# EasyVision-Ton/VMG

Measured on AMD Instinct MI355X. Metric: LR-frames/s (train: forward+loss+backward+AdamW), VMG-REDS-few_levels 4x SR, higher is better.
Workload: dtype bf16; 1 GPU; VMG-REDS-few_levels train step, per-GPU batch 4x7x3x64x64 -> 4x SR (BASELINE configs[1]); global_batch=4, frames_per_clip=7, parallelism=dp1, launch=eager, recompute_chains=False, fp8_chains=False

## Files before the change

include/vmg_hip.h:

```cpp
#ifndef VMG_HIP_H
#define VMG_HIP_H

#include <stdint.h>

#ifdef __cplusplus
extern "C" {
#endif

#define VMG_F32 0
#define VMG_BF16 1

#define VMG_ACT_NONE 0
#define VMG_ACT_RELU 1
#define VMG_ACT_LRELU 2
#define VMG_ACT_GELU 3

#define VMG_CONV_GENERAL 0
#define VMG_CONV_KSPLIT 2
#define VMG_CONV_WS 3
#define VMG_CONV_LINEAR_WRES 4
#define VMG_CONV_WSTAT 6

const char* vmg_last_error(void);
int vmg_version(void);

typedef struct vmg_ctx vmg_ctx;
vmg_ctx* vmg_create(int device);
int vmg_destroy(vmg_ctx* ctx);
int vmg_ctx_device(const vmg_ctx* ctx);
int vmg_max_lds_bytes(void);

int64_t vmg_conv_pack_bytes(int dtype, int ks, int on, int nsrc, const int* src_ch, int cout_tiles);
int vmg_conv_pack(int dtype, const float* w, int O, int I, int ks, int o0, int on, int nsrc, const int* src_off,
                  const int* src_ch, int transpose_flip, int cout_tiles, void* packed, void* stream);

int64_t vmg_convws_pack_bytes(int on, int nsrc, const int* src_ch, int cout_tiles);
int vmg_convws_pack(const float* w, int O, int I, int o0, int on, int nsrc, const int* src_off, const int* src_ch, int transpose_flip,
                    int cout_tiles, void* packed, void* stream);

typedef struct vmg_conv_desc {
  int dtype, ks, cout_tiles;
  int N, H, W, Cout;
  int nsrc;
  const void* src[4];
  int64_t src_ps[4];
  int src_ch[4];
  const void* packed;
  const float* bias;
  void* out;
  int64_t out_ps;
  void* out_pre;
  const void* res;
  int64_t res_ps;
  const void* aux;
  int64_t aux_ps;
  int act;
  float slope, alpha;
  int actgrad;
  int pixel_shuffle;
  int mt;
  int deep;
} vmg_conv_desc;

int vmg_conv_fwd(const vmg_conv_desc* d, void* stream);
enum {
  VMG_CONV_FAM_IGEMM = 1,
  VMG_CONV_FAM_KSPLIT = 2,
  VMG_CONV_FAM_WS = 3,
  VMG_CONV_FAM_LINEAR_WRES = 4,
  VMG_CONV_FAM_WSTAT = 5,
  VMG_CONV_PLAN_INTS = 11
};
int vmg_conv_fwd_plan(const vmg_conv_desc* d, int ncu, int* plan);
typedef struct vmg_chain_desc {
  int dtype, N, H, W, C, nblk, nsrc;
  const void* src[4];
  int64_t src_ps[4];
  int src_ch[4];
  const void* packed0;
  const float* bias0;
  float slope0;
  int cout_tiles0, deep0;
  const void* const* packed1;
  const float* const* bias1;
  const void* const* packed2;
  const float* const* bias2;
  float r_scaling;
  int cout_tiles, deep;
  void* const* y;
  void* const* t;
  void* const* g_y;
  void* const* g_t;
} vmg_chain_desc;
int vmg_resblock_chain_fwd(const vmg_chain_desc* d, void* stream);
int vmg_resblock_chain_bwd(const vmg_chain_desc* d, void* stream);

void* vmg_replay_build(void* hip_graph, int* n_ops, int* n_kernels);
int vmg_replay_kernel_info(void* replay, int idx, void** func, unsigned* grid_x, unsigned* block_x, void** first_arg);
int vmg_replay_run(void* replay, int first, int last, void* stream);
void vmg_replay_destroy(void* replay);

int vmg_pack_entry_bytes(void);
int vmg_pack_entry(void* entry, int kind, int dtype, const float* w, int O, int I, int ks, int o0, int on, int nsrc, const int* src_off,
                   const int* src_ch, int transpose_flip, int cout_tiles, void* packed, int blk0);
int vmg_pack_run(const void* plan_dev, int n, int total_blocks, void* stream);

int vmg_conv_debug_stamps(void* buf);

int vmg_conv_wgrad(int dtype, int ks, int N, int H, int W, const void* x, int64_t x_ps, int Cin, const void* dy,
                   int64_t dy_ps, int Cout, float* dW, int I_total, int o0, int i0, float* db, float scale,
                   void* stream);
int vmg_conv_wgrad_batched(int dtype, int ks, int npairs, const void* const* x, const void* const* dy, int N, int H, int W,
                           int64_t x_ps, int Cin, int64_t dy_ps, int Cout, float* dW, int I_total, int o0, int i0, float* db,
                           float scale, void* stream);

int64_t vmg_conv_wgrad_ws_bytes(void);
int vmg_conv_wgrad_batched_ws(int dtype, int ks, int npairs, const void* const* x, const void* const* dy, int N, int H, int W,
                              int64_t x_ps, int Cin, int64_t dy_ps, int Cout, float* dW, int I_total, int o0, int i0, float* db,
                              float scale, void* ws, int64_t ws_bytes, void* stream);
int vmg_conv_wgrad3_multi(int nprob, int npairs, const void* const* x, const void* const* dy, int N, int H, int W, int64_t x_ps, int Cin,
                          int64_t dy_ps, int Cout, float* const* dW, int I_total, int o0, int i0, float* const* db, const float* scales, void* ws,
                          int64_t ws_bytes, void* stream);
int vmg_conv_wgrad3_variant(int variant);
int vmg_linear_wgrad2_multi(int nprob, int npairs, const void* const* x, const void* const* dy, int64_t M, int64_t x_ps, int Cin, int64_t dy_ps,
                            int Cout, float* const* dW, int I_total, int o0, int i0, float* const* db, const float* scales, void* ws,
                            int64_t ws_bytes, void* stream);
#define VMG_WGRAD_V1 1
#define VMG_WGRAD_3 2
#define VMG_WGRAD_3B 3
#define VMG_WGRAD_L2 4
#define VMG_WGRAD_7 5
int vmg_conv_wgrad_last_kernel(void);
#define VMG_WGRAD_ENTRY_PLAIN 0
#define VMG_WGRAD_ENTRY_WS 1
#define VMG_WGRAD_ENTRY_MULTI 2
#define VMG_WGRAD_ALIGN_X16 1
#define VMG_WGRAD_ALIGN_DY16 2
#define VMG_WGRAD_ALIGN_DY2 4
#define VMG_WGRAD_PLAN_INTS 7
int vmg_conv_wgrad_plan(int entry, int dtype, int ks, int nprob, int npairs, int N, int H, int W, int64_t x_ps, int Cin, int64_t dy_ps, int Cout,
                        int I_total, int o0, int i0, int align, int64_t ws_bytes, int* plan);

int vmg_act_bwd(int dtype, const void* dy, const void* ref, void* out, int64_t n, int act, float slope, float alpha,
                void* stream);
int vmg_pixel_shuffle(int dtype, const void* in, void* out, int N, int H, int W, int c, int to_depth, void* stream);
int vmg_sum_n(int dtype, const void* const* srcs, int nsrc, void* out, int64_t n, void* stream);
int vmg_cast_clear(int dtype, float* acc, const void* add, void* out, int64_t n, void* stream);
int vmg_pair_steps(int dtype, int mode, void* const* steps, void* a, void* b, int n, int t, int64_t frame_elems, void* stream);
int vmg_frame_gather(int dtype, const void* src, void* dst, const int* idx, int64_t frame_elems, int n_src_frames, int n_dst_frames, int nsrc,
                     void* stream);
int vmg_pixel_unshuffle_actgrad(int dtype, const void* dy, const void* ref, void* out, int N, int H, int W, int c, int act, float slope,
                                float alpha, void* stream);
int vmg_layernorm_fwd(int dtype, const void* x, const float* w, const float* b, void* y, float* mean, float* rstd, int64_t M,
                      int C, float eps, void* stream);
int64_t vmg_layernorm_bwd_ws_bytes(void);
int vmg_layernorm_bwd(int dtype, int ndy, const void* const* dy, const void* x, const float* mean, const float* rstd, const float* w,
                      const void* add, void* dx, float* dw, float* db, int64_t M, int C, void* ws, void* stream);

int vmg_space_depth_ln_fwd(int dtype, int mode, const void* x, const float* w, const float* b, void* y, float* mean, float* rstd, int N, int H,
                           int W, int cseg, float eps, void* stream);
int vmg_space_depth_ln_bwd(int dtype, int mode, const void* dy, const void* x, const float* mean, const float* rstd, const float* w, void* dx,
                           float* dw, float* db, int N, int H, int W, int cseg, void* ws, void* stream);

int64_t vmg_group_reduce_ws_bytes(void);
int vmg_group_reduce(int dtype, const void* a, const void* b, const void* c3, float* out, int G, int64_t R, int C, int mode, float scale,
                     float* ws, int64_t ws_bytes, void* stream);
int vmg_group_reduce3(int dtype, const void* a, const void* b0, const void* b1, const void* b2, float* out, int G, int64_t R, int C, float scale,
                      float* ws, int64_t ws_bytes, void* stream);
int vmg_tab_elementwise(int dtype, int op, const void* p0, const void* p1, const void* p2, const float* coef, const float* add, float s,
                        void* o0, void* o1, void* o2, int64_t rows, int64_t R, int C, void* stream);

int vmg_warp_bilinear_fwd(int dtype, const void* x, const float* flow, void* out, int N, int H, int W, int C, void* stream);
int vmg_warp_bilinear_bwd(int dtype, const void* x, const float* flow, const void* dy, void* dx_acc, float* dflow, int N, int H,
                          int W, int C, void* stream);
int vmg_warp_nearest_planes(const float* loc, const float* flow, float* out, int N, int K2, int H, int W, void* stream);
int vmg_flow_smooth(const float* in, float* out, int64_t planes, int H, int W, int r, int backward, void* stream);

int vmg_ltam_fwd(int dtype, const void* q, const void* const* keys, const void* const* vals, const float* loc, const float* rpe,
                 const float* decay, void* out, float* lse, int n, int h, int w, int c, int heads, int wh, int ww, int t, float scale,
                 void* stream);
int vmg_ltam_bwd(int dtype, const void* q, const void* const* keys, const void* const* vals, const float* loc, const float* rpe,
                 const float* decay, const void* out, const float* lse, const void* dout, void* dq, void* const* dk_acc,
                 void* const* dv_acc, float* drpe, int n, int h, int w, int c, int heads, int wh, int ww, int t, float scale,
                 void* stream);
int64_t vmg_ltam_tab_bytes(int t);
int vmg_ltam_fwd_tab(int dtype, const void* q, const void* const* keys, const void* const* vals, const float* loc, const float* rpe,
                     const float* decay, void* out, float* lse, int n, int h, int w, int c, int heads, int wh, int ww, int t, float scale,
                     void* ws, int64_t ws_bytes, void* stream);
int vmg_ltam_bwd_tab(int dtype, const void* q, const void* const* keys, const void* const* vals, const float* loc, const float* rpe,
                     const float* decay, const void* out, const float* lse, const void* dout, void* dq, void* const* dk_acc,
                     void* const* dv_acc, float* drpe, int n, int h, int w, int c, int heads, int wh, int ww, int t, float scale,
                     void* ws, int64_t ws_bytes, void* stream);

int vmg_ltam_max_fwd(int dtype, const void* q, const void* const* keys, const void* const* vals, const float* loc, void* out, int* idx,
                     float* score, int n, int h, int w, int c, int heads, int t, void* stream);
int vmg_ltam_max_bwd(int dtype, const void* q, const void* const* keys, const void* const* vals, const float* loc, const int* idx,
                     const void* dout, void* dq, void* const* dk_acc, void* const* dv_acc, int n, int h, int w, int c, int heads, int t,
                     void* stream);
int vmg_ltam_max_fwd_tab(int dtype, const void* q, const void* const* keys, const void* const* vals, const float* loc, void* out, int* idx,
                         float* score, int n, int h, int w, int c, int heads, int t, void* ws, int64_t ws_bytes, void* stream);
int vmg_ltam_max_bwd_tab(int dtype, const void* q, const void* const* keys, const void* const* vals, const float* loc, const int* idx,
                         const void* dout, void* dq, void* const* dk_acc, void* const* dv_acc, int n, int h, int w, int c, int heads, int t,
                         void* ws, int64_t ws_bytes, void* stream);

int vmg_prof_begin(vmg_ctx* ctx, int klass, int stride, int max_samples);
int vmg_prof_end(vmg_ctx* ctx, int64_t* launches_seen, int* samples, double* total_ms);
int vmg_prof_select_pixels(vmg_ctx* ctx, int64_t pixels);
double vmg_prof_null_interval_us(int reps, void* stream);

int vmg_morphfc_fwd(int axis, int chunk, const void* x, const void* relu_mask, const void* packed, const float* bias, void* out, void* tok_out,
                    int BT, int H, int W, int C, int Cp, int cout_tiles, int relu, float in_scale, float out_scale, void* stream);
int64_t vmg_morphfc_token_rows(int axis, int chunk, int BT, int H, int W);
int64_t vmg_morph_token_rows(int axis, int chunk, int BT, int H, int W);
int vmg_morph_tokens_gather(int dtype, int axis, int chunk, const void* x, void* tok, int BT, int H, int W, int C, int Cp, int ld, void* stream);
int vmg_morph_tokens_scatter(int dtype, int axis, int chunk, const void* tok, void* out, int BT, int H, int W, int C, int Cp, int ld, void* stream);

int vmg_win3d_attn_fwd(int dtype, const void* q, const void* kv, const float* bq, const float* bkv, const float* table, void* out, float* lse,
                       int B, int D, int H, int W, int C, int heads, int wt, int sd, int sh, int sw, void* stream);
int64_t vmg_win3d_attn_bwd_ws_bytes(int B, int D, int H, int W, int heads, int wt);
int vmg_win3d_attn_bwd(int dtype, const void* q, const void* kv, const float* bq, const float* bkv, const float* table, const void* out,
                       const float* lse, const void* d_out, void* dq, void* dkv, float* dtable, float* dbq, float* dbkv, void* ws, int B, int D, int H, int W,
                       int C, int heads, int wt, int sd, int sh, int sw, void* stream);
int vmg_win3d_variant(int variant);

int vmg_maxpool_fwd(int dtype, const void* x, void* y, unsigned char* idx, int N, int H, int W, int C, int f, void* stream);
int vmg_maxpool_bwd(int dtype, const void* dy, const unsigned char* idx, void* dx, int N, int H, int W, int C, int f, void* stream);

int vmg_se_mlp_fwd(const float* m, const float* w1, const float* b1, const float* w2, const float* b2, float* pre, float* out, int G, int C,
                   int Hd, int Co, int act1, int mode, void* stream);
int vmg_se_mlp_bwd(const float* dout, const float* out, const float* m, const float* pre, const float* w1, const float* w2, float* dm,
                   float* dw1, float* db1, float* dw2, float* db2, float* ws, int G, int C, int Hd, int Co, int act1, int mode, float dm_scale,
                   int accumulate, void* stream);

int vmg_avgpool2_nhwc(int dtype, const void* x, void* y, int n, int h, int w, int c, void* stream);
int vmg_upsample2x_ac_fwd(const float* x, float* y, int n, int h, int w, int c, float scale, void* stream);
int vmg_upsample2x_ac_bwd(const float* dy, float* dx, int n, int h, int w, int c, float scale, void* stream);
int vmg_spy_operand_fwd(int dtype, const void* ref, const void* warped, const float* up, void* out, int64_t npix, void* stream);
int vmg_spy_operand_bwd(int dtype, const void* dx8, void* dwarped, float* dup, int64_t npix, void* stream);
int vmg_spy_flow_add(int dtype, const float* up, const void* res, float* out, int64_t n, void* stream);
int vmg_spy_prep(int dtype, const float* img, const float* mean, const float* stdv, void* out, int64_t n, int h, int w, void* stream);
typedef struct vmg_spy_module_desc {
  int N, H, W;
  const void* x;
  const void* packed[5];
  const float* bias[5];
  void* y[4];
  void* out;
  void* dpre[4];
} vmg_spy_module_desc;
int vmg_spy_module_fwd(const vmg_spy_module_desc* d, void* stream);
int vmg_spy_module_bwd(const vmg_spy_module_desc* d, void* stream);

int vmg_tile_accumulate(int dtype, const void* patch, float* E, float* Wt, int64_t planes, int ph, int pw, int EH, int EW, int oh, int ow,
                        int top, int bottom, int left, int right, void* stream);
int vmg_tile_finalize(const float* E, const float* Wt, float* out_f32, unsigned char* out_u8, int64_t n, void* stream);

int64_t vmg_frame_metrics_ws_bytes(int T, int H, int W);
// ... 86 lines not shown
```

vmg_amd/csrc/conv_igemm.hip:

```cpp
#include <stdlib.h>

#include <type_traits>

#include "common.h"

namespace {

constexpr int MAX_ISRC = 32;
constexpr int CBMAX = 160;

__host__ __device__ constexpr int kstg(int ks) { return ks > 1 ? ks : 2; }
__host__ __device__ constexpr int stage_bytes(int ks, int ntb, int cb) { return kstg(ks) * 4 * ntb * 16 * cb; }
__host__ __device__ constexpr int stage_stride(int ks, int ntb, int cb) { return (stage_bytes(ks, ntb, cb) + 4095) / 4096 * 4096; }
__host__ __device__ inline int stages_of(int ks, int ch) {
  const int nb = (ch / 8 + 3) / 4;
  return ks > 1 ? ks * nb : (nb + 1) / 2;
}

struct ConvK {
  const char* src[MAX_ISRC];
  long long src_ps[MAX_ISRC];
  short src_ch[MAX_ISRC];
  short src_nst[MAX_ISRC];
  int src_pixb[MAX_ISRC];
  int nsrc;
  const char* wpack;
  const float* bias;
  char* out;
  long long out_ps;
  char* out_pre;
  const char* res;
  long long res_ps;
  const char* aux;
  long long aux_ps;
  int N, H, W, Cout, tiles_x, tiles_y;
  long long M;
  int act;
  float slope, alpha;
  int actgrad, ps;
  int nstages;
  int halo_bytes;
  int ring;
  int vec8;
  unsigned long long* stamps;
  int dbg;
};

template <typename T>
struct Frag;
template <>
struct Frag<bf16> {
  bf16x8 v;
  __device__ __forceinline__ void load(const char* p) { v = *reinterpret_cast<const bf16x8*>(p); }
};
template <>
struct Frag<float> {
  float4 lo, hi;
  __device__ __forceinline__ void load(const char* p) {
    lo = *reinterpret_cast<const float4*>(p);
    hi = *reinterpret_cast<const float4*>(p + 16);
  }
};
__device__ __forceinline__ f32x4 mma(const Frag<bf16>& w, const Frag<bf16>& x, f32x4 c) {
  return __builtin_amdgcn_mfma_f32_16x16x32_bf16(w.v, x.v, c, 0, 0, 0);
}
__device__ __forceinline__ f32x4 mma(const Frag<float>& w, const Frag<float>& x, f32x4 c) {
  c = __builtin_amdgcn_mfma_f32_16x16x4f32(w.lo.x, x.lo.x, c, 0, 0, 0);
  c = __builtin_amdgcn_mfma_f32_16x16x4f32(w.lo.y, x.lo.y, c, 0, 0, 0);
  c = __builtin_amdgcn_mfma_f32_16x16x4f32(w.lo.z, x.lo.z, c, 0, 0, 0);
  c = __builtin_amdgcn_mfma_f32_16x16x4f32(w.lo.w, x.lo.w, c, 0, 0, 0);
  c = __builtin_amdgcn_mfma_f32_16x16x4f32(w.hi.x, x.hi.x, c, 0, 0, 0);
  c = __builtin_amdgcn_mfma_f32_16x16x4f32(w.hi.y, x.hi.y, c, 0, 0, 0);
  c = __builtin_amdgcn_mfma_f32_16x16x4f32(w.hi.z, x.hi.z, c, 0, 0, 0);
  c = __builtin_amdgcn_mfma_f32_16x16x4f32(w.hi.w, x.hi.w, c, 0, 0, 0);
  return c;
}

__device__ uint4 g_conv_zero16;
__device__ uint4 g_wstat_trash;

#ifdef VMG_DIAG
#define VMG_DBG(a, bit) ((a).dbg & (bit))
__device__ __forceinline__ void conv_stamp(const ConvK& a, int wave, int slot) {
  if (a.stamps) {
    const unsigned long long t = __builtin_amdgcn_s_memrealtime();
    if ((threadIdx.x & 63) == 0) a.stamps[((size_t)(blockIdx.y * gridDim.x + blockIdx.x) * 4 + wave) * 8 + slot] = t;
  }
}
#else
#define VMG_DBG(a, bit) 0
__device__ __forceinline__ void conv_stamp(const ConvK&, int, int) {}
#endif

__device__ __forceinline__ int xcd_remap(int bid, int nblk, int dbg) {
#ifndef VMG_DIAG
  dbg = 0;
#endif
  if ((nblk & 7) != 0 || (dbg & 128)) return bid;
  return (bid & 7) * (nblk >> 3) + (bid >> 3);
}

__device__ __forceinline__ void glds16_asm(const char* gsrc, char* lds_dst) {
  unsigned keep;
  const unsigned ldst = __builtin_amdgcn_readfirstlane((unsigned)(uintptr_t)LDS_PTR(lds_dst));
  asm volatile("s_mov_b32 %0, m0\n\ts_mov_b32 m0, %2\n\ts_nop 0\n\tglobal_load_lds_dwordx4 %1, off\n\ts_mov_b32 m0, %0"
               : "=&s"(keep) : "v"(gsrc), "s"(ldst) : "memory");
}

__device__ __forceinline__ void glds16_asm_s(const char* sbase, int voff, char* lds_dst) {
  unsigned keep;
  const unsigned ldst = __builtin_amdgcn_readfirstlane((unsigned)(uintptr_t)LDS_PTR(lds_dst));
  asm volatile("s_mov_b32 %0, m0\n\ts_mov_b32 m0, %3\n\ts_nop 0\n\tglobal_load_lds_dwordx4 %1, %2\n\ts_mov_b32 m0, %0"
               : "=&s"(keep) : "v"(voff), "s"(sbase), "s"(ldst) : "memory");
}

template <typename T, int KS, int MT>
__device__ __forceinline__ void stage_halo(const ConvK& a, int s, char* halo, int n, int ty, int tx, long long m0, int tid) {
  constexpr int ES = ElemTraits<T>::ES;
  constexpr int TH = 4 * MT;
  constexpr int TWH = 16 + KS - 1;
  constexpr int THH = TH + KS - 1;
  const int lane = tid & 63, wave = tid >> 6;
// ... 301 lines not shown
        if (j + 1 < KSTG) load_frags(j + 1, (j + 1) & 1);
#pragma unroll
        for (int ct = 0; ct < NTB; ++ct)
#pragma unroll
          for (int mt = 0; mt < MT; ++mt) acc[ct][mt] = mma(wf[j & 1][ct], xf[j & 1][mt], acc[ct][mt]);
      }
    }
  }
  asm volatile("s_waitcnt vmcnt(0)" ::: "memory");

#pragma unroll
  for (int mt = 0; mt < MT; ++mt) {
    f32x4 r[NTB];
#pragma unroll
    for (int ct = 0; ct < NTB; ++ct) r[ct] = acc[ct][mt];
    conv_epilogue_row<T, KS, NTB>(a, r, wave * MT + mt, TH, cb, nt_real, n, ty, tx, m0, px, g);
  }
}

template <int NTB>
struct EpiLds {
  static constexpr int COB = NTB * 16, C8 = 2 * NTB, PSTR = COB * 4 + 16, NIT = (16 * C8 + 63) / 64;
  static constexpr int BYTES = 16 * PSTR;
};

template <int KS, int NTB>
__device__ __forceinline__ void conv_epilogue_prefetch8(const ConvK& a, int row, int TH, int cb, int n, int ty, int tx, long long m0, int lane,
                                                        bf16x8 (&pre_res)[EpiLds<NTB>::NIT], bf16x8 (&pre_aux)[EpiLds<NTB>::NIT]) {
  using E = EpiLds<NTB>;
  const bf16* res = reinterpret_cast<const bf16*>(a.res);
  const bf16* aux = reinterpret_cast<const bf16*>(a.aux);
#pragma unroll
  for (int it = 0; it < E::NIT; ++it) {
    const int j = it * 64 + lane, pxi = j / E::C8, c8 = j - pxi * E::C8;
    long long pix;
    const bool valid = conv_row_pixel<KS>(a, row, TH, n, ty, tx, m0, pxi & 15, pix);
    const int co = cb * E::COB + c8 * 8;
    if (j < 16 * E::C8 && valid && co < a.Cout) {
      if (res) pre_res[it] = *reinterpret_cast<const bf16x8*>(res + pix * a.res_ps + co);
      if (aux) pre_aux[it] = *reinterpret_cast<const bf16x8*>(aux + pix * a.aux_ps + co);
    }
  }
}

template <int KS, int NTB>
__device__ __forceinline__ void conv_epilogue_lds8(const ConvK& a, const f32x4 (&acc)[NTB], char* stg, int row, int TH, int cb, int n, int ty, int tx,
                                                   long long m0, int lane, const bf16x8 (&pre_res)[EpiLds<NTB>::NIT],
                                                   const bf16x8 (&pre_aux)[EpiLds<NTB>::NIT], const float* lbias) {
  using E = EpiLds<NTB>;
  const int px = lane & 15, g = lane >> 4;
#pragma unroll
  for (int ct = 0; ct < NTB; ++ct) *reinterpret_cast<f32x4*>(stg + px * E::PSTR + (ct * 16 + g * 4) * 4) = acc[ct];
  bf16* out = reinterpret_cast<bf16*>(a.out);
  bf16* out_pre = reinterpret_cast<bf16*>(a.out_pre);
  const float neg = a.act == VMG_ACT_RELU ? 0.f : (a.act == VMG_ACT_LRELU ? a.slope : 1.f);
#pragma unroll
  for (int it = 0; it < E::NIT; ++it) {
    const int j = it * 64 + lane, pxi = j / E::C8, c8 = j - pxi * E::C8;
    long long pix;
    const bool valid = conv_row_pixel<KS>(a, row, TH, n, ty, tx, m0, pxi & 15, pix);
    const int co = cb * E::COB + c8 * 8;
    if (!(j < 16 * E::C8 && valid && co < a.Cout) || VMG_DBG(a, 8)) continue;
    const f32x4 lo = *reinterpret_cast<const f32x4*>(stg + pxi * E::PSTR + c8 * 32);
    const f32x4 hi = *reinterpret_cast<const f32x4*>(stg + pxi * E::PSTR + c8 * 32 + 16);
    float v[8] = {lo[0], lo[1], lo[2], lo[3], hi[0], hi[1], hi[2], hi[3]};
    if (a.bias) {
      const f32x4 b0 = *reinterpret_cast<const f32x4*>(lbias + c8 * 8), b1 = *reinterpret_cast<const f32x4*>(lbias + c8 * 8 + 4);
#pragma unroll
      for (int r = 0; r < 4; ++r) { v[r] += b0[r]; v[4 + r] += b1[r]; }
    }
    if (out_pre) {
      bf16x8 t;
#pragma unroll
      for (int r = 0; r < 8; ++r) t[r] = (bf16)v[r];
      *reinterpret_cast<bf16x8*>(out_pre + pix * a.out_ps + co) = t;
    }
    if (a.act == VMG_ACT_GELU) {
#pragma unroll
      for (int r = 0; r < 8; ++r) v[r] = gelu_erf(v[r]) * a.alpha;
    } else {
#pragma unroll
      for (int r = 0; r < 8; ++r) v[r] = (v[r] > 0.f ? v[r] : v[r] * neg) * a.alpha;
    }
    if (a.aux) {
#pragma unroll
      for (int r = 0; r < 8; ++r) {
        const float u = (float)pre_aux[it][r];
        v[r] *= a.actgrad == 3 ? gelu_erf_grad(u) : (u > 0.f ? 1.f : (a.actgrad == 2 ? a.slope : 0.f));
      }
    }
    if (a.res) {
#pragma unroll
      for (int r = 0; r < 8; ++r) v[r] += (float)pre_res[it][r];
    }
    bf16x8 t;
#pragma unroll
    for (int r = 0; r < 8; ++r) t[r] = (bf16)v[r];
    *reinterpret_cast<bf16x8*>(out + pix * a.out_ps + co) = t;
  }
}

template <typename T, int KS, int NTB>
__global__ __launch_bounds__(256, (NTB <= 3 ? 3 : 2)) void conv_ksplit_kernel(const ConvK a) {
  constexpr int ES = ElemTraits<T>::ES, CB = ElemTraits<T>::CHUNKB;
  constexpr int TH = 4;
  constexpr int TWH = 16 + KS - 1;
  constexpr int COB = NTB * 16;
  constexpr int SS = stage_stride(KS, NTB, CB);
  constexpr int KSB = 4 * COB * CB;
  extern __shared__ __attribute__((aligned(16))) char smem[];
  char* halo = smem;
  char* zslot = smem + a.halo_bytes;
  float* lbias = reinterpret_cast<float*>(zslot + 16);
  if (VMG_DBG(a, 16)) return;

  const int tid = threadIdx.x, lane = tid & 63;
  const int wave = __builtin_amdgcn_readfirstlane(tid >> 6);
  const int px = lane & 15, g = lane >> 4;
  const int cb = blockIdx.y;
  const int nt_real = min(NTB, (a.Cout - cb * COB + 15) >> 4);
  int n = 0, ty = 0, tx = 0;
  long long m0 = 0;
  if (KS > 1) {
    int bid = xcd_remap(blockIdx.x, gridDim.x, a.dbg);
    tx = bid % a.tiles_x;
    int r = bid / a.tiles_x;
    ty = r % a.tiles_y;
    n = r / a.tiles_y;
  } else {
    m0 = (long long)blockIdx.x * 64;
  }
  conv_stamp(a, wave, 0);
  if (tid < 4) reinterpret_cast<int*>(zslot)[tid] = 0;
  const float bias_r = (tid < COB && a.bias && cb * COB + tid < a.Cout) ? a.bias[cb * COB + tid] : 0.f;

  constexpr bool BF = std::is_same<T, bf16>::value;
  const bool vec8 = BF && a.vec8 != 0;
  bf16x8 pre_res[EpiLds<NTB>::NIT], pre_aux[EpiLds<NTB>::NIT];
  if (vec8) conv_epilogue_prefetch8<KS, NTB>(a, wave, TH, cb, n, ty, tx, m0, lane, pre_res, pre_aux);

  f32x4 acc[NTB][4];
#pragma unroll
  for (int ct = 0; ct < NTB; ++ct)
#pragma unroll
    for (int i = 0; i < 4; ++i) acc[ct][i] = f32x4{0.f, 0.f, 0.f, 0.f};

  const char* wlane = a.wpack + (long long)cb * a.nstages * SS + g * (COB * CB) + px * CB;
  int st0 = 0;
  for (int s = 0; s < a.nsrc; ++s) {
    const int ch = a.src_ch[s], pixb = a.src_pixb[s];
    const int CH = ch >> 3, nb = (CH + 3) >> 2;
    if (s > 0) __syncthreads();
    conv_stamp(a, wave, 1);
    stage_halo<T, KS, 1>(a, s, halo, n, ty, tx, m0, tid);
    if (s == 0 && tid < COB) lbias[tid] = bias_r;
    conv_stamp(a, wave, 3);
    __syncthreads();
    conv_stamp(a, wave, 4);

    const int nks = VMG_DBG(a, 32) ? 0 : (KS > 1 ? 9 * nb : nb);
    const int per = ((nks + 3) / 4 + 2) / 3 * 3;
    const int k0 = wave * per;
    const int rowb = TWH * pixb;
    const char* pixp = halo + px * pixb;
    int rowoff[4];
#pragma unroll
    for (int i = 0; i < 4; ++i) rowoff[i] = ((wave + i) & 3) * rowb;

    Frag<T> wf[3][NTB], xf[3][4];
    struct Cur { int k, cbk, ky, kx; long long woff; };
    auto cur_at = [&](int k) {
      Cur c;
      c.k = k;
      const int kc = min(k, nks - 1);
      if (KS > 1) {
        c.cbk = kc / 9;
        const int tap = kc - 9 * c.cbk;
// ... 266 lines not shown
      }
    };
    bf16* out = reinterpret_cast<bf16*>(a.out);
    bf16* out_pre = FULL ? reinterpret_cast<bf16*>(a.out_pre) : nullptr;
    const bf16* res = FULL ? reinterpret_cast<const bf16*>(a.res) : nullptr;
    const bf16* aux = FULL ? reinterpret_cast<const bf16*>(a.aux) : nullptr;
    const float neg = a.act == VMG_ACT_RELU ? 0.f : (a.act == VMG_ACT_LRELU ? a.slope : 1.f);
    int ipos[NCT], ipatch[NCT], ico[NCT];
#pragma unroll
    for (int i = 0; i < NCT; ++i) {
      const int j = 64 * h + lane + 256 * i;
      const int p = j / C8, c8 = j - p * C8;
      ipos[i] = ((p >> 4) << 8) | (p & 15);
      ipatch[i] = p * PSTR + c8 * 32;
      ico[i] = c8 * 8;
    }
    const int nstore = NCT * (out_pre ? 2 : 1);
    int ioff[NCT];
    float ibias[NCT][8];
#pragma unroll
    for (int i = 0; i < NCT; ++i) {
      ioff[i] = (((ipos[i] >> 8) * a.W + (ipos[i] & 255)) * (int)a.out_ps + ico[i]) * 2;
#pragma unroll
      for (int q = 0; q < 8; ++q) ibias[i][q] = (a.bias && cb * COB + ico[i] + q < a.Cout) ? a.bias[cb * COB + ico[i] + q] : 0.f;
    }

    if (tile_of(0) < band1) issue_halo(tile_of(0), 0);
    asm volatile("s_waitcnt vmcnt(0)" ::: "memory");
    for (int it = 0;; ++it) {
      barrier();
      const bool more = tile_of(it) < band1;
      if (more && tile_of(it + 1) < band1) issue_halo(tile_of(it + 1), (it + 1) & 1);
      if (it > 0 && !VMG_DBG(a, 64)) {
        const int t = tile_of(it - 1);
        const int tx = t % a.tiles_x, r = t / a.tiles_x;
        const int ty = r % a.tiles_y, n = r / a.tiles_y;
        const long long pix0 = ((long long)n * a.H + ty * TH) * a.W + tx * 16;
        if (!FULL && ty * TH + TH <= a.H && tx * 16 + 16 <= a.W && cb * COB + COB <= a.Cout && !VMG_DBG(a, 8)) {
          char* obase = reinterpret_cast<char*>(out + pix0 * a.out_ps + cb * COB);
#pragma unroll
          for (int i = 0; i < NCT; ++i) {
            const f32x4 lo = *reinterpret_cast<const f32x4*>(patch + ipatch[i]);
            const f32x4 hi = *reinterpret_cast<const f32x4*>(patch + ipatch[i] + 16);
            float v[8] = {lo[0], lo[1], lo[2], lo[3], hi[0], hi[1], hi[2], hi[3]};
            bf16x8 tq;
#pragma unroll
            for (int q = 0; q < 8; ++q) {
              if (a.bias) v[q] += ibias[i][q];
              v[q] = (v[q] > 0.f ? v[q] : v[q] * neg) * a.alpha;
              tq[q] = (bf16)v[q];
            }
            *reinterpret_cast<bf16x8*>(obase + ioff[i]) = tq;
          }
        } else
#pragma unroll
        for (int i = 0; i < NCT; ++i) {
          const int y = ty * TH + (ipos[i] >> 8), x = tx * 16 + (ipos[i] & 255);
          const int co = cb * COB + ico[i];
          const bool valid = y < a.H && x < a.W && co < a.Cout && !VMG_DBG(a, 8);
          const long long pix = valid ? pix0 + (long long)(ipos[i] >> 8) * a.W + (ipos[i] & 255) : 0;
          const f32x4 lo = *reinterpret_cast<const f32x4*>(patch + ipatch[i]);
          const f32x4 hi = *reinterpret_cast<const f32x4*>(patch + ipatch[i] + 16);
          float v[8] = {lo[0], lo[1], lo[2], lo[3], hi[0], hi[1], hi[2], hi[3]};
          if (a.bias) {
            const f32x4 b0 = *reinterpret_cast<const f32x4*>(lbias + ico[i]), b1 = *reinterpret_cast<const f32x4*>(lbias + ico[i] + 4);
#pragma unroll
            for (int q = 0; q < 4; ++q) { v[q] += b0[q]; v[4 + q] += b1[q]; }
          }
          const int cov = valid ? co : 0;
          if (out_pre) {
            bf16x8 tq;
#pragma unroll
            for (int q = 0; q < 8; ++q) tq[q] = (bf16)v[q];
            bf16* dstp = valid ? out_pre + pix * a.out_ps + co : reinterpret_cast<bf16*>(&g_wstat_trash);
            *reinterpret_cast<bf16x8*>(dstp) = tq;
          }
          if (FULL && a.act == VMG_ACT_GELU) {
#pragma unroll
            for (int q = 0; q < 8; ++q) v[q] = gelu_erf(v[q]) * a.alpha;
          } else {
#pragma unroll
            for (int q = 0; q < 8; ++q) v[q] = (v[q] > 0.f ? v[q] : v[q] * neg) * a.alpha;
          }
          if (aux) {
            const bf16x8 au = *reinterpret_cast<const bf16x8*>(aux + pix * a.aux_ps + cov);
#pragma unroll
            for (int q = 0; q < 8; ++q) {
              const float u = (float)au[q];
              v[q] *= a.actgrad == 3 ? gelu_erf_grad(u) : (u > 0.f ? 1.f : (a.actgrad == 2 ? a.slope : 0.f));
            }
          }
          if (res) {
            const bf16x8 rv = *reinterpret_cast<const bf16x8*>(res + pix * a.res_ps + cov);
#pragma unroll
            for (int q = 0; q < 8; ++q) v[q] += (float)rv[q];
          }
          bf16x8 tq;
#pragma unroll
          for (int q = 0; q < 8; ++q) tq[q] = (bf16)v[q];
          bf16* dst = valid ? out + pix * a.out_ps + co : reinterpret_cast<bf16*>(&g_wstat_trash);
          *reinterpret_cast<bf16x8*>(dst) = tq;
        }
      }
      if (!more) break;
      barrier();
      if (it > 0 && !VMG_DBG(a, 64)) {
        if (nstore == NCT) asm volatile("s_waitcnt vmcnt(%0)" ::"n"(NCT) : "memory");
        else asm volatile("s_waitcnt vmcnt(%0)" ::"n"(2 * NCT) : "memory");
      } else {
        asm volatile("s_waitcnt vmcnt(0)" ::: "memory");
      }
    }
    return;
  }

  barrier();
  Frag<T> wreg[NK][RW];
  const char* wlane = wl + g * (COB * CB) + px * CB;
#pragma unroll
  for (int j = 0; j < NK; ++j)
#pragma unroll
    for (int ct = 0; ct < RW; ++ct) wreg[j][ct].load(wlane + (j / 3) * SS + (j % 3) * KSB + ct * 16 * CB);
  for (int it = 0;; ++it) {
    const int t = tile_of(it);
    if (t >= band1) break;
    const int buf = it & 1;
    f32x4 acc[2][NCT];
#pragma unroll
    for (int mt = 0; mt < 2; ++mt)
#pragma unroll
      for (int ct = 0; ct < NCT; ++ct) acc[mt][ct] = f32x4{0.f, 0.f, 0.f, 0.f};
    const char* hb = halo + buf * HB + ((2 * wave) * TWH + px) * PIXB;
    if (!VMG_DBG(a, 32)) {
      Frag<T> xf[2][2], wf[2][NCT > RW ? NCT - RW : 1];
      auto load_frags = [&](int j, int set) {
        const int cbk = j / 9, tap = j - cbk * 9, ky = tap / 3, kx = tap - ky * 3;
        const char* xc = hb + min(4 * cbk + g, CH - 1) * CB;
#pragma unroll
        for (int mt = 0; mt < 2; ++mt) xf[set][mt].load(xc + ((mt + ky) * TWH + kx) * PIXB);
#pragma unroll
        for (int ct = RW; ct < NCT; ++ct) wf[set][ct - RW].load(wlane + (j / 3) * SS + (j % 3) * KSB + ct * 16 * CB);
      };
      load_frags(0, 0);
#pragma unroll
      for (int j = 0; j < NK; ++j) {
        if (j + 1 < NK) load_frags(j + 1, (j + 1) & 1);
#pragma unroll
        for (int ct = 0; ct < NCT; ++ct)
#pragma unroll
          for (int mt = 0; mt < 2; ++mt) acc[mt][ct] = mma(ct < RW ? wreg[j][ct < RW ? ct : 0] : wf[j & 1][ct >= RW ? ct - RW : 0], xf[j & 1][mt], acc[mt][ct]);
      }
    }
    barrier();
#pragma unroll
    for (int mt = 0; mt < 2; ++mt)
#pragma unroll
      for (int ct = 0; ct < NCT; ++ct) *reinterpret_cast<f32x4*>(patch + ((2 * wave + mt) * 16 + px) * PSTR + (ct * 16 + g * 4) * 4) = acc[mt][ct];
    barrier();
  }
}

template <int NCT>
struct WsGeo {
  static constexpr int COB = NCT * 16;
  static constexpr int KSB = COB * 64;
  static constexpr int STG = 3 * KSB;
  static constexpr int TH = 8, TWH = 18, THH = 10;
  static constexpr int NLW = 3;
  static constexpr int THREADS = (4 + NLW) * 64;
  static constexpr int NIT = EpiLds<NCT>::NIT;
};
__host__ __device__ inline int ws_rem_ksteps(int R) { return R == 0 ? 0 : (R == 1 ? 3 : (R == 2 ? 6 : 9)); }
__host__ __device__ inline int ws_ksteps(int CH) { return 9 * (CH / 4) + ws_rem_ksteps(CH % 4); }
__host__ __device__ inline void ws_slot(int CH, int j, int g, int& tap, int& chunk) {
  const int nfull = CH / 4, R = CH % 4;
  if (j < 9 * nfull) { tap = j % 9; chunk = 4 * (j / 9) + g; return; }
  const int jr = j - 9 * nfull;
  if (R == 1) { tap = 4 * jr + g; chunk = 4 * nfull; }
  else if (R == 2) { tap = 2 * jr + (g >> 1); chunk = 4 * nfull + (g & 1); }
// ... 248 lines not shown
        rd(2, 2);
        mm(1);
        phase_fence();
        if (R == 3) __builtin_amdgcn_s_waitcnt(0xC07F);
        ws_stamp(a, wave, 3 + t);
        __builtin_amdgcn_s_barrier();
        asm volatile("" ::: "memory");
        advance();
        stage_offsets();
        rd(0, 0);
        mm(2);
        phase_fence();
      }
      rd(1, 1);
      mm(0);
      phase_fence();
      rd(2, 2);
      mm(1);
      phase_fence();
      __builtin_amdgcn_s_waitcnt(0xC07F);
      ws_stamp(a, wave, 3 + t);
      __builtin_amdgcn_s_barrier();
      asm volatile("" ::: "memory");
      mm(2);
      __builtin_amdgcn_sched_barrier(0);
      ++t;
      if (s + 1 < a.nsrc) {
        __builtin_amdgcn_s_barrier();
        asm volatile("" ::: "memory");
        next_source();
        stage_offsets();
        rd(0, 0);
        __builtin_amdgcn_sched_barrier(0);
      }
    }
    ws_stamp(a, wave, 28);
    char* prow = ring + ((2 * wave) * 16 + px) * I::PSTR + g * 16;
#pragma unroll
    for (int ct = 0; ct < NCT; ++ct) {
      *reinterpret_cast<f32x4*>(prow + ct * 64) = acc[ct][0];
      *reinterpret_cast<f32x4*>(prow + 16 * I::PSTR + ct * 64) = acc[ct][1];
    }
    __builtin_amdgcn_s_waitcnt(0xC07F);
  }
  ws_stamp(a, wave, 29);
  __builtin_amdgcn_s_barrier();
  asm volatile("" ::: "memory");

  {
    bf16* out = reinterpret_cast<bf16*>(a.out) + tile_pix * a.out_ps + cb * COB;
    bf16* out_pre = a.out_pre ? reinterpret_cast<bf16*>(a.out_pre) + tile_pix * a.out_ps + cb * COB : nullptr;
    const bf16* auxb = a.aux ? reinterpret_cast<const bf16*>(a.aux) + tile_pix * a.aux_ps + cb * COB : nullptr;
#pragma unroll
    for (int it = 0; it < I::NIT; ++it) {
      int pxl, c8;
      I::decode(it * I::THREADS + tid, pxl, c8);
      const int row = pxl >> 4, col = pxl & 15;
      const bool valid = (pxl < 128) & (ty * G::TH + row < a.H) & (tx * 16 + col < a.W) & (cb * COB + c8 * 8 < a.Cout);
      if (!valid) continue;
      const char* pp = ring + pxl * I::PSTR + c8 * 32;
      const f32x4 lo = *reinterpret_cast<const f32x4*>(pp), hi = *reinterpret_cast<const f32x4*>(pp + 16);
      float v[8] = {lo[0], lo[1], lo[2], lo[3], hi[0], hi[1], hi[2], hi[3]};
      const int opix = row * a.W + col;
      if (out_pre) {
        bf16x8 tq;
#pragma unroll
        for (int r = 0; r < 8; ++r) tq[r] = (bf16)v[r];
        *reinterpret_cast<bf16x8*>(out_pre + opix * (int)a.out_ps + c8 * 8) = tq;
      }
      if (a.act == VMG_ACT_GELU) {
#pragma unroll
        for (int r = 0; r < 8; ++r) v[r] = gelu_erf(v[r]);
      } else if (a.act == VMG_ACT_RELU) {
#pragma unroll
        for (int r = 0; r < 8; ++r) v[r] = fmaxf(v[r], 0.f);
      } else if (a.act == VMG_ACT_LRELU) {
#pragma unroll
        for (int r = 0; r < 8; ++r) v[r] = v[r] > 0.f ? v[r] : v[r] * a.slope;
      }
      if (a.alpha != 1.0f) {
#pragma unroll
        for (int r = 0; r < 8; ++r) v[r] *= a.alpha;
      }
      if (auxb) {
        bf16x8 u = pre[it];
        if (a.res) u = *reinterpret_cast<const bf16x8*>(auxb + opix * (int)a.aux_ps + c8 * 8);
#pragma unroll
        for (int r = 0; r < 8; ++r) {
          const float uf = (float)u[r];
          v[r] *= a.actgrad == 3 ? gelu_erf_grad(uf) : (uf > 0.f ? 1.f : (a.actgrad == 2 ? a.slope : 0.f));
        }
      }
      if (a.res) {
#pragma unroll
        for (int r = 0; r < 8; ++r) v[r] += (float)pre[it][r];
      }
      bf16x8 tq;
#pragma unroll
      for (int r = 0; r < 8; ++r) tq[r] = (bf16)v[r];
      __builtin_nontemporal_store(tq, reinterpret_cast<bf16x8*>(out + opix * (int)a.out_ps + c8 * 8));
    }
  }
  ws_stamp(a, wave, 31);
}

struct PackK {
  const float* w;
  char* out;
  int O, I, ks, o0, on, nsrc, transpose_flip, cob, ncb, nstages, ss_elems;
  int groups;
  int fast3;
  long long units;
  short src_off[MAX_ISRC], src_ch[MAX_ISRC], src_st0[MAX_ISRC], src_nst[MAX_ISRC];
};

__device__ __forceinline__ float pack_weight_value(const PackK& p, int oc, int kc, int tap, int KK) {
  if (p.groups <= 1) {
    if (!p.transpose_flip) return p.w[((long long)oc * p.I + kc) * KK + tap];
    return p.w[((long long)kc * p.I + oc) * KK + (KK - 1 - tap)];
  }
  const int og = p.O / p.groups;
  if (!p.transpose_flip) {
    const int kl = kc - (oc / og) * p.I;
    return (kl >= 0 && kl < p.I) ? p.w[((long long)oc * p.I + kl) * KK + tap] : 0.f;
  }
  const int g = oc / p.I;
  return (kc / og == g) ? p.w[((long long)kc * p.I + (oc - g * p.I)) * KK + (KK - 1 - tap)] : 0.f;
}

template <typename T>
__device__ __forceinline__ void pack_std_vec8(const PackK& p, long long i8) {
  const unsigned i = (unsigned)i8 * 8u;
  const int KK = p.ks * p.ks, KSTG = kstg(p.ks);
  const int body = KSTG * 4 * p.cob * 8;
  const unsigned r = i / (unsigned)p.ss_elems;
  const int within = (int)(i - r * (unsigned)p.ss_elems);
  const int cb = (int)(r / (unsigned)p.nstages);
  const int stage = (int)(r - (unsigned)cb * (unsigned)p.nstages);
  float v[8];
#pragma unroll
  for (int e = 0; e < 8; ++e) v[e] = 0.f;
  if (within < body) {
    int t = within >> 3;
    const int co = t % p.cob;
    t /= p.cob;
    const int g = t & 3, j = t >> 2;
    int s = 0;
    while (s + 1 < p.nsrc && stage >= p.src_st0[s + 1]) ++s;
    const int sl = stage - p.src_st0[s];
    const int CH = p.src_ch[s] >> 3;
    int tap, q;
    if (p.ks > 1) { const int cbk = sl / p.ks, ky = sl - p.ks * cbk; tap = ky * p.ks + j; q = 4 * cbk + g; }
    else { tap = 0; q = 4 * (2 * sl + j) + g; }
    const int col = cb * p.cob + co;
    if (q < CH && col < p.on) {
      const int kc = p.src_off[s] + q * 8;
      const int oc = p.o0 + col;
#pragma unroll
      for (int e = 0; e < 8; ++e) v[e] = pack_weight_value(p, oc, kc + e, tap, KK);
    }
  }
  if constexpr (std::is_same<T, bf16>::value) {
    bf16x8 o;
#pragma unroll
    for (int e = 0; e < 8; ++e) o[e] = (bf16)v[e];
    *reinterpret_cast<bf16x8*>(reinterpret_cast<bf16*>(p.out) + i) = o;
  } else {
    f32x4* o = reinterpret_cast<f32x4*>(reinterpret_cast<float*>(p.out) + i);
    o[0] = f32x4{v[0], v[1], v[2], v[3]};
    o[1] = f32x4{v[4], v[5], v[6], v[7]};
  }
}

template <typename T>
__global__ void conv_pack_kernel(const PackK p) {
  const long long total8 = (long long)p.ncb * p.nstages * p.ss_elems / 8;
  for (long long i = blockIdx.x * (long long)blockDim.x + threadIdx.x; i < total8; i += (long long)gridDim.x * blockDim.x) pack_std_vec8<T>(p, i);
}

// ... 499 lines not shown
  VMG_LAUNCH_CHECK();
  return 0;
}

extern "C" int vmg_pack_entry_bytes(void) { return (int)sizeof(PackEntry); }

extern "C" int vmg_pack_entry(void* entry, int kind, int dtype, const float* w, int O, int I, int ks, int o0, int on, int nsrc, const int* src_off,
                              const int* src_ch, int transpose_flip, int cout_tiles, void* packed, int blk0) {
  VMG_CHECK(entry && (kind == 0 || kind == 1) && blk0 >= 0, "pack_entry: bad arguments");
  PackEntry e;
  memset(&e, 0, sizeof(e));
  int rc;
  if (kind == 1) {
    VMG_CHECK(ks == 3 && dtype == VMG_BF16, "pack_entry: the weight-streaming layout is bf16 3x3");
    rc = fill_pack_ws(e.p, e.total, w, O, I, o0, on, nsrc, src_off, src_ch, transpose_flip, cout_tiles, packed);
  } else {
    rc = fill_pack_std(e.p, e.total, dtype, w, O, I, ks, o0, on, nsrc, src_off, src_ch, transpose_flip, cout_tiles, packed);
  }
  if (rc) return rc;
  e.kind = kind; e.dtype = dtype; e.blk0 = blk0;
  long long nb = e.p.fast3 ? (e.p.units + 255) / 256 : (e.total + 256LL * 16 - 1) / (256LL * 16);
  e.nblk = (int)(nb < 1 ? 1 : (nb > 64 ? 64 : nb));
  memcpy(entry, &e, sizeof(e));
  return e.nblk;
}

extern "C" int vmg_pack_run(const void* plan_dev, int n, int total_blocks, void* stream) {
  VMG_CHECK(plan_dev && n > 0 && total_blocks > 0, "pack_run: bad arguments");
  static_assert(sizeof(PackEntry) % 4 == 0, "the block-owner table sits behind the entries");
  hipLaunchKernelGGL(pack_batch_kernel, dim3(total_blocks), dim3(256), 0, (hipStream_t)stream, (const PackEntry*)plan_dev, n);
  VMG_LAUNCH_CHECK();
  return 0;
}

static int conv_plan(const vmg_conv_desc* d, int ncu, ConvK& k, ConvPlan& p) {
  VMG_CHECK(d != nullptr, "conv_fwd: null descriptor");
  VMG_CHECK(d->ks == 1 || d->ks == 3 || d->ks == 7, "conv_fwd: ks must be 1, 3 or 7");
  VMG_CHECK(d->dtype == VMG_F32 || d->dtype == VMG_BF16, "conv_fwd: bad dtype");
  VMG_CHECK(d->nsrc >= 1 && d->nsrc <= 4, "conv_fwd: nsrc must be 1..4");
  VMG_CHECK(d->N > 0 && d->H > 0 && d->W > 0 && d->Cout > 0, "conv_fwd: bad shape");
  VMG_CHECK(d->packed && d->out, "conv_fwd: null packed weights / output");
  VMG_CHECK(!d->pixel_shuffle || (d->Cout % 4 == 0), "conv_fwd: pixel_shuffle needs Cout %% 4 == 0");
  VMG_CHECK(!(d->actgrad != 0 && d->aux == nullptr), "conv_fwd: actgrad without aux");
  VMG_CHECK(d->deep == VMG_CONV_GENERAL || d->deep == VMG_CONV_KSPLIT || d->deep == VMG_CONV_WS || d->deep == VMG_CONV_LINEAR_WRES ||
                d->deep == VMG_CONV_WSTAT,
            "conv_fwd: unknown kernel route deep = %d", d->deep);
  const int es = d->dtype == VMG_BF16 ? 2 : 4, cbytes = es * 8;
  memset(&k, 0, sizeof(k));
  memset(&p, 0, sizeof(p));
  short xoff[MAX_ISRC];
  int parent[MAX_ISRC];
  const int n = expand_sources(d->nsrc, nullptr, d->src_ch, xoff, k.src_ch, parent);
  VMG_CHECK(n > 0, "conv_fwd: source channel counts must be multiples of 8");
  int mt = d->mt;
  if (d->dtype == VMG_F32) mt = 1;
  const long long M = (long long)d->N * d->H * d->W;
  const int ntb = d->cout_tiles;
  VMG_CHECK(ntb > 0, "conv_fwd: cout_tiles must be positive");
  const int ncb = cdiv(d->Cout, ntb * 16);
  if (d->ks == 7) mt = 1;
  if (mt == 0) mt = 1;
  VMG_CHECK(mt == 1 || mt == 2, "conv_fwd: mt must be 1 or 2");
  const int TH = 4 * mt, TWH = 16 + d->ks - 1, THH = TH + d->ks - 1;
  int kt = 0, halo = 0;
  for (int s = 0; s < n; ++s) {
    const int par = parent[s];
    VMG_CHECK(d->src[par] != nullptr, "conv_fwd: null source %d", par);
    VMG_CHECK(d->src_ps[par] >= d->src_ch[par] && (d->src_ps[par] * es) % 16 == 0, "conv_fwd: source pixel stride must be >= channels and 16-byte aligned");
    VMG_CHECK(((uintptr_t)d->src[par]) % 16 == 0, "conv_fwd: source pointer must be 16-byte aligned");
    k.src[s] = (const char*)d->src[par] + (long long)xoff[s] * es;
    k.src_ps[s] = d->src_ps[par];
    k.src_nst[s] = (short)stages_of(d->ks, k.src_ch[s]);
    k.src_pixb[s] = choose_pixb(k.src_ch[s], es, cbytes);
    kt += k.src_nst[s];
    const int hb = THH * TWH * k.src_pixb[s];
    if (hb > halo) halo = hb;
  }
  k.nsrc = n;
  k.wpack = (const char*)d->packed; k.bias = d->bias;
  k.out = (char*)d->out; k.out_ps = d->out_ps; k.out_pre = (char*)d->out_pre;
  k.res = (const char*)d->res; k.res_ps = d->res_ps; k.aux = (const char*)d->aux; k.aux_ps = d->aux_ps;
  k.N = d->N; k.H = d->H; k.W = d->W; k.Cout = d->Cout; k.M = M;
  k.tiles_x = cdiv(d->W, 16); k.tiles_y = cdiv(d->H, TH);
  k.act = d->act; k.slope = d->slope; k.alpha = d->alpha; k.actgrad = d->aux ? d->actgrad : 0; k.ps = d->pixel_shuffle;
#ifdef VMG_DIAG
  {
    const char* e = getenv("VMG_CONV_DBG");
    k.dbg = e ? atoi(e) : 0;
    k.stamps = g_conv_stamps;
  }
#endif
  {
    auto al = [](const void* ptr) { return ((uintptr_t)ptr & 15) == 0; };
    k.vec8 = d->dtype == VMG_BF16 && !d->pixel_shuffle && (d->Cout % 16) == 0 && (d->out_ps % 8) == 0 && al(d->out) &&
             (!d->out_pre || al(d->out_pre)) && (!d->res || ((d->res_ps % 8) == 0 && al(d->res))) &&
             (!d->aux || ((d->aux_ps % 8) == 0 && al(d->aux)));
  }
  k.nstages = kt; k.halo_bytes = (halo + 1023) & ~1023;
  VMG_CHECK(d->out_ps >= (d->pixel_shuffle ? d->Cout / 4 : d->Cout), "conv_fwd: out pixel stride too small");
  p.dtype = d->dtype; p.ks = d->ks; p.mt = mt; p.ntb = ntb; p.vec8 = k.vec8; p.gy = ncb;
  auto cus = [&]() { return ncu > 0 ? ncu : vmg_cu_count(vmg_current_device()); };
  if (d->deep == VMG_CONV_WS) {
    VMG_CHECK(d->dtype == VMG_BF16 && d->ks == 3 && k.vec8 && (ntb == 3 || ntb == 7 || ntb == 8 || ntb == 9), "conv_fwd: the weight-streaming kernel is bf16 3x3 with 16-byte aligned rows, cout_tiles 3, 7, 8 or 9");
    for (int s = 0; s < n; ++s) VMG_CHECK(k.src_ch[s] % 16 == 0, "conv_fwd: the weight-streaming kernel takes channel blocks that are multiples of 16 (got %d)", k.src_ch[s]);
    int kt3 = 0, halo3 = 0;
    for (int s = 0; s < n; ++s) {
      k.src_pixb[s] = k.src_ch[s] * 2;
      k.src_nst[s] = (short)(ws_ksteps(k.src_ch[s] >> 3) / 3);
      kt3 += k.src_nst[s];
      const int hb = 10 * 18 * k.src_pixb[s];
      if (hb > halo3) halo3 = hb;
    }
    k.nstages = kt3;
    k.halo_bytes = (halo3 + 1023) & ~1023;
    k.tiles_y = cdiv(d->H, 8);
    k.ring = ntb <= 3 ? 3 : ((k.halo_bytes + 4 * ws_stage_bytes(ntb) + ntb * 16 * 4 <= 160 * 1024) ? 4 : 3);
    p.lds = k.halo_bytes + k.ring * ws_stage_bytes(ntb) + ntb * 16 * 4;
    VMG_CHECK(p.lds <= 160 * 1024, "conv (weight-streaming): LDS request %d B exceeds 160 KiB", p.lds);
    const long long nblk = (long long)k.N * k.tiles_y * k.tiles_x;
    VMG_CHECK(nblk > 0 && nblk < (1ll << 31), "conv: bad grid %lld", nblk);
    p.family = VMG_CONV_FAM_WS; p.gx = (int)nblk;
    return 0;
  }
  if (d->deep == VMG_CONV_WSTAT && d->dtype == VMG_BF16 && d->ks == 3 && mt == 1 && k.vec8 && n == 1 && (ntb == 1 || ntb == 3 || ntb == 4) && k.src_ch[0] <= 64 && k.src_ch[0] % 8 == 0 &&
      k.src_ps[0] % 8 == 0 && d->W <= 255 * 16 && (long long)d->W * k.src_ps[0] * 2 * 10 < (1ll << 31)) {
    const int nb = (k.src_ch[0] / 8 + 3) / 4;
    VMG_CHECK(k.nstages == 3 * nb, "conv (weights-stationary): %d stages in the pack, %d expected", k.nstages, 3 * nb);
    k.tiles_y = cdiv(d->H, 8);
    const long long ntiles = (long long)k.N * k.tiles_y * k.tiles_x;
    VMG_CHECK(ntiles > 0 && ntiles < (1ll << 30), "conv: bad tile count %lld", ntiles);
    int nwg = cus() & ~7;
    if (nwg < 8) nwg = 8;
    while (nwg > 8 && (long long)(nwg >> 3) > cdiv64(ntiles, 8)) nwg -= 8;
    const bool full = k.res || k.aux || k.out_pre || k.act == VMG_ACT_GELU;
    p.family = VMG_CONV_FAM_WSTAT; p.variant = nb | (full ? 16 : 0); p.gx = nwg; p.lds = wstat_lds_bytes(ntb, nb);
    return 0;
  }
  if (d->deep == VMG_CONV_LINEAR_WRES && d->dtype == VMG_BF16 && d->ks == 1 && k.vec8 && (ntb == 3 || ntb == 5)) {
    int ns = 0;
    if (n == 1 && k.src_ch[0] <= 160 && k.src_pixb[0] == k.src_ch[0] * 2) ns = 1;
    else if (n == 2 && ntb == 3 && d->nsrc == 1 && k.src_ch[0] == k.src_ch[1] && k.src_ch[0] <= 160 && k.src[1] == k.src[0] + k.src_ch[0] * 2 &&
             k.src_nst[0] == k.src_nst[1])
      ns = 2;
    if (ns) {
      const long long ntiles = cdiv64(k.M, 16);
      VMG_CHECK(ntiles > 0 && ntiles < (1ll << 31), "conv: bad tile count %lld", ntiles);
      const int wg_per_cu = ns == 1 ? 2 : 1, c = cus();
      long long waves = (long long)(wg_per_cu * c / ncb > 0 ? wg_per_cu * c / ncb : 1) * 4;
      long long tpw = cdiv64(ntiles, waves);
      if (tpw < 4) tpw = 4;
      p.family = VMG_CONV_FAM_LINEAR_WRES; p.variant = ns; p.gx = (int)cdiv64(cdiv64(ntiles, tpw), 4); p.tpw = (int)tpw; p.lds = wres_lds_bytes(ntb, ns);
      return 0;
    }
  }
  const bool ksplit = d->ks != 7 && d->deep == VMG_CONV_KSPLIT;
  if (ksplit) {
    VMG_CHECK(d->dtype == VMG_BF16 && mt == 1, "conv_fwd: the k-split variant is bf16, mt = 1");
    if (!(ntb == 1 || ntb == 3 || ntb == 4 || ntb == 5)) {
      vmg_set_error("conv (k-split): cout_tiles must be 1, 3, 4 or 5 (got %d)", ntb);
      return -1;
    }
    const int scratch = 12 * ntb * 1024;
    p.lds = (k.halo_bytes > scratch ? k.halo_bytes : scratch) + 16 + ntb * 16 * 4;
    VMG_CHECK(p.lds <= 160 * 1024, "conv (k-split): LDS request %d B exceeds 160 KiB", p.lds);
    k.halo_bytes = p.lds - 16 - ntb * 16 * 4;
    p.family = VMG_CONV_FAM_KSPLIT;
  } else {
    if (d->ks == 7) {
      if (!(ntb == 1 || ntb == 2 || ntb == 4)) {
        vmg_set_error("conv (7x7): cout_tiles must be 1, 2 or 4 (got %d)", ntb);
        return -1;
      }
    } else if (!(ntb == 1 || ntb == 3 || ntb == 4 || ntb == 5 || ntb == 7 || ntb == 8 || ntb == 9)) {
      vmg_set_error("conv: cout_tiles must be 1, 3, 4, 5, 7, 8 or 9 (got %d)", ntb);
      return -1;
    }
    p.lds = k.halo_bytes + 2 * stage_stride(d->ks, ntb, cbytes);
    VMG_CHECK(p.lds <= 160 * 1024, "conv: LDS request %d B exceeds 160 KiB", p.lds);
    p.family = VMG_CONV_FAM_IGEMM;
  }
  const long long nblk = (d->ks > 1) ? (long long)k.N * k.tiles_y * k.tiles_x : cdiv64(k.M, 64 * mt);
  VMG_CHECK(nblk > 0 && nblk < (1ll << 31), "conv: bad grid %lld", nblk);
  p.gx = (int)nblk;
  return 0;
}

static int conv_launch(const ConvK& k, const ConvPlan& p, hipStream_t st) {
  switch (p.family) {
    case VMG_CONV_FAM_WS:
      return p.ntb == 9 ? launch_ws<9>(k, p, st) : (p.ntb == 7 ? launch_ws<7>(k, p, st) : (p.ntb == 8 ? launch_ws<8>(k, p, st) : launch_ws<3>(k, p, st)));
    case VMG_CONV_FAM_WSTAT:
      switch (p.ntb * 2 + ((p.variant & 15) - 1)) {
        case 2: return launch_wstat<1, 1>(k, p, st);
        case 3: return launch_wstat<1, 2>(k, p, st);
        case 6: return launch_wstat<3, 1>(k, p, st);
        case 7: return launch_wstat<3, 2>(k, p, st);
        case 8: return launch_wstat<4, 1>(k, p, st);
        case 9: return launch_wstat<4, 2>(k, p, st);
      }
      break;
    case VMG_CONV_FAM_LINEAR_WRES:
      if (p.variant == 2) return launch_linear_wres<3, 2>(k, p, st);
      return p.ntb == 3 ? launch_linear_wres<3>(k, p, st) : launch_linear_wres<5>(k, p, st);
    case VMG_CONV_FAM_KSPLIT:
      return p.ks == 3 ? dispatch_ksplit<bf16, 3>(k, p, st) : dispatch_ksplit<bf16, 1>(k, p, st);
    case VMG_CONV_FAM_IGEMM:
      if (p.ks == 7) return p.dtype == VMG_BF16 ? dispatch_ks7<bf16>(k, p, st) : dispatch_ks7<float>(k, p, st);
      if (p.dtype == VMG_BF16) {
        if (p.ks == 3) return p.mt == 2 ? dispatch_ntb<bf16, 3, 2>(k, p, st) : dispatch_ntb<bf16, 3, 1>(k, p, st);
        return p.mt == 2 ? dispatch_ntb<bf16, 1, 2>(k, p, st) : dispatch_ntb<bf16, 1, 1>(k, p, st);
      }
      if (p.ks == 3) return dispatch_ntb<float, 3, 1>(k, p, st);
      return dispatch_ntb<float, 1, 1>(k, p, st);
  }
  vmg_set_error("conv_fwd: no kernel for plan family %d", p.family);
  return -1;
}

extern "C" int vmg_conv_fwd(const vmg_conv_desc* d, void* stream) {
  ConvK k;
  ConvPlan p;
  if (conv_plan(d, 0, k, p)) return -1;
  return conv_launch(k, p, (hipStream_t)stream);
}

extern "C" int vmg_conv_fwd_plan(const vmg_conv_desc* d, int ncu, int* plan) {
  VMG_CHECK(plan != nullptr && ncu >= 0, "conv_fwd_plan: null plan / negative ncu");
  ConvK k;
  ConvPlan p;
  if (conv_plan(d, ncu, k, p)) return -1;
  const int v[VMG_CONV_PLAN_INTS] = {p.family, p.dtype, p.ks, p.mt, p.ntb, p.variant, p.vec8, p.gx, p.gy, p.tpw, p.lds};
  for (int i = 0; i < VMG_CONV_PLAN_INTS; ++i) plan[i] = v[i];
  return 0;
}

static void chain_base(const vmg_chain_desc* c, vmg_conv_desc& d) {
  memset(&d, 0, sizeof(d));
  d.dtype = c->dtype; d.ks = 3; d.N = c->N; d.H = c->H; d.W = c->W; d.Cout = c->C; d.alpha = 1.f;
  d.nsrc = 1; d.src_ps[0] = c->C; d.src_ch[0] = c->C; d.out_ps = c->C; d.cout_tiles = c->cout_tiles; d.deep = c->deep; d.mt = 1;
}

extern "C" int vmg_resblock_chain_fwd(const vmg_chain_desc* c, void* stream) {
  VMG_CHECK(c && c->nblk >= 0 && c->nsrc >= 1 && c->nsrc <= 4 && c->y && c->packed0, "resblock_chain_fwd: bad descriptor");
  VMG_CHECK(c->nblk == 0 || (c->t && c->packed1 && c->packed2 && c->bias1 && c->bias2), "resblock_chain_fwd: null block arrays");
  vmg_conv_desc d;
  chain_base(c, d);
  d.nsrc = c->nsrc;
  for (int s = 0; s < c->nsrc; ++s) { d.src[s] = c->src[s]; d.src_ps[s] = c->src_ps[s]; d.src_ch[s] = c->src_ch[s]; }
  d.packed = c->packed0; d.bias = c->bias0; d.out = c->y[0]; d.act = VMG_ACT_LRELU; d.slope = c->slope0;
  d.cout_tiles = c->cout_tiles0; d.deep = c->deep0;
  int rc = vmg_conv_fwd(&d, stream);
  if (rc) return rc;
  for (int k = 0; k < c->nblk; ++k) {
    chain_base(c, d);
    d.src[0] = c->y[k]; d.packed = c->packed1[k]; d.bias = c->bias1[k]; d.out = c->t[k]; d.act = VMG_ACT_RELU;
    if ((rc = vmg_conv_fwd(&d, stream))) return rc;
    chain_base(c, d);
    d.src[0] = c->t[k]; d.packed = c->packed2[k]; d.bias = c->bias2[k]; d.out = c->y[k + 1]; d.alpha = c->r_scaling;
    d.res = c->y[k]; d.res_ps = c->C;
    if ((rc = vmg_conv_fwd(&d, stream))) return rc;
  }
  return 0;
}

extern "C" int vmg_resblock_chain_bwd(const vmg_chain_desc* c, void* stream) {
  VMG_CHECK(c && c->nblk >= 0 && c->g_y, "resblock_chain_bwd: bad descriptor");
  VMG_CHECK(c->nblk == 0 || (c->t && c->g_t && c->packed1 && c->packed2), "resblock_chain_bwd: null block arrays");
  vmg_conv_desc d;
  for (int k = c->nblk - 1; k >= 0; --k) {
    chain_base(c, d);
    d.src[0] = c->g_y[k + 1]; d.packed = c->packed2[k]; d.out = c->g_t[k]; d.alpha = c->r_scaling; d.aux = c->t[k]; d.aux_ps = c->C; d.actgrad = 1;
    int rc = vmg_conv_fwd(&d, stream);
    if (rc) return rc;
    chain_base(c, d);
    d.src[0] = c->g_t[k]; d.packed = c->packed1[k]; d.out = c->g_y[k]; d.res = c->g_y[k + 1]; d.res_ps = c->C;
    if ((rc = vmg_conv_fwd(&d, stream))) return rc;
  }
  return 0;
}
```

vmg_amd/csrc/warp.hip:

```cpp
#include "common.h"

namespace {

__device__ __forceinline__ float unnorm_coord(float pix, float flow, int size) {
  const float g = __fadd_rn(pix, flow);
  const float denom = (float)(size - 1 > 1 ? size - 1 : 1);
  const float gn = __fsub_rn(__fdiv_rn(__fmul_rn(2.0f, g), denom), 1.0f);
  return __fmul_rn(__fdiv_rn(__fadd_rn(gn, 1.0f), 2.0f), (float)(size - 1));
}

__device__ __forceinline__ float clip_border(float v, int size, float* grad_mult) {
  const float hi = (float)(size - 1);
  if (v <= 0.f) { if (grad_mult) *grad_mult = 0.f; return 0.f; }
  if (v >= hi) { if (grad_mult) *grad_mult = 0.f; return hi; }
  if (grad_mult) *grad_mult = 1.f;
  return v;
}

template <typename T>
struct V16 {
  static constexpr int N = 16 / sizeof(T);
  T v[N];
};

template <typename T>
__global__ __launch_bounds__(256) void warp_bilinear_fwd_kernel(const T* __restrict__ x, const float* __restrict__ flow,
                                                                T* __restrict__ out, int N, int H, int W, int C) {
  constexpr int VN = V16<T>::N;
  const int nvec = C / VN;
  const long long total = (long long)N * H * W * nvec;
  for (long long i = blockIdx.x * 256LL + threadIdx.x; i < total; i += (long long)gridDim.x * 256) {
    const int v = (int)(i % nvec);
    const long long pix = i / nvec;
    const int px = (int)(pix % W);
    const int py = (int)((pix / W) % H);
    const long long n = pix / ((long long)W * H);
    const float fx = flow[pix * 2], fy = flow[pix * 2 + 1];
    const float ix = clip_border(unnorm_coord((float)px, fx, W), W, nullptr);
    const float iy = clip_border(unnorm_coord((float)py, fy, H), H, nullptr);
    const float x0f = floorf(ix), y0f = floorf(iy);
    const int x0 = (int)x0f, y0 = (int)y0f, x1 = x0 + 1, y1 = y0 + 1;
    const float x1f = x0f + 1.f, y1f = y0f + 1.f;
    const float wnw = (x1f - ix) * (y1f - iy), wne = (ix - x0f) * (y1f - iy), wsw = (x1f - ix) * (iy - y0f), wse = (ix - x0f) * (iy - y0f);
    const T* base = x + n * H * W * C + v * VN;
    float acc[VN];
#pragma unroll
    for (int e = 0; e < VN; ++e) acc[e] = 0.f;
    auto corner = [&](int yy, int xx, float wgt) {
      if (yy >= 0 && yy < H && xx >= 0 && xx < W) {
        const V16<T> t = *reinterpret_cast<const V16<T>*>(base + ((long long)yy * W + xx) * C);
#pragma unroll
        for (int e = 0; e < VN; ++e) acc[e] += to_f32(t.v[e]) * wgt;
      }
    };
    corner(y0, x0, wnw);
    corner(y0, x1, wne);
    corner(y1, x0, wsw);
    corner(y1, x1, wse);
    V16<T> o;
#pragma unroll
    for (int e = 0; e < VN; ++e) o.v[e] = from_f32<T>(acc[e]);
    *reinterpret_cast<V16<T>*>(out + pix * C + v * VN) = o;
  }
}

typedef __attribute__((ext_vector_type(2))) __bf16 wp_bf16x2;
template <typename T>
__global__ __launch_bounds__(256) void warp_bilinear_bwd_kernel(const T* __restrict__ x, const float* __restrict__ flow,
                                                                const T* __restrict__ dy, float* __restrict__ dx_acc,
                                                                float* __restrict__ dflow, int N, int H, int W, int C) {
  const int lane = threadIdx.x & 63;
  const long long npix = (long long)N * H * W;
  for (long long pix = blockIdx.x * 4LL + (threadIdx.x >> 6); pix < npix; pix += (long long)gridDim.x * 4) {
    const int px = (int)(pix % W);
    const int py = (int)((pix / W) % H);
    const long long n = pix / ((long long)W * H);
    const float fx = flow[pix * 2], fy = flow[pix * 2 + 1];
    float gmx, gmy;
    const float ix = clip_border(unnorm_coord((float)px, fx, W), W, &gmx);
    const float iy = clip_border(unnorm_coord((float)py, fy, H), H, &gmy);
    const float x0f = floorf(ix), y0f = floorf(iy);
    const int x0 = (int)x0f, y0 = (int)y0f, x1 = x0 + 1, y1 = y0 + 1;
    const float x1f = x0f + 1.f, y1f = y0f + 1.f;
    const float tx = ix - x0f, ty = iy - y0f;
    const float wnw = (x1f - ix) * (y1f - iy), wne = (ix - x0f) * (y1f - iy), wsw = (x1f - ix) * (iy - y0f), wse = (ix - x0f) * (iy - y0f);
    const bool vnw = y0 >= 0 && y0 < H && x0 >= 0 && x0 < W, vne = y0 >= 0 && y0 < H && x1 >= 0 && x1 < W;
    const bool vsw = y1 >= 0 && y1 < H && x0 >= 0 && x0 < W, vse = y1 >= 0 && y1 < H && x1 >= 0 && x1 < W;
    const long long ib = n * H * W * C;
    const long long onw = ib + ((long long)y0 * W + x0) * C, one = ib + ((long long)y0 * W + x1) * C;
    const long long osw = ib + ((long long)y1 * W + x0) * C, ose = ib + ((long long)y1 * W + x1) * C;
    float gix = 0.f, giy = 0.f;
    if constexpr (sizeof(T) == 2) {
      for (int cb = 0; cb < C; cb += 128) {
        const int cp = cb + 2 * lane;
        const bool in = cp < C;
        const long long own = pix * C;
        const int cl = in ? cp : 0;
        const wp_bf16x2 gp = *reinterpret_cast<const wp_bf16x2*>(dy + own + cl);
        const wp_bf16x2 xnw = *reinterpret_cast<const wp_bf16x2*>(x + (vnw ? onw : own) + cl), xne = *reinterpret_cast<const wp_bf16x2*>(x + (vne ? one : own) + cl);
        const wp_bf16x2 xsw = *reinterpret_cast<const wp_bf16x2*>(x + (vsw ? osw : own) + cl), xse = *reinterpret_cast<const wp_bf16x2*>(x + (vse ? ose : own) + cl);
        const float g0 = in ? (float)gp[0] : 0.f, g1 = in ? (float)gp[1] : 0.f;
        const int sl = lane >> 1;
        const float a0 = __shfl(g0, sl, 64), a1 = __shfl(g1, sl, 64), b0 = __shfl(g0, 32 + sl, 64), b1 = __shfl(g1, 32 + sl, 64);
        const float glo = (lane & 1) ? a1 : a0, ghi = (lane & 1) ? b1 : b0;
        const int clo = cb + lane, chi = cb + 64 + lane;
        auto corner = [&](long long o, float wgt, float sx, float sy, wp_bf16x2 xp) __attribute__((always_inline)) {
          if (clo < C) atomicAdd(dx_acc + o + clo, glo * wgt);
          if (chi < C) atomicAdd(dx_acc + o + chi, ghi * wgt);
          const float xv = (float)xp[0] * g0 + (float)xp[1] * g1;
          gix += xv * sx;
          giy += xv * sy;
        };
        if (vnw) corner(onw, wnw, -(1.f - ty), -(1.f - tx), xnw);
        if (vne) corner(one, wne, (1.f - ty), -tx, xne);
        if (vsw) corner(osw, wsw, -ty, (1.f - tx), xsw);
        if (vse) corner(ose, wse, ty, tx, xse);
      }
    } else {
      for (int c = lane; c < C; c += 64) {
        const float g = to_f32(dy[pix * C + c]);
        if (vnw) { atomicAdd(dx_acc + onw + c, g * wnw); const float xv = to_f32(x[onw + c]) * g; gix -= xv * (1.f - ty); giy -= xv * (1.f - tx); }
        if (vne) { atomicAdd(dx_acc + one + c, g * wne); const float xv = to_f32(x[one + c]) * g; gix += xv * (1.f - ty); giy -= xv * tx; }
        if (vsw) { atomicAdd(dx_acc + osw + c, g * wsw); const float xv = to_f32(x[osw + c]) * g; gix -= xv * ty; giy += xv * (1.f - tx); }
        if (vse) { atomicAdd(dx_acc + ose + c, g * wse); const float xv = to_f32(x[ose + c]) * g; gix += xv * ty; giy += xv * tx; }
      }
    }
    gix = wave_sum(gix);
    giy = wave_sum(giy);
    if (lane == 0) {
      dflow[pix * 2] = gix * gmx;
      dflow[pix * 2 + 1] = giy * gmy;
    }
  }
}

__global__ __launch_bounds__(256) void warp_nearest_planes_kernel(const float* __restrict__ loc, const float* __restrict__ flow,
                                                                  float* __restrict__ out, int N, int K2, int H, int W) {
  const long long total = (long long)N * H * W;
  for (long long pix = blockIdx.x * 256LL + threadIdx.x; pix < total; pix += (long long)gridDim.x * 256) {
    const int px = (int)(pix % W);
    const int py = (int)((pix / W) % H);
    const long long n = pix / ((long long)W * H);
    const float ix = clip_border(unnorm_coord((float)px, flow[pix * 2], W), W, nullptr);
    const float iy = clip_border(unnorm_coord((float)py, flow[pix * 2 + 1], H), H, nullptr);
    const int xn = (int)nearbyintf(ix), yn = (int)nearbyintf(iy);
    const bool ok = xn >= 0 && xn < W && yn >= 0 && yn < H;
    for (int k = 0; k < K2; ++k) {
      const long long plane = (n * K2 + k) * H * W;
      out[plane + (long long)py * W + px] = ok ? loc[plane + (long long)yn * W + xn] : 0.f;
    }
  }
}

int grid_for(long long total) {
  long long b = (total + 255) / 256;
  return (int)(b > 8192 ? 8192 : (b < 1 ? 1 : b));
}

__device__ __forceinline__ int fs_reflect(int p, int n) { return p < n ? p : 2 * (n - 1) - p; }

__global__ void flow_smooth_fwd_kernel(const float* __restrict__ in, float* __restrict__ out, long long planes, int H, int W, int r) {
  const long long total = planes * H * W;
  const float inv = 1.0f / (float)(r * r);
  for (long long i = blockIdx.x * (long long)blockDim.x + threadIdx.x; i < total; i += (long long)gridDim.x * blockDim.x) {
    const int x = (int)(i % W), y = (int)((i / W) % H);
    const float* pl = in + (i / ((long long)W * H)) * H * W;
    const int y0 = (y / r) * r, x0 = (x / r) * r;
    float s = 0.f;
    for (int dy = 0; dy < r; ++dy) {
      const float* row = pl + (long long)fs_reflect(y0 + dy, H) * W;
      for (int dx = 0; dx < r; ++dx) s += row[fs_reflect(x0 + dx, W)];
    }
    out[i] = s * inv;
  }
}

__global__ void flow_smooth_bwd_kernel(const float* __restrict__ dout, float* __restrict__ din, long long planes, int H, int W, int r) {
  const long long total = planes * H * W;
  const int hf = (H + r - 1) / r * r, wf = (W + r - 1) / r * r;
  const float inv = 1.0f / (float)(r * r);
  for (long long i = blockIdx.x * (long long)blockDim.x + threadIdx.x; i < total; i += (long long)gridDim.x * blockDim.x) {
    const int x = (int)(i % W), y = (int)((i / W) % H);
    const float* pl = dout + (i / ((long long)W * H)) * H * W;
    int py[2] = {y, 2 * (H - 1) - y}, px[2] = {x, 2 * (W - 1) - x};
    const int ny = (py[1] >= H && py[1] < hf) ? 2 : 1, nx = (px[1] >= W && px[1] < wf) ? 2 : 1;
    float acc = 0.f;
    for (int a = 0; a < ny; ++a) {
      const int y0 = (py[a] / r) * r;
      for (int b = 0; b < nx; ++b) {
        const int x0 = (px[b] / r) * r;
        float g = 0.f;
        for (int dy = 0; dy < r && y0 + dy < H; ++dy)
          for (int dx = 0; dx < r && x0 + dx < W; ++dx) g += pl[(long long)(y0 + dy) * W + x0 + dx];
        acc += g;
      }
    }
    din[i] = acc * inv;
  }
}

}

extern "C" int vmg_warp_bilinear_fwd(int dtype, const void* x, const float* flow, void* out, int N, int H, int W, int C, void* stream) {
  VMG_CHECK(dtype == VMG_F32 || dtype == VMG_BF16, "warp_fwd: bad dtype");
  VMG_CHECK(x && flow && out && N > 0 && H > 0 && W > 0 && C > 0, "warp_fwd: bad arguments");
  const int vn = dtype == VMG_BF16 ? 8 : 4;
  VMG_CHECK(C % vn == 0, "warp_fwd: C must be a multiple of %d", vn);
  VMG_CHECK(((uintptr_t)x | (uintptr_t)out) % 16 == 0, "warp_fwd: pointers must be 16-byte aligned");
  const long long total = (long long)N * H * W * (C / vn);
  hipStream_t st = (hipStream_t)stream;
  if (dtype == VMG_BF16) hipLaunchKernelGGL(warp_bilinear_fwd_kernel<bf16>, dim3(grid_for(total)), dim3(256), 0, st, (const bf16*)x, flow, (bf16*)out, N, H, W, C);
  else hipLaunchKernelGGL(warp_bilinear_fwd_kernel<float>, dim3(grid_for(total)), dim3(256), 0, st, (const float*)x, flow, (float*)out, N, H, W, C);
  VMG_LAUNCH_CHECK();
  return 0;
}

extern "C" int vmg_warp_bilinear_bwd(int dtype, const void* x, const float* flow, const void* dy, void* dx_acc, float* dflow, int N,
                                     int H, int W, int C, void* stream) {
  VMG_CHECK(dtype == VMG_F32 || dtype == VMG_BF16, "warp_bwd: bad dtype");
  VMG_CHECK(x && flow && dy && dx_acc && dflow && N > 0 && H > 0 && W > 0 && C > 0, "warp_bwd: bad arguments");
  const int vn = dtype == VMG_BF16 ? 8 : 4;
  VMG_CHECK(C % vn == 0, "warp_bwd: C must be a multiple of %d", vn);
  VMG_CHECK(((uintptr_t)x | (uintptr_t)dy | (uintptr_t)dx_acc) % 16 == 0, "warp_bwd: pointers must be 16-byte aligned");
  const long long total = (long long)N * H * W * 64;
  hipStream_t st = (hipStream_t)stream;
  if (dtype == VMG_BF16) {
    hipLaunchKernelGGL(warp_bilinear_bwd_kernel<bf16>, dim3(grid_for(total)), dim3(256), 0, st, (const bf16*)x, flow, (const bf16*)dy, (float*)dx_acc, dflow, N, H, W, C);
  } else {
    hipLaunchKernelGGL(warp_bilinear_bwd_kernel<float>, dim3(grid_for(total)), dim3(256), 0, st, (const float*)x, flow, (const float*)dy, (float*)dx_acc, dflow, N, H, W, C);
  }
  VMG_LAUNCH_CHECK();
  return 0;
}

extern "C" int vmg_warp_nearest_planes(const float* loc, const float* flow, float* out, int N, int K2, int H, int W, void* stream) {
  VMG_CHECK(loc && flow && out && N > 0 && K2 > 0 && H > 0 && W > 0, "warp_nearest: bad arguments");
  hipLaunchKernelGGL(warp_nearest_planes_kernel, dim3(grid_for((long long)N * H * W)), dim3(256), 0, (hipStream_t)stream, loc, flow, out, N, K2, H, W);
  VMG_LAUNCH_CHECK();
  return 0;
}

extern "C" int vmg_flow_smooth(const float* in, float* out, int64_t planes, int H, int W, int r, int backward, void* stream) {
  VMG_CHECK(in && out && planes > 0 && H > 0 && W > 0 && r >= 1, "flow_smooth: bad arguments");
  const int hf = (H + r - 1) / r * r, wf = (W + r - 1) / r * r;
  VMG_CHECK(hf - H < H && wf - W < W, "flow_smooth: the reflected padding must be smaller than the plane (as F.pad(mode='reflect') demands)");
  const long long total = planes * H * W;
  if (backward) hipLaunchKernelGGL(flow_smooth_bwd_kernel, dim3(grid_for(total)), dim3(256), 0, (hipStream_t)stream, in, out, (long long)planes, H, W, r);
  else hipLaunchKernelGGL(flow_smooth_fwd_kernel, dim3(grid_for(total)), dim3(256), 0, (hipStream_t)stream, in, out, (long long)planes, H, W, r);
  VMG_LAUNCH_CHECK();
  return 0;
}
```

vmg_amd/functional.py:

```python
from __future__ import annotations

import contextlib
from typing import List, Optional, Sequence

import torch

from . import hip
from . import kernels as K
from .hip import HipError
from .wgrad import DEFERRED, _wgrad_entries, _wgrad_now, flush_deferred_wgrads, recorded, set_wgrad_mode

class _Fn(torch.autograd.Function):

    @classmethod
    def apply(cls, *args):
        return super(torch.autograd.Function, cls).apply(*args)


def _pad_to(n: int, m: int = 8) -> int:
    return (n + m - 1) // m * m


def choose_tiling(M: int, cout: int, ks: int, dtype: torch.dtype, src_ch: Optional[Sequence[int]] = None, pixel_shuffle: bool = False):
    if USE_WS and src_ch is not None and not pixel_shuffle:
        t = K.ws_eligible(cout, ks, dtype, src_ch)
        if t and M <= 16384 and cout in (112, 144):
            return (4 if cout == 112 else 3), 1, hip.CONV_KSPLIT
        if t:
            return t, 1, hip.CONV_WS
    if dtype == torch.bfloat16 and ks == 3 and cout in (144, 288):
        return 3, 1, hip.CONV_KSPLIT
    if dtype == torch.bfloat16 and ks == 1 and src_ch is not None and len(src_ch) == 1 and M >= 65536 and not pixel_shuffle:
        if cout == 144 and src_ch[0] == 144:
            return 5, 1, hip.CONV_LINEAR_WRES
        if cout == 288 and src_ch[0] == 144:
            return 5, 1, hip.CONV_LINEAR_WRES
        if cout == 144 and src_ch[0] == 288:
            return 3, 1, hip.CONV_LINEAR_WRES
    if dtype == torch.bfloat16 and ks == 3 and not pixel_shuffle and M >= (1 << 18) and src_ch is not None and len(src_ch) == 1 and \
            src_ch[0] <= 64 and src_ch[0] % 8 == 0 and cout in (16, 48, 64):
        return cout // 16, 1, hip.CONV_WSTAT
    if dtype == torch.bfloat16 and ks == 3 and not pixel_shuffle and M >= (1 << 20) and src_ch is not None and len(src_ch) == 1 and \
            (cout <= 16 or src_ch[0] <= 16):
        return None, 2, hip.CONV_GENERAL
    return None, 1, hip.CONV_GENERAL


USE_WS = True
GROUPED_DENSE = True

class _PlanState:

    def __init__(self):
        self.plan, self.stamp, self.wkey, self.ents, self.packs = K.PackPlan(), -1, None, [], []


def _from_param(ent) -> bool:
    pw, weight = ent[1], ent[2]
    return pw.call is not None and pw.call[0] == weight.data_ptr()


class _PackCache:

    def __init__(self):
        self.ents = {}
        self.q8 = {}
        self.volatile = set()
        self.epoch = 0
        self.stamp = 0
        self.stable = _PlanState()
        self.vol = _PlanState()
        self.decay = None

    def get(self, key, weight: torch.Tensor, build, planned: bool = True):
        ents = self.ents if planned else self.q8
        ver = (weight._version, self.epoch)
        hit = ents.get(key)
        buf = None
        if hit is not None:
            if hit[2] is weight:
                if hit[0] == ver:
                    return hit[1]
                buf = hit[1].buf
            if planned and hit[0][1] == ver[1] and key not in self.volatile:
                self.volatile.add(key)
                self.stamp += 1
        ent = [ver, build(key, weight, buf), weight]
        if planned and key not in self.volatile and _from_param(ent):
            self.stamp += 1
        ents[key] = ent
        return ent[1]

    def clear(self):
        self.ents.clear()
        self.q8.clear()
        self.volatile.clear()
        self.decay = None
        self.stamp += 1

    def bump_epoch(self):
        self.epoch += 1

    def settled(self, since: int, with_repack: bool) -> bool:
        return self.stamp == since and self.vol.stamp == since and (not with_repack or self.stable.stamp == since)

    def _run_plan(self, st: _PlanState, wkey, member, reset_sig: bool = False):
        fresh = st.stamp != self.stamp or st.wkey != wkey
        if fresh:
            st.ents = [ent for key, ent in self.ents.items() if member(key, ent)]
            st.packs, st.stamp, st.wkey = [ent[1] for ent in st.ents], self.stamp, wkey
            if reset_sig:
                st.plan.sig = None
        if not st.packs:
            return
        st.plan.run(st.packs, reuse=not fresh)
        ep = self.epoch
        for ent in st.ents:
            ent[0] = (ent[2]._version, ep)

    def repack_all(self):
        self._run_plan(self.stable, None, lambda key, ent: key not in self.volatile and _from_param(ent))

    def decay_weights_and_repack(self, weights: Sequence[torch.Tensor], gammas: Sequence[torch.Tensor], n: int = 1):
        wkey = tuple(map(id, weights))
        if weights[0].is_cuda:
            dkey = (wkey, tuple(map(id, gammas)))
            if self.decay is None or self.decay[0] != dkey:
                self.decay = (dkey, K.DecayList(weights, gammas))
            self.decay[1].run(n)
        else:
            with torch.no_grad():
                for _ in range(int(n)):
# ... 331 lines not shown
    y0, _ = K.conv_forward(srcs, packed(w0, dt, "fwd", src_ch, tiles=t0_, deep=d0_), b0, N, H, W, act=hip.ACT_LRELU, slope=0.1, mt=m0_, deep=d0_)
    ys, ts = K.resblock_chain_forward_q8(y0, [packed_q8(params[2 + 4 * k]) for k in range(nblk)], [params[3 + 4 * k] for k in range(nblk)],
                                         [packed_q8(params[4 + 4 * k]) for k in range(nblk)], [params[5 + 4 * k] for k in range(nblk)], r_scaling, keep_t)
    FP8_STATS["chains"] += 1
    return ys, ts


class _ResidualChain(_Fn):

    @staticmethod
    def _run(srcs, params, r_scaling, own_output):
        nblk = (len(params) - 2) // 4
        N, H, W = srcs[0].shape[0], srcs[0].shape[1], srcs[0].shape[2]
        dt = srcs[0].dtype
        M = N * H * W
        src_ch = [t.shape[-1] for t in srcs]
        w0, b0 = params[0], params[1]
        C = w0.shape[0]
        t0_, _, d0_ = choose_tiling(M, C, 3, dt, src_ch)
        tiles, _, deep = choose_tiling(M, C, 3, dt, [C])
        pw1 = [packed(params[2 + 4 * k], dt, "fwd", [C], tiles=tiles, deep=deep) for k in range(nblk)]
        pw2 = [packed(params[4 + 4 * k], dt, "fwd", [C], tiles=tiles, deep=deep) for k in range(nblk)]
        return K.resblock_chain_forward(srcs, packed(w0, dt, "fwd", src_ch, tiles=t0_, deep=d0_), b0, 0.1, d0_, pw1,
                                        [params[3 + 4 * k] for k in range(nblk)], pw2, [params[5 + 4 * k] for k in range(nblk)], r_scaling, deep,
                                        own_output=own_output)

    @staticmethod
    def forward(ctx, r_scaling, nsrc, fp8, *args):
        recompute = nsrc < 0
        nsrc = abs(nsrc)
        srcs = list(args[:nsrc])
        params = args[nsrc:]
        nblk = (len(params) - 2) // 4
        N, H, W = srcs[0].shape[0], srcs[0].shape[1], srcs[0].shape[2]
        dt = srcs[0].dtype
        M = N * H * W
        src_ch = [t.shape[-1] for t in srcs]
        w0, b0 = params[0], params[1]
        C = w0.shape[0]
        fp8 = bool(fp8) and dt == torch.bfloat16 and nblk > 0 and K.q8_eligible(C, C)
        ctx.fp8 = fp8
        if fp8:
            ys, ts = _chain_forward_fp8(srcs, params, r_scaling, keep_t=any(ctx.needs_input_grad) and not recompute)
        else:
            t0_, _, d0_ = choose_tiling(M, C, 3, dt, src_ch)
            tiles, _, deep = choose_tiling(M, C, 3, dt, [C])
            pw1 = [packed(params[2 + 4 * k], dt, "fwd", [C], tiles=tiles, deep=deep) for k in range(nblk)]
            pw2 = [packed(params[4 + 4 * k], dt, "fwd", [C], tiles=tiles, deep=deep) for k in range(nblk)]
            ys, ts = K.resblock_chain_forward(srcs, packed(w0, dt, "fwd", src_ch, tiles=t0_, deep=d0_), b0, 0.1, d0_, pw1,
                                              [params[3 + 4 * k] for k in range(nblk)], pw2, [params[5 + 4 * k] for k in range(nblk)], r_scaling, deep,
                                              own_output=recompute)
        ctx.recompute = recompute
        ctx.meta = (r_scaling, nsrc, nblk, N, H, W, src_ch, C)
        ctx.wgrad = any(ctx.needs_input_grad[3 + nsrc:])
        ctx.defer = ctx.wgrad and DEFERRED.mode == "deferred"
        if ctx.defer:
            for p, pb in zip(params[0::2], params[1::2]):
                ctx.gen = DEFERRED.note_use(p, pb)
        ctx.params = params
        if recompute:
            ctx.save_for_backward(*srcs)
        else:
            ctx.save_for_backward(*srcs, *ys[:max(nblk, 1)], *ts)
        return ys[-1]

    @staticmethod
    def backward(ctx, g):
        r, nsrc, nblk, N, H, W, src_ch, C = ctx.meta
        params = ctx.params
        srcs = list(ctx.saved_tensors[:nsrc])
        if ctx.recompute:
            ys, ts = _chain_forward_fp8(srcs, params, r, True) if ctx.fp8 else _ResidualChain._run(srcs, params, r, False)
            ys = ys[:max(nblk, 1)]
        else:
            ys = list(ctx.saved_tensors[nsrc:nsrc + max(nblk, 1)])
            ts = list(ctx.saved_tensors[nsrc + max(nblk, 1):])
        y0 = ys[0]
        dt = g.dtype
        M = N * H * W
        tiles, mt, deep = choose_tiling(M, C, 3, dt, [C])
        pg = [None] * len(params)
        pd1 = [packed(params[2 + 4 * k], dt, "dgrad", None, 0, C, tiles=tiles, deep=deep) for k in range(nblk)]
        pd2 = [packed(params[4 + 4 * k], dt, "dgrad", None, 0, C, tiles=tiles, deep=deep) for k in range(nblk)]
        gys, gts = K.resblock_chain_backward(g, ts, pd1, pd2, r, deep)
        with DEFERRED.collecting() if ctx.defer else contextlib.nullcontext():
            for k in range(nblk - 1, -1, -1):
                w1, b1, w2, b2 = params[2 + 4 * k: 6 + 4 * k]
                if ctx.defer:
                    DEFERRED.add(w2, b2, [ts[k]], [C], gys[k + 1], 3, N, H, W, scale=r, gen=ctx.gen)
                    DEFERRED.add(w1, b1, [ys[k]], [C], gts[k], 3, N, H, W, gen=ctx.gen)
                elif ctx.wgrad:
                    pg[4 + 4 * k], pg[5 + 4 * k] = _wgrad_now(w2, True, [ts[k]], [C], gys[k + 1], 3, N, H, W, scale=r)
                    pg[2 + 4 * k], pg[3 + 4 * k] = _wgrad_now(w1, True, [ys[k]], [C], gts[k], 3, N, H, W)
            g = gys[0]
            w0, b0 = params[0], params[1]
            dpre0 = K.act_backward(g, y0, hip.ACT_LRELU, 0.1, 1.0)
            d_srcs = []
            off = 0
            for i, c in enumerate(src_ch):
                if ctx.needs_input_grad[3 + i]:
                    t_, m_, d_ = choose_tiling(M, c, 3, dt, [C])
                    dx, _ = K.conv_forward([dpre0], packed(w0, dt, "dgrad", None, off, c, tiles=t_, deep=d_), None, N, H, W, mt=m_, deep=d_)
                    d_srcs.append(dx)
                else:
                    d_srcs.append(None)
                off += c
            if ctx.defer:
                DEFERRED.add(w0, b0, srcs, src_ch, dpre0, 3, N, H, W, gen=ctx.gen)
            elif ctx.wgrad:
                pg[0], pg[1] = _wgrad_now(w0, True, srcs, src_ch, dpre0, 3, N, H, W)
        return (None, None, None, *d_srcs, *pg)


def residual_chain(srcs: Sequence[torch.Tensor], conv0, blocks, r_scaling: float, recompute: bool = False, fp8: bool = False) -> torch.Tensor:
    params = [conv0.weight, conv0.bias]
    for b in blocks:
        params += [b.conv1.weight, b.conv1.bias, b.conv2.weight, b.conv2.bias]
    ok = all(isinstance(p, torch.nn.Parameter) for p in params) and all(t.is_contiguous() and t.shape[-1] % 8 == 0 for t in srcs)
    if not ok:
        raise HipError("residual_chain needs contiguous sources with multiples of 8 channels and nn.Parameter weights")
    return _ResidualChain.apply(float(r_scaling), -len(srcs) if recompute else len(srcs), bool(fp8 or FP8_CHAINS), *srcs, *params)


def linear(x: torch.Tensor, weight: torch.Tensor, bias: Optional[torch.Tensor], act: int = hip.ACT_NONE, alpha: float = 1.0,
           res: Optional[torch.Tensor] = None, slope: float = 0.0, fuse_src_act: bool = False) -> torch.Tensor:
    M = x.numel() // x.shape[-1]
    out = conv2d([x], weight, bias, 1, 1, M, ks=1, act=act, slope=slope, alpha=alpha,
                 res=None if res is None else res, fuse_src_act=fuse_src_act)
    y = out.reshape(*x.shape[:-1], weight.shape[0])
    tok = getattr(out, "_vmg_act_tok", None)
    if tok is not None and y is not out:
        y._vmg_act_tok = tok
    return y


def _ln_forward(ctx, x, w, b, eps, mode=None):
    x = x.contiguous()
    y, mean, rstd = K.layernorm_forward(x, w, b, eps) if mode is None else K.space_depth_ln_forward(x, mode, w, b, eps)
    ctx.mode = mode
    ctx.save_for_backward(x, mean, rstd, w)
    DEFERRED.claim(ctx, w, b)
    return y, x


def _ln_backward(ctx, dys, dskip=None):
    if not dys:
        DEFERRED.done(ctx)
        return dskip, None, None
    x, mean, rstd, w = ctx.saved_tensors
    if ctx.mode is None:
        dx, dw, db = K.layernorm_backward(dys, x, mean, rstd, w, into=DEFERRED.into(ctx), add=dskip)
    else:
        dx, dw, db = K.space_depth_ln_backward(dys[0], x, ctx.mode, mean, rstd, w, into=DEFERRED.into(ctx))
    DEFERRED.done(ctx)
    return (dx, None, None) if ctx.direct else (dx, dw, db)


class _LayerNorm(_Fn):

    @staticmethod
    def forward(ctx, x, w, b, eps):
        return _ln_forward(ctx, x, w, b, eps)[0]

    @staticmethod
    def backward(ctx, dy):
        return (*_ln_backward(ctx, [dy]), None)


class _SpaceDepthLayerNorm(_Fn):

    @staticmethod
    def forward(ctx, x, w, b, eps, mode):
        return _ln_forward(ctx, x, w, b, eps, mode)[0]

    @staticmethod
    def backward(ctx, dy):
        return (*_ln_backward(ctx, [dy]), None, None)


# ... 531 lines not shown


def spy_operand(ref: torch.Tensor, warped: torch.Tensor, up: torch.Tensor) -> torch.Tensor:
    return _SpyOperand.apply(ref, warped, up)


class _SpyFlowAdd(_Fn):
    @staticmethod
    def forward(ctx, up, res):
        ctx.dt = res.dtype
        return K.spy_flow_add(up.contiguous(), res.contiguous())

    @staticmethod
    def backward(ctx, g):
        return g, g.to(ctx.dt)


def spy_flow_add(up: torch.Tensor, res: torch.Tensor) -> torch.Tensor:
    return _SpyFlowAdd.apply(up, res)


class _SpyModule(_Fn):

    @staticmethod
    def forward(ctx, x8, *wb):
        ws, bs = wb[0::2], wb[1::2]
        dt = x8.dtype
        n, h, w, _ = x8.shape
        ctx.want_dx = ctx.needs_input_grad[0]
        ctx.want_w = [ctx.needs_input_grad[1 + 2 * i] for i in range(5)]
        ctx.want_b = [ctx.needs_input_grad[2 + 2 * i] for i in range(5)]
        keep = any(ctx.needs_input_grad)
        packs = [packed(wt, dt, "fwd", [wt.shape[1]]) for wt in ws]
        out, ys = K.spy_module_forward(x8.contiguous(), packs, bs, keep)
        ctx.geo = (n, h, w)
        if keep:
            ctx.defer = [DEFERRED.defers(ws[i], bs[i], ctx.want_w[i]) for i in range(5)]
            ctx.gen = [DEFERRED.note_use(ws[i], bs[i]) if ctx.defer[i] else 0 for i in range(5)]
            ctx.bias_ref = bs
            ctx.save_for_backward(x8, *ys, *ws)
        return out

    @staticmethod
    def backward(ctx, dy):
        n, h, w = ctx.geo
        saved = ctx.saved_tensors
        x8, ys, ws = saved[0], saved[1:5], saved[5:10]
        dpre4 = _pad_channels(dy.contiguous())
        pds = [packed(wt, dy.dtype, "dgrad", None, 0, wt.shape[1]) for wt in ws]
        dpre, dx = K.spy_module_backward(dpre4, pds, ys, ctx.want_dx)
        dpre_w = list(dpre) + [dpre4[..., :2]]
        grads = [None] * 10
        for i in range(4, -1, -1):
            srcs, src_ch = [x8 if i == 0 else ys[i - 1]], [ws[i].shape[1]]
            if ctx.defer[i]:
                DEFERRED.add(ws[i], ctx.bias_ref[i], srcs, src_ch, dpre_w[i], 7, n, h, w, gen=ctx.gen[i])
            elif ctx.want_w[i]:
                grads[2 * i], grads[2 * i + 1] = _wgrad_now(ws[i], ctx.want_b[i], srcs, src_ch, dpre_w[i], 7, n, h, w)
            elif ctx.want_b[i]:
                grads[2 * i + 1] = dpre_w[i].float().reshape(-1, ws[i].shape[0]).sum(0)
        return (dx, *grads)


def spy_module(x8: torch.Tensor, convs) -> torch.Tensor:
    wb = []
    for c in convs:
        wb += [c.weight, c.bias]
    return _SpyModule.apply(x8, *wb)


def identity_grid(n: int, h: int, w: int, device) -> torch.Tensor:
    ys, xs = torch.meshgrid(torch.arange(h, device=device), torch.arange(w, device=device), indexing="ij")
    return torch.stack([xs, ys], 0).float()[None].expand(n, -1, -1, -1).contiguous()


def _norm_grid(g, h, w):
    gx = 2.0 * g[..., 0] / max(w - 1, 1) - 1.0
    gy = 2.0 * g[..., 1] / max(h - 1, 1) - 1.0
    return torch.stack((gx, gy), -1)


class _WarpBilinear(_Fn):
    @staticmethod
    def forward(ctx, x, flow):
        x = x.contiguous()
        flow = flow.contiguous()
        ctx.save_for_backward(x, flow)
        return K.warp_bilinear_forward(x, flow)

    @staticmethod
    def backward(ctx, dy):
        x, flow = ctx.saved_tensors
        return K.warp_bilinear_backward(x, flow, dy)


def grid_sample_flow(x: torch.Tensor, flow: torch.Tensor, mode: str, padding: str) -> torch.Tensor:
    if mode != "bilinear" or padding != "border":
        raise HipError("the HIP flow warp implements bilinear / border (the only combination on the path)")
    return _WarpBilinear.apply(x, flow.float())


class _FlowSmooth(_Fn):
    @staticmethod
    def forward(ctx, flow, r):
        ctx.r = r
        return K.flow_smooth(flow.contiguous(), r)

    @staticmethod
    def backward(ctx, g):
        return K.flow_smooth(g.contiguous(), ctx.r, backward=True), None


def flow_smooth(flow: torch.Tensor, r: int) -> torch.Tensor:
    return _FlowSmooth.apply(flow.float(), int(r))


def warp_locations(loc: torch.Tensor, flow: torch.Tensor) -> torch.Tensor:
    return K.warp_nearest_planes(loc.detach(), flow.detach().contiguous())


class _FanOut(_Fn):
    @staticmethod
    def forward(ctx, x, k):
        ctx.set_materialize_grads(False)
        return tuple(x.view_as(x) for _ in range(k))

    @staticmethod
    def backward(ctx, *gs):
        gs = [g for g in gs if g is not None]
        if not gs:
            return None, None
        if len(gs) == 1:
            return gs[0], None
        g0 = gs[0]
        vn = 8 if g0.dtype == torch.bfloat16 else 4
        if len(gs) <= 4 and g0.dtype in (torch.bfloat16, torch.float32) and g0.numel() % vn == 0 and all(g.dtype == g0.dtype and g.shape == g0.shape for g in gs):
            return K.sum_n([g.contiguous() for g in gs]), None
        tot = gs[0]
        for g in gs[1:]:
            tot = tot + g
        return tot, None


def fan_out(x: torch.Tensor, k: int):
    if k == 1 or not (torch.is_grad_enabled() and x.requires_grad):
        return (x,) * k
    return _FanOut.apply(x, k)


class _GradBank:
    __slots__ = ("buf", "dtype")

    def __init__(self, dtype):
        self.buf = None
        self.dtype = dtype


class _Banked(_Fn):

    @staticmethod
    def forward(ctx, x, bank):
        ctx.bank = bank
        ctx.set_materialize_grads(False)
        return x.view_as(x)

    @staticmethod
    def backward(ctx, g):
        buf, ctx.bank.buf = ctx.bank.buf, None
        if buf is None:
            return g, None
        dt = ctx.bank.dtype
        if dt != torch.float32 and buf.numel() % 4 == 0 and (g is None or g.dtype == dt):
            out = K.cast_clear(buf, dt, add=g.contiguous() if g is not None else None)
            K.ACC_POOL.give(buf)
            return out, None
        if g is not None:
            buf.add_(g)
        return buf.to(dt), None


def grad_bank(x: torch.Tensor) -> torch.Tensor:
    if not (torch.is_grad_enabled() and x.requires_grad):
        return x
    bank = _GradBank(x.dtype)
    y = _Banked.apply(x, bank)
    y._vmg_bank = bank
    return y


LTAM_ARG_KEYFRAMES = 32


def ltam_route(t: int) -> str:
    return "args" if t <= LTAM_ARG_KEYFRAMES else "table"


class _LTAM(_Fn):
    @staticmethod
    def forward(ctx, q, loc, rpe, decay_v, cfg, *kv):
        heads, wh, ww, scale, banks = cfg
        t = len(kv) // 2
        keys = [x.contiguous() for x in kv[:t]]
        vals = [x.contiguous() for x in kv[t:]]
        q = q.contiguous()
        loc = loc.contiguous()
        rpe_c = rpe.detach().contiguous()
        fwd = K.ltam_forward if ltam_route(t) == "args" else K.ltam_forward_tab
        out, lse = fwd(q, keys, vals, loc, rpe_c, decay_v, heads, wh, ww, scale)
        ctx.cfg = cfg
        ctx.t = t
        ctx.direct = DEFERRED.direct(rpe) and rpe.dtype == torch.float32 and rpe.is_contiguous()
        if ctx.direct:
            ctx.rpe_param, ctx.gen = rpe, DEFERRED.note_params(rpe)
        ctx.save_for_backward(q, loc, rpe_c, decay_v, out, lse, *keys, *vals)
        return out

    @staticmethod
    def backward(ctx, dout):
        heads, wh, ww, scale, banks = ctx.cfg
        t = ctx.t
        q, loc, rpe, decay_v, out, lse = ctx.saved_tensors[:6]
        keys = list(ctx.saved_tensors[6:6 + t])
        vals = list(ctx.saved_tensors[6 + t:])
        into = []
        for i, b in enumerate(banks):
            if b is None or not ctx.needs_input_grad[5 + i]:
                into.append(None)
                continue
            if b.buf is None:
                b.buf = K.ACC_POOL.take(q.shape, q.device) if q.dtype != torch.float32 else torch.zeros_like(q, dtype=torch.float32)
            into.append(b.buf)
        bwd = K.ltam_backward if ltam_route(t) == "args" else K.ltam_backward_tab
        dq, dk, dv, drpe = bwd(q, keys, vals, loc, rpe, decay_v, out, lse, dout, heads, wh, ww, scale, dk_into=into[:t], dv_into=into[t:],
                               drpe_into=DEFERRED.grad_of(ctx.rpe_param) if ctx.direct else None)
        if ctx.direct:
            DEFERRED.written(ctx.gen, ctx.rpe_param)
            drpe = None
        gkv = [None if into[i] is not None else (g if g.dtype == q.dtype else g.to(q.dtype)) for i, g in enumerate(dk + dv)]
        return (dq, None, drpe, None, None, *gkv)


def ltam_attention(q, keys, vals, loc, rpe, decay_v, heads: int, wh: int, ww: int, scale: float):
    banks = tuple(getattr(x, "_vmg_bank", None) for x in list(keys) + list(vals))
    return _LTAM.apply(q, loc, rpe, decay_v, (heads, wh, ww, float(scale), banks), *keys, *vals)


class _LTAMMax(_Fn):
    @staticmethod
    def forward(ctx, q, loc, cfg, *kv):
        heads, banks = cfg
        t = len(kv) // 2
        keys = [x.contiguous() for x in kv[:t]]
        vals = [x.contiguous() for x in kv[t:]]
        q = q.contiguous()
        loc = loc.contiguous()
        fwd = K.ltam_max_forward if ltam_route(t) == "args" else K.ltam_max_forward_tab
        out, idx, _ = fwd(q, keys, vals, loc, heads)
        ctx.cfg = cfg
        ctx.t = t
        ctx.save_for_backward(q, loc, idx, *keys, *vals)
        return out

    @staticmethod
    def backward(ctx, dout):
        heads, banks = ctx.cfg
        t = ctx.t
        q, loc, idx = ctx.saved_tensors[:3]
        keys = list(ctx.saved_tensors[3:3 + t])
        vals = list(ctx.saved_tensors[3 + t:])
        into = []
        for i, b in enumerate(banks):
            if b is None or not ctx.needs_input_grad[3 + i]:
                into.append(None)
                continue
            if b.buf is None:
                b.buf = K.ACC_POOL.take(q.shape, q.device) if q.dtype != torch.float32 else torch.zeros_like(q, dtype=torch.float32)
            into.append(b.buf)
        bwd = K.ltam_max_backward if ltam_route(t) == "args" else K.ltam_max_backward_tab
        dq, dk, dv = bwd(q, keys, vals, loc, idx, dout, heads, dk_into=into[:t], dv_into=into[t:])
        gkv = [None if into[i] is not None else (g if g.dtype == q.dtype else g.to(q.dtype)) for i, g in enumerate(dk + dv)]
        return (dq, None, None, *gkv)


def ltam_max_attention(q, keys, vals, loc, heads: int):
    banks = tuple(getattr(x, "_vmg_bank", None) for x in list(keys) + list(vals))
    return _LTAMMax.apply(q, loc, (heads, banks), *keys, *vals)


class _Win3dAttention(_Fn):

    @staticmethod
    def forward(ctx, q, kv, bq, bkv, table, heads, wt, shift):
        q, kv = q.contiguous(), kv.contiguous()
        tab = table.detach().contiguous()
        out, lse = K.win3d_attn_forward(q, kv, bq, bkv, tab, heads, wt, shift)
        ctx.cfg = (heads, wt, shift)
        ctx.save_for_backward(q, kv, bq, bkv, tab, out, lse)
        ctx.direct = bq is not None and bkv is not None and DEFERRED.direct(bq, bkv)
        if ctx.direct:
            ctx.params, ctx.gen = (bq, bkv), DEFERRED.note_extra(bq, bkv)
        return out

    @staticmethod
    def backward(ctx, dout):
        q, kv, bq, bkv, tab, out, lse = ctx.saved_tensors
        heads, wt, shift = ctx.cfg
        if ctx.direct:
            into = tuple(DEFERRED.grad_of(p) for p in ctx.params)
            dq, dkv, dtable, _, _ = K.win3d_attn_backward(q, kv, bq, bkv, tab, out, lse, dout, heads, wt, shift, into=into)
            DEFERRED.extra_written(ctx.gen, *ctx.params)
            return dq, dkv, None, None, dtable, None, None, None
        dq, dkv, dtable, dbq, dbkv = K.win3d_attn_backward(q, kv, bq, bkv, tab, out, lse, dout, heads, wt, shift)
        return dq, dkv, dbq, dbkv, dtable, None, None, None


def win3d_attention(q: torch.Tensor, kv: torch.Tensor, bq, bkv, table: torch.Tensor, heads: int, wt: int, shift) -> torch.Tensor:
    return _Win3dAttention.apply(q, kv, bq, bkv, table, int(heads), int(wt), tuple(int(v) for v in shift))
```

vmg_amd/hip.py:

```python
from __future__ import annotations

import ctypes
import os
from ctypes import POINTER, c_char_p, c_float, c_int, c_int64, c_void_p

import torch

HERE = os.path.dirname(os.path.abspath(__file__))
LIB_PATH = os.environ.get("VMG_HIP_LIB") or os.path.join(HERE, "libvmg_hip.so")

F32, BF16 = 0, 1
ACT_NONE, ACT_RELU, ACT_LRELU, ACT_GELU = 0, 1, 2, 3
CONV_GENERAL, CONV_KSPLIT, CONV_WS, CONV_LINEAR_WRES, CONV_WSTAT = 0, 2, 3, 4, 6
CONV_FAM_IGEMM, CONV_FAM_KSPLIT, CONV_FAM_WS, CONV_FAM_LINEAR_WRES, CONV_FAM_WSTAT = 1, 2, 3, 4, 5
CONV_PLAN_INTS = 11
WGRAD_V1, WGRAD_3, WGRAD_3B, WGRAD_L2, WGRAD_7 = 1, 2, 3, 4, 5


def wgrad_kernel_id(kind: int, a: int = 0, b: int = 0, c: int = 0) -> int:
    return kind << 24 | a << 16 | b << 8 | c


class HipError(RuntimeError):
    pass


class ConvDesc(ctypes.Structure):
    _fields_ = [
        ("dtype", c_int), ("ks", c_int), ("cout_tiles", c_int),
        ("N", c_int), ("H", c_int), ("W", c_int), ("Cout", c_int),
        ("nsrc", c_int),
        ("src", c_void_p * 4), ("src_ps", c_int64 * 4), ("src_ch", c_int * 4),
        ("packed", c_void_p), ("bias", c_void_p),
        ("out", c_void_p), ("out_ps", c_int64), ("out_pre", c_void_p),
        ("res", c_void_p), ("res_ps", c_int64),
        ("aux", c_void_p), ("aux_ps", c_int64),
        ("act", c_int), ("slope", c_float), ("alpha", c_float),
        ("actgrad", c_int), ("pixel_shuffle", c_int), ("mt", c_int), ("deep", c_int),
    ]


class ChainDesc(ctypes.Structure):
    _fields_ = [
        ("dtype", c_int), ("N", c_int), ("H", c_int), ("W", c_int), ("C", c_int), ("nblk", c_int), ("nsrc", c_int),
        ("src", c_void_p * 4), ("src_ps", c_int64 * 4), ("src_ch", c_int * 4),
        ("packed0", c_void_p), ("bias0", c_void_p), ("slope0", c_float), ("cout_tiles0", c_int), ("deep0", c_int),
        ("packed1", POINTER(c_void_p)), ("bias1", POINTER(c_void_p)), ("packed2", POINTER(c_void_p)), ("bias2", POINTER(c_void_p)),
        ("r_scaling", c_float), ("cout_tiles", c_int), ("deep", c_int),
        ("y", POINTER(c_void_p)), ("t", POINTER(c_void_p)), ("g_y", POINTER(c_void_p)), ("g_t", POINTER(c_void_p)),
    ]


class SpyModuleDesc(ctypes.Structure):
    _fields_ = [
        ("N", c_int), ("H", c_int), ("W", c_int),
        ("x", c_void_p), ("packed", c_void_p * 5), ("bias", c_void_p * 5), ("y", c_void_p * 4), ("out", c_void_p), ("dpre", c_void_p * 4),
    ]


class ConvQ8Desc(ctypes.Structure):
    _fields_ = [
        ("N", c_int), ("H", c_int), ("W", c_int), ("Cin", c_int), ("Cout", c_int),
        ("src", c_void_p), ("packed", c_void_p), ("bias", c_void_p),
        ("out", c_void_p), ("out_ps", c_int64), ("outq", c_void_p),
        ("res", c_void_p), ("res_ps", c_int64),
        ("act", c_int), ("slope", c_float), ("alpha", c_float),
    ]


class ChainQ8Desc(ctypes.Structure):
    _fields_ = [
        ("N", c_int), ("H", c_int), ("W", c_int), ("C", c_int), ("nblk", c_int),
        ("q0", c_void_p), ("qa", c_void_p), ("qb", c_void_p),
        ("packed1", POINTER(c_void_p)), ("bias1", POINTER(c_void_p)), ("packed2", POINTER(c_void_p)), ("bias2", POINTER(c_void_p)),
        ("y", POINTER(c_void_p)), ("t", POINTER(c_void_p)), ("r_scaling", c_float),
    ]


_lib = None

SIGNATURES = {
    "vmg_last_error": (c_char_p, []),
    "vmg_version": (c_int, []),
    "vmg_max_lds_bytes": (c_int, []),
    "vmg_conv_pack_bytes": (c_int64, [c_int, c_int, c_int, c_int, POINTER(c_int), c_int]),
    "vmg_conv_pack": (c_int, [c_int, c_void_p, c_int, c_int, c_int, c_int, c_int, c_int, POINTER(c_int), POINTER(c_int),
                              c_int, c_int, c_void_p, c_void_p]),
    "vmg_convws_pack_bytes": (c_int64, [c_int, c_int, POINTER(c_int), c_int]),
    "vmg_convws_pack": (c_int, [c_void_p, c_int, c_int, c_int, c_int, c_int, POINTER(c_int), POINTER(c_int), c_int, c_int, c_void_p, c_void_p]),
    "vmg_conv_fwd": (c_int, [POINTER(ConvDesc), c_void_p]),
    "vmg_conv_fwd_plan": (c_int, [POINTER(ConvDesc), c_int, POINTER(c_int)]),
    "vmg_resblock_chain_fwd": (c_int, [POINTER(ChainDesc), c_void_p]),
    "vmg_resblock_chain_bwd": (c_int, [POINTER(ChainDesc), c_void_p]),
    "vmg_act_bwd": (c_int, [c_int, c_void_p, c_void_p, c_void_p, c_int64, c_int, c_float, c_float, c_void_p]),
    "vmg_pixel_shuffle": (c_int, [c_int, c_void_p, c_void_p, c_int, c_int, c_int, c_int, c_int, c_void_p]),
    "vmg_sum_n": (c_int, [c_int, c_void_p, c_int, c_void_p, c_int64, c_void_p]),
    "vmg_cast_clear": (c_int, [c_int, c_void_p, c_void_p, c_void_p, c_int64, c_void_p]),
    "vmg_pair_steps": (c_int, [c_int, c_int, c_void_p, c_void_p, c_void_p, c_int, c_int, c_int64, c_void_p]),
    "vmg_frame_gather": (c_int, [c_int, c_void_p, c_void_p, c_void_p, c_int64, c_int, c_int, c_int, c_void_p]),
    "vmg_pixel_unshuffle_actgrad": (c_int, [c_int, c_void_p, c_void_p, c_void_p, c_int, c_int, c_int, c_int, c_int, c_float, c_float, c_void_p]),
    "vmg_layernorm_fwd": (c_int, [c_int, c_void_p, c_void_p, c_void_p, c_void_p, c_void_p, c_void_p, c_int64, c_int, c_float, c_void_p]),
    "vmg_layernorm_bwd_ws_bytes": (c_int64, []),
    "vmg_layernorm_bwd": (c_int, [c_int, c_int, POINTER(c_void_p), c_void_p, c_void_p, c_void_p, c_void_p, c_void_p, c_void_p, c_void_p, c_void_p, c_int64, c_int,
                                  c_void_p, c_void_p]),
    "vmg_morphfc_fwd": (c_int, [c_int, c_int, c_void_p, c_void_p, c_void_p, c_void_p, c_void_p, c_void_p, c_int, c_int, c_int, c_int, c_int, c_int, c_int, c_float, c_float,
                                c_void_p]),
    "vmg_morphfc_token_rows": (c_int64, [c_int, c_int, c_int, c_int, c_int]),
    "vmg_morph_token_rows": (c_int64, [c_int, c_int, c_int, c_int, c_int]),
    "vmg_morph_tokens_gather": (c_int, [c_int, c_int, c_int, c_void_p, c_void_p, c_int, c_int, c_int, c_int, c_int, c_int, c_void_p]),
    "vmg_morph_tokens_scatter": (c_int, [c_int, c_int, c_int, c_void_p, c_void_p, c_int, c_int, c_int, c_int, c_int, c_int, c_void_p]),
    "vmg_win3d_attn_fwd": (c_int, [c_int, c_void_p, c_void_p, c_void_p, c_void_p, c_void_p, c_void_p, c_void_p, c_int, c_int, c_int, c_int, c_int, c_int, c_int,
                                   c_int, c_int, c_int, c_void_p]),
    "vmg_win3d_attn_bwd": (c_int, [c_int, c_void_p, c_void_p, c_void_p, c_void_p, c_void_p, c_void_p, c_void_p, c_void_p, c_void_p, c_void_p, c_void_p, c_void_p,
                                   c_void_p, c_void_p, c_int, c_int, c_int, c_int, c_int, c_int, c_int, c_int, c_int, c_int, c_void_p]),
    "vmg_win3d_attn_bwd_ws_bytes": (c_int64, [c_int, c_int, c_int, c_int, c_int, c_int]),
    "vmg_conv_wgrad3_multi": (c_int, [c_int, c_int, c_void_p, c_void_p, c_int, c_int, c_int, c_int64, c_int, c_int64, c_int, c_void_p, c_int, c_int, c_int,
                                      c_void_p, c_void_p, c_void_p, c_int64, c_void_p]),
    "vmg_conv_wgrad3_variant": (c_int, [c_int]),
    "vmg_conv_wgrad_last_kernel": (c_int, []),
    "vmg_conv_wgrad_plan": (c_int, [c_int, c_int, c_int, c_int, c_int, c_int, c_int, c_int, c_int64, c_int, c_int64, c_int, c_int, c_int, c_int, c_int, c_int64,
                                    POINTER(c_int)]),
    "vmg_win3d_variant": (c_int, [c_int]),
    "vmg_linear_wgrad2_multi": (c_int, [c_int, c_int, c_void_p, c_void_p, c_int64, c_int64, c_int, c_int64, c_int, c_void_p, c_int, c_int, c_int,
                                        c_void_p, c_void_p, c_void_p, c_int64, c_void_p]),
    "vmg_replay_build": (c_void_p, [c_void_p, c_void_p, c_void_p]),
    "vmg_replay_kernel_info": (c_int, [c_void_p, c_int, c_void_p, c_void_p, c_void_p, c_void_p]),
    "vmg_replay_run": (c_int, [c_void_p, c_int, c_int, c_void_p]),
    "vmg_replay_destroy": (None, [c_void_p]),
    "vmg_pack_entry_bytes": (c_int, []),
    "vmg_pack_entry": (c_int, [c_void_p, c_int, c_int, c_void_p, c_int, c_int, c_int, c_int, c_int, c_int, c_void_p, c_void_p, c_int, c_int, c_void_p,
                               c_int]),
    "vmg_pack_run": (c_int, [c_void_p, c_int, c_int, c_void_p]),
    "vmg_group_reduce3": (c_int, [c_int, c_void_p, c_void_p, c_void_p, c_void_p, c_void_p, c_int, c_int64, c_int, ctypes.c_float, c_void_p, c_int64, c_void_p]),
    "vmg_group_reduce_ws_bytes": (c_int64, []),
    "vmg_se_mlp_fwd": (c_int, [c_void_p] * 7 + [c_int] * 6 + [c_void_p]),
    "vmg_se_mlp_bwd": (c_int, [c_void_p] * 12 + [c_int] * 6 + [ctypes.c_float, c_int, c_void_p]),
    "vmg_maxpool_fwd": (c_int, [c_int, c_void_p, c_void_p, c_void_p, c_int, c_int, c_int, c_int, c_int, c_void_p]),
    "vmg_maxpool_bwd": (c_int, [c_int, c_void_p, c_void_p, c_void_p, c_int, c_int, c_int, c_int, c_int, c_void_p]),
    "vmg_avgpool2_nhwc": (c_int, [c_int, c_void_p, c_void_p, c_int, c_int, c_int, c_int, c_void_p]),
    "vmg_upsample2x_ac_fwd": (c_int, [c_void_p, c_void_p, c_int, c_int, c_int, c_int, c_float, c_void_p]),
    "vmg_upsample2x_ac_bwd": (c_int, [c_void_p, c_void_p, c_int, c_int, c_int, c_int, c_float, c_void_p]),
    "vmg_spy_operand_fwd": (c_int, [c_int, c_void_p, c_void_p, c_void_p, c_void_p, c_int64, c_void_p]),
    "vmg_spy_operand_bwd": (c_int, [c_int, c_void_p, c_void_p, c_void_p, c_int64, c_void_p]),
    "vmg_spy_flow_add": (c_int, [c_int, c_void_p, c_void_p, c_void_p, c_int64, c_void_p]),
    "vmg_spy_prep": (c_int, [c_int, c_void_p, c_void_p, c_void_p, c_void_p, c_int64, c_int, c_int, c_void_p]),
    "vmg_spy_module_fwd": (c_int, [POINTER(SpyModuleDesc), c_void_p]),
    "vmg_spy_module_bwd": (c_int, [POINTER(SpyModuleDesc), c_void_p]),
    "vmg_space_depth_ln_fwd": (c_int, [c_int, c_int, c_void_p, c_void_p, c_void_p, c_void_p, c_void_p, c_void_p, c_int, c_int, c_int, c_int, c_float, c_void_p]),
    "vmg_space_depth_ln_bwd": (c_int, [c_int, c_int, c_void_p, c_void_p, c_void_p, c_void_p, c_void_p, c_void_p, c_void_p, c_void_p, c_int, c_int, c_int, c_int,
                                       c_void_p, c_void_p]),
    "vmg_conv_wgrad_batched": (c_int, [c_int, c_int, c_int, POINTER(c_void_p), POINTER(c_void_p), c_int, c_int, c_int, c_int64, c_int,
                                       c_int64, c_int, c_void_p, c_int, c_int, c_int, c_void_p, c_float, c_void_p]),
    "vmg_warp_bilinear_fwd": (c_int, [c_int, c_void_p, c_void_p, c_void_p, c_int, c_int, c_int, c_int, c_void_p]),
    "vmg_warp_bilinear_bwd": (c_int, [c_int, c_void_p, c_void_p, c_void_p, c_void_p, c_void_p, c_int, c_int, c_int, c_int, c_void_p]),
    "vmg_warp_nearest_planes": (c_int, [c_void_p, c_void_p, c_void_p, c_int, c_int, c_int, c_int, c_void_p]),
    "vmg_flow_smooth": (c_int, [c_void_p, c_void_p, c_int64, c_int, c_int, c_int, c_int, c_void_p]),
    "vmg_ltam_fwd": (c_int, [c_int, c_void_p, POINTER(c_void_p), POINTER(c_void_p), c_void_p, c_void_p, c_void_p, c_void_p, c_void_p,
                             c_int, c_int, c_int, c_int, c_int, c_int, c_int, c_int, c_float, c_void_p]),
    "vmg_ltam_bwd": (c_int, [c_int, c_void_p, POINTER(c_void_p), POINTER(c_void_p), c_void_p, c_void_p, c_void_p, c_void_p, c_void_p,
                             c_void_p, c_void_p, POINTER(c_void_p), POINTER(c_void_p), c_void_p, c_int, c_int, c_int, c_int, c_int,
                             c_int, c_int, c_int, c_float, c_void_p]),
    "vmg_ltam_tab_bytes": (c_int64, [c_int]),
    "vmg_ltam_fwd_tab": (c_int, [c_int, c_void_p, POINTER(c_void_p), POINTER(c_void_p), c_void_p, c_void_p, c_void_p, c_void_p, c_void_p,
                                 c_int, c_int, c_int, c_int, c_int, c_int, c_int, c_int, c_float, c_void_p, c_int64, c_void_p]),
    "vmg_ltam_bwd_tab": (c_int, [c_int, c_void_p, POINTER(c_void_p), POINTER(c_void_p), c_void_p, c_void_p, c_void_p, c_void_p, c_void_p,
                                 c_void_p, c_void_p, POINTER(c_void_p), POINTER(c_void_p), c_void_p, c_int, c_int, c_int, c_int, c_int,
                                 c_int, c_int, c_int, c_float, c_void_p, c_int64, c_void_p]),
    "vmg_ltam_max_fwd": (c_int, [c_int, c_void_p, POINTER(c_void_p), POINTER(c_void_p), c_void_p, c_void_p, c_void_p, c_void_p,
                                 c_int, c_int, c_int, c_int, c_int, c_int, c_void_p]),
    "vmg_ltam_max_bwd": (c_int, [c_int, c_void_p, POINTER(c_void_p), POINTER(c_void_p), c_void_p, c_void_p, c_void_p, c_void_p,
                                 POINTER(c_void_p), POINTER(c_void_p), c_int, c_int, c_int, c_int, c_int, c_int, c_void_p]),
    "vmg_ltam_max_fwd_tab": (c_int, [c_int, c_void_p, POINTER(c_void_p), POINTER(c_void_p), c_void_p, c_void_p, c_void_p, c_void_p,
                                     c_int, c_int, c_int, c_int, c_int, c_int, c_void_p, c_int64, c_void_p]),
    "vmg_ltam_max_bwd_tab": (c_int, [c_int, c_void_p, POINTER(c_void_p), POINTER(c_void_p), c_void_p, c_void_p, c_void_p, c_void_p,
                                     POINTER(c_void_p), POINTER(c_void_p), c_int, c_int, c_int, c_int, c_int, c_int, c_void_p, c_int64,
                                     c_void_p]),
    "vmg_charbonnier_edge_blocks": (c_int, [c_int64, c_int, c_int]),
    "vmg_charbonnier_edge_fwd": (c_int, [c_void_p, c_void_p, c_void_p, c_void_p, c_void_p, c_int64, c_int, c_int, c_float, c_void_p]),
    "vmg_charbonnier_edge_bwd": (c_int, [c_void_p, c_void_p, c_void_p, c_void_p, c_void_p, c_int64, c_int, c_int, c_float, c_float, c_float, c_void_p]),
    "vmg_adamw_flat": (c_int, [c_void_p, c_void_p, c_void_p, c_void_p, c_int64, c_void_p, c_float, c_float, c_float, c_void_p]),
    "vmg_q8_record_bytes": (c_int, [c_int]),
    "vmg_q8_quantize": (c_int, [c_void_p, c_int64, c_void_p, c_int64, c_int, c_void_p]),
    "vmg_convq8_pack_bytes": (c_int64, [c_int, c_int]),
    "vmg_convq8_pack": (c_int, [c_void_p, c_int, c_int, c_int, c_void_p, c_void_p]),
    "vmg_convq8_fwd": (c_int, [POINTER(ConvQ8Desc), c_void_p]),
    "vmg_resblock_chain_fwd_q8": (c_int, [POINTER(ChainQ8Desc), c_void_p]),
    "vmg_grad_clip_ws_bytes": (c_int64, []),
    "vmg_grad_clip_norm": (c_int, [c_void_p, c_int64, c_float, c_void_p, c_void_p, c_void_p]),
    "vmg_grad_pack_bf16": (c_int, [c_void_p, c_void_p, c_int64, c_float, c_void_p]),
    "vmg_grad_unpack_bf16": (c_int, [c_void_p, c_void_p, c_int64, c_void_p]),
    "vmg_tile_accumulate": (c_int, [c_int, c_void_p, c_void_p, c_void_p, c_int64, c_int, c_int, c_int, c_int, c_int, c_int, c_int, c_int, c_int,
                                    c_int, c_void_p]),
    "vmg_tile_finalize": (c_int, [c_void_p, c_void_p, c_void_p, c_void_p, c_int64, c_void_p]),
    "vmg_frame_metrics_ws_bytes": (c_int64, [c_int, c_int, c_int]),
    "vmg_frame_metrics": (c_int, [c_void_p, POINTER(c_int64), c_void_p, POINTER(c_int64), c_int, c_int, c_int, POINTER(ctypes.c_double), c_void_p, c_int64,
                                  c_void_p, c_void_p, c_void_p]),
    "vmg_bicubic_down": (c_int, [c_void_p, POINTER(c_int64), c_int, c_int, c_int, c_int, c_int, c_void_p, c_void_p]),
    "vmg_crop_batch": (c_int, [c_void_p, POINTER(c_int64), c_void_p, c_int, c_int, c_int, c_int, c_int, c_int, c_int, c_void_p, c_void_p]),
    "vmg_decay_weights": (c_int, [POINTER(c_void_p), POINTER(c_void_p), POINTER(c_int64), c_int, c_int, c_void_p]),
    "vmg_conv_debug_stamps": (c_int, [c_void_p]),
    "vmg_create": (c_void_p, [c_int]),
    "vmg_destroy": (c_int, [c_void_p]),
    "vmg_ctx_device": (c_int, [c_void_p]),
    "vmg_prof_select_pixels": (c_int, [c_void_p, c_int64]),
    "vmg_prof_null_interval_us": (ctypes.c_double, [c_int, c_void_p]),
    "vmg_conv_wgrad_ws_bytes": (c_int64, []),
    "vmg_conv_wgrad_batched_ws": (c_int, [c_int, c_int, c_int, POINTER(c_void_p), POINTER(c_void_p), c_int, c_int, c_int, c_int64, c_int,
                                          c_int64, c_int, c_void_p, c_int, c_int, c_int, c_void_p, c_float, c_void_p, c_int64, c_void_p]),
    "vmg_group_reduce": (c_int, [c_int, c_void_p, c_void_p, c_void_p, c_void_p, c_int, c_int64, c_int, c_int, c_float, c_void_p, c_int64, c_void_p]),
    "vmg_tab_elementwise": (c_int, [c_int, c_int, c_void_p, c_void_p, c_void_p, c_void_p, c_void_p, c_float, c_void_p, c_void_p, c_void_p,
                                    c_int64, c_int64, c_int, c_void_p]),
    "vmg_prof_begin": (c_int, [c_void_p, c_int, c_int, c_int]),
    "vmg_prof_end": (c_int, [c_void_p, POINTER(c_int64), POINTER(c_int), POINTER(ctypes.c_double)]),
    "vmg_conv_wgrad": (c_int, [c_int, c_int, c_int, c_int, c_int, c_void_p, c_int64, c_int, c_void_p, c_int64, c_int,
                               c_void_p, c_int, c_int, c_int, c_void_p, c_float, c_void_p]),
    "vmg_frame_sqerr_ws_bytes": (c_int64, [c_int, c_int, c_int, c_int]),
    "vmg_frame_sqerr": (c_int, [c_int, c_void_p, c_int64, c_int, c_void_p, c_int64, c_int, c_int, c_int, c_int, c_void_p, c_int64, c_void_p, c_void_p]),
    "vmg_best_window_select": (c_int, [c_int, c_void_p, c_int64, c_void_p, c_int, c_int64, c_int, c_int, c_int, c_float, c_void_p, c_void_p, c_void_p,
                                       c_void_p, c_void_p, c_void_p, c_int, c_void_p]),
    "vmg_convert_frames": (c_int, [c_int, c_void_p, POINTER(c_int64), c_int, c_void_p, POINTER(c_int64), c_int, c_int, c_int, c_int, c_void_p]),
}


def lib() -> ctypes.CDLL:
    global _lib
    if _lib is None:
        if not os.path.exists(LIB_PATH):
            raise HipError(f"{LIB_PATH} is missing: the VMG hot path has no fallback. Run `python -m vmg_amd.build`.")
        l = ctypes.CDLL(LIB_PATH)
        for name, (res, args) in SIGNATURES.items():
            fn = getattr(l, name)
            fn.restype = res
            fn.argtypes = args
        _lib = l
    return _lib


# ... 50 lines not shown
```

vmg_amd/kernels.py:

```python
from __future__ import annotations

import collections
import ctypes
import os
import struct
from typing import Optional, Sequence, Tuple

import torch

from . import hip
from .hip import ConvDesc, HipError


def _intarr(v: Sequence[int]):
    return (ctypes.c_int * len(v))(*[int(x) for x in v])


def cout_tiles_for(cout: int, dtype: torch.dtype = torch.bfloat16, ks: int = 3) -> int:
    t = (cout + 15) // 16
    if t <= 1:
        return 1
    if ks == 7:
        return 2 if t == 2 else 4
    if t <= 4:
# ... 135 lines not shown
    if len(srcs) != len(pw.src_ch):
        raise HipError(f"conv expects {len(pw.src_ch)} sources, got {len(srcs)}")
    x0 = srcs[0]
    hip.require_cuda(*srcs, bias, res, aux, out)
    dt = x0.dtype
    if dt != pw.dtype:
        raise HipError(f"activation dtype {dt} != packed weight dtype {pw.dtype}")
    M = N * H * W
    nsrc = len(srcs)
    if (pw.layout == "ws") != (deep == hip.CONV_WS):
        deep = hip.CONV_WS if pw.layout == "ws" else hip.CONV_GENERAL
    sp, sps, sch = [0, 0, 0, 0], [0, 0, 0, 0], [0, 0, 0, 0]
    for i, s in enumerate(srcs):
        if s.dtype != dt or s.shape[-1] != pw.src_ch[i] or s.numel() // s.shape[-1] != M:
            raise HipError(f"source {i}: shape {tuple(s.shape)} / dtype {s.dtype} does not match conv (M={M}, C={pw.src_ch[i]}, {dt})")
        sp[i], sps[i], sch[i] = s.data_ptr(), _pix_stride(s), pw.src_ch[i]
    bias_p = 0
    if bias is not None:
        if bias.dtype != torch.float32 or bias.numel() != pw.cout or not bias.is_contiguous():
            raise HipError("bias must be contiguous fp32 of length Cout")
        bias_p = bias.data_ptr()
    if pixel_shuffle:
        oshape = (N, 2 * H, 2 * W, pw.cout // 4)
    else:
        oshape = (N, H, W, pw.cout)
    if out is None:
        out = torch.empty(oshape, dtype=dt, device=x0.device)
    elif out.dtype != dt or out.numel() // out.shape[-1] != (4 * M if pixel_shuffle else M) or out.shape[-1] != oshape[-1]:
        raise HipError(f"bad output tensor {tuple(out.shape)} for conv output {oshape}")
    out_ps = _pix_stride(out)
    if want_pre and out_pre is None:
        if pixel_shuffle:
            raise HipError("out_pre is not available with pixel_shuffle")
        out_pre = torch.empty(oshape, dtype=dt, device=x0.device)
    pre_p = 0
    if out_pre is not None:
        if _pix_stride(out_pre) != out_ps or out_pre.shape[-1] != pw.cout or out_pre.dtype != dt:
            raise HipError("out_pre must have the layout of out")
        pre_p = out_pre.data_ptr()
    extra = [0, 0, 0, 0]
    for k, (name, t) in enumerate((("res", res), ("aux", aux))):
        if t is None:
            continue
        if pixel_shuffle:
            raise HipError(f"{name} is not supported together with pixel_shuffle")
        if t.dtype != dt or t.shape[-1] != pw.cout or t.numel() // t.shape[-1] != M:
            raise HipError(f"{name}: shape {tuple(t.shape)} does not match conv output")
        extra[2 * k], extra[2 * k + 1] = t.data_ptr(), _pix_stride(t)
    d = _CONV_DESC
    _CONV_PACK(d, 0, hip.dtype_code(dt), pw.ks, pw.cout_tiles, N, H, W, pw.cout, nsrc, sp[0], sp[1], sp[2], sp[3], sps[0], sps[1], sps[2], sps[3],
               sch[0], sch[1], sch[2], sch[3], pw.buf.data_ptr(), bias_p, out.data_ptr(), out_ps, pre_p, extra[0], extra[1], extra[2], extra[3],
               act, slope, alpha, actgrad, int(pixel_shuffle), mt, deep)
    return d, out, out_pre


def conv_forward(srcs: Sequence[torch.Tensor], pw: PackedConv, bias: Optional[torch.Tensor], N: int, H: int, W: int,
                 act: int = hip.ACT_NONE, slope: float = 0.0, alpha: float = 1.0, res: Optional[torch.Tensor] = None,
                 aux: Optional[torch.Tensor] = None, actgrad: int = 0, pixel_shuffle: bool = False,
                 out: Optional[torch.Tensor] = None, out_pre: Optional[torch.Tensor] = None, want_pre: bool = False,
                 mt: int = 0, deep: int = hip.CONV_GENERAL) -> Tuple[torch.Tensor, Optional[torch.Tensor]]:
    d, out, out_pre = _conv_fill(srcs, pw, bias, N, H, W, act, slope, alpha, res, aux, actgrad, pixel_shuffle, out, out_pre, want_pre, mt, deep)
    hip.check(hip.lib().vmg_conv_fwd(ctypes.byref(d), hip.stream_ptr()), "vmg_conv_fwd")
    return out, out_pre


ConvPlan = collections.namedtuple("ConvPlan", "family dtype ks mt ntb variant vec8 grid_x grid_y tiles_per_wave lds_bytes")


def conv_forward_plan(srcs: Sequence[torch.Tensor], pw: PackedConv, bias: Optional[torch.Tensor], N: int, H: int, W: int,
                      act: int = hip.ACT_NONE, slope: float = 0.0, alpha: float = 1.0, res: Optional[torch.Tensor] = None,
                      aux: Optional[torch.Tensor] = None, actgrad: int = 0, pixel_shuffle: bool = False,
                      out: Optional[torch.Tensor] = None, out_pre: Optional[torch.Tensor] = None, want_pre: bool = False,
                      mt: int = 0, deep: int = hip.CONV_GENERAL, ncu: int = 0) -> ConvPlan:
    d, _, _ = _conv_fill(srcs, pw, bias, N, H, W, act, slope, alpha, res, aux, actgrad, pixel_shuffle, out, out_pre, want_pre, mt, deep)
    plan = (ctypes.c_int * hip.CONV_PLAN_INTS)()
    hip.check(hip.lib().vmg_conv_fwd_plan(ctypes.byref(d), ncu, plan), "vmg_conv_fwd_plan")
    return ConvPlan(*plan)


def _parr(ts):
    return (ctypes.c_void_p * max(1, len(ts)))(*[(t.data_ptr() if t is not None else None) for t in ts])


CHAIN_STATS = {"fwd": {}, "bwd": {}}


def resblock_chain_forward(srcs: Sequence[torch.Tensor], pw0: PackedConv, b0: torch.Tensor, slope0: float, deep0: int, pw1: Sequence[PackedConv],
                           b1: Sequence[torch.Tensor], pw2: Sequence[PackedConv], b2: Sequence[torch.Tensor], r_scaling: float, deep: int,
                           own_output: bool = False):
    x0 = srcs[0]
    hip.require_cuda(*srcs, b0, *b1, *b2)
    N, H, W = x0.shape[0], x0.shape[1], x0.shape[2]
    M = N * H * W
    C, nblk, dt = pw0.cout, len(pw1), x0.dtype
    if len(srcs) != len(pw0.src_ch) or any(s.dtype != dt or s.shape[-1] != c or s.numel() // s.shape[-1] != M for s, c in zip(srcs, pw0.src_ch)):
        raise HipError("resblock_chain: sources do not match conv0's pack")
    if any(p.cout != C or p.src_ch != [C] or p.dtype != dt or p.layout != pw1[0].layout or p.cout_tiles != pw1[0].cout_tiles for p in list(pw1) + list(pw2)) or \
            pw0.dtype != dt or len(pw2) != nblk or len(b1) != nblk or len(b2) != nblk:
        raise HipError("resblock_chain: block packs must be C -> C packs of one layout")
    for b in [b0] + list(b1) + list(b2):
        if b.dtype != torch.float32 or b.numel() != C or not b.is_contiguous():
            raise HipError("resblock_chain: biases must be contiguous fp32 of length C")
    blk = torch.empty((2 * nblk + 1, N, H, W, C), dtype=dt, device=x0.device).unbind(0)
    ys, ts = list(blk[:nblk + 1]), list(blk[nblk + 1:])
    if own_output:
        ys[-1] = torch.empty((N, H, W, C), dtype=dt, device=x0.device)
    d = hip.ChainDesc()
    d.dtype, d.N, d.H, d.W, d.C, d.nblk, d.nsrc = hip.dtype_code(dt), N, H, W, C, nblk, len(srcs)
    for i, s in enumerate(srcs):
        d.src[i], d.src_ps[i], d.src_ch[i] = s.data_ptr(), _pix_stride(s), pw0.src_ch[i]
    d.packed0, d.bias0, d.slope0 = pw0.buf.data_ptr(), b0.data_ptr(), slope0
    d.cout_tiles0, d.deep0 = pw0.cout_tiles, hip.CONV_WS if pw0.layout == "ws" else deep0
    keep = [_parr([p.buf for p in pw1]), _parr(list(b1)), _parr([p.buf for p in pw2]), _parr(list(b2)), _parr(ys), _parr(ts)]
    d.packed1, d.bias1, d.packed2, d.bias2, d.y, d.t = keep
    d.r_scaling = r_scaling
    d.cout_tiles = pw1[0].cout_tiles if nblk else pw0.cout_tiles
    d.deep = (hip.CONV_WS if pw1[0].layout == "ws" else deep) if nblk else hip.CONV_GENERAL
    hip.check(hip.lib().vmg_resblock_chain_fwd(ctypes.byref(d), hip.stream_ptr()), "vmg_resblock_chain_fwd")
    CHAIN_STATS["fwd"][d.deep] = CHAIN_STATS["fwd"].get(d.deep, 0) + 1
    return ys, ts


def resblock_chain_backward(g: torch.Tensor, ts: Sequence[torch.Tensor], pd1: Sequence[PackedConv], pd2: Sequence[PackedConv], r_scaling: float,
                            deep: int):
    hip.require_cuda(g, *ts)
    nblk = len(ts)
    N, H, W, C = g.shape
    g = g.contiguous()
    if nblk == 0:
        return [g], []
    blk = torch.empty((2 * nblk, N, H, W, C), dtype=g.dtype, device=g.device).unbind(0)
    gys, gts = list(blk[:nblk]) + [g], list(blk[nblk:])
    d = hip.ChainDesc()
    d.dtype, d.N, d.H, d.W, d.C, d.nblk, d.nsrc = hip.dtype_code(g.dtype), N, H, W, C, nblk, 1
    keep = [_parr([p.buf for p in pd1]), _parr([p.buf for p in pd2]), _parr(list(ts)), _parr(gys), _parr(gts)]
    d.packed1, d.packed2, d.t, d.g_y, d.g_t = keep
    d.r_scaling = r_scaling
    d.cout_tiles = pd1[0].cout_tiles
    d.deep = hip.CONV_WS if pd1[0].layout == "ws" else deep
    hip.check(hip.lib().vmg_resblock_chain_bwd(ctypes.byref(d), hip.stream_ptr()), "vmg_resblock_chain_bwd")
    CHAIN_STATS["bwd"][d.deep] = CHAIN_STATS["bwd"].get(d.deep, 0) + 1
    return gys, gts


def _wgrad_operands(name: str, xs, dys, dW: torch.Tensor, db: Optional[torch.Tensor], ks: int, M: int, o0: int = 0, i0: int = 0, like=None,
                    whole: bool = False):
    hip.require_cuda(dW, db, *xs, *dys)
    if dW.dtype != torch.float32 or not dW.is_contiguous() or (db is not None and (db.dtype != torch.float32 or not db.is_contiguous())):
        raise HipError(f"{name}: parameter gradients must be contiguous fp32")
    x0, d0 = like or (xs[0], dys[0])
    Cin, Cout = x0.shape[-1], d0.shape[-1]
    xps, dps = _pix_stride(x0), _pix_stride(d0)
    for x, d in zip(xs, dys):
        if x.dtype != x0.dtype or d.dtype != x0.dtype or x.shape[-1] != Cin or d.shape[-1] != Cout or x.numel() // Cin != M or \
                d.numel() // Cout != M or _pix_stride(x) != xps or _pix_stride(d) != dps:
            raise HipError(f"{name}: all pairs must share dtype, shape and strides and cover the N*H*W pixels")
    O_total, I_total = dW.shape[0], dW.shape[1]
    kk = 1 if dW.dim() == 2 else dW.shape[2]
    fits = kk == ks and o0 + Cout <= O_total and i0 + Cin <= I_total and (db is None or db.numel() == O_total)
    if whole:
        fits = fits and O_total == Cout and (dW.dim() == 4 if ks == 3 else (I_total == Cin and dW.numel() == Cout * Cin))
    if not fits:
        raise HipError(f"{name}: gradient tensor {tuple(dW.shape)} does not match conv (ks={ks}, Cout={Cout}+{o0}, Cin={Cin}+{i0})")
    return Cin, Cout, xps, dps, I_total


def conv_wgrad(x: torch.Tensor, dy: torch.Tensor, dW: torch.Tensor, db: Optional[torch.Tensor], ks: int, N: int, H: int,
               W: int, scale: float = 1.0, o0: int = 0, i0: int = 0):
    Cin, Cout, xps, dps, I_total = _wgrad_operands("conv_wgrad", [x], [dy], dW, db, ks, N * H * W, o0, i0)
    hip.check(hip.lib().vmg_conv_wgrad(hip.dtype_code(x.dtype), ks, N, H, W, x.data_ptr(), xps, Cin, dy.data_ptr(), dps, Cout, dW.data_ptr(), I_total, o0, i0,
                                       db.data_ptr() if db is not None else None, scale, hip.stream_ptr()), "vmg_conv_wgrad")


def act_backward(dy: torch.Tensor, ref: torch.Tensor, act: int, slope: float, alpha: float) -> torch.Tensor:
    hip.require_cuda(dy, ref)
    if dy.shape != ref.shape or dy.dtype != ref.dtype or not dy.is_contiguous() or not ref.is_contiguous():
        raise HipError("act_backward: dy / ref must be contiguous tensors of one shape and dtype")
    out = torch.empty_like(dy)
    hip.check(hip.lib().vmg_act_bwd(hip.dtype_code(dy.dtype), dy.data_ptr(), ref.data_ptr(), out.data_ptr(), dy.numel(), act, slope,
                                    alpha, hip.stream_ptr()), "vmg_act_bwd")
    return out


def pixel_shuffle(x: torch.Tensor, N: int, H: int, W: int) -> torch.Tensor:
    hip.require_cuda(x)
    c4 = x.shape[-1]
    if c4 % 4 or x.numel() != N * H * W * c4 or not x.is_contiguous():
        raise HipError("pixel_shuffle: bad input")
    out = torch.empty((N, 2 * H, 2 * W, c4 // 4), dtype=x.dtype, device=x.device)
    hip.check(hip.lib().vmg_pixel_shuffle(hip.dtype_code(x.dtype), x.data_ptr(), out.data_ptr(), N, H, W, c4 // 4, 0, hip.stream_ptr()),
              "vmg_pixel_shuffle")
    return out


def frame_gather(src: torch.Tensor, idx: torch.Tensor, n_dst: int, frame_shape) -> torch.Tensor:
    hip.require_cuda(src, idx)
    fe = 1
    for d in frame_shape:
        fe *= int(d)
    if not src.is_contiguous() or src.numel() % fe or idx.dtype != torch.int32 or idx.dim() != 2 or idx.shape[0] != n_dst or idx.shape[1] not in (1, 2) or not idx.is_contiguous():
        raise HipError("frame_gather: contiguous src of whole frames and a contiguous int32 (n_dst, 1|2) index table expected")
    dst = torch.empty((n_dst, *frame_shape), dtype=src.dtype, device=src.device)
    hip.check(hip.lib().vmg_frame_gather(hip.dtype_code(src.dtype), src.data_ptr(), dst.data_ptr(), idx.data_ptr(), fe, src.numel() // fe, n_dst, idx.shape[1],
                                         hip.stream_ptr()), "vmg_frame_gather")
    return dst


def sum_n(ts: Sequence[torch.Tensor]) -> torch.Tensor:
    hip.require_cuda(*ts)
    t0 = ts[0]
    vn = 8 if t0.dtype == torch.bfloat16 else 4
    if not 2 <= len(ts) <= 4 or t0.numel() % vn or any(t.shape != t0.shape or t.dtype != t0.dtype or not t.is_contiguous() for t in ts):
        raise HipError("sum_n: 2..4 contiguous tensors of one shape and dtype, whole 16-byte vectors")
    out = torch.empty_like(t0)
    ptrs = (ctypes.c_void_p * len(ts))(*[t.data_ptr() for t in ts])
    hip.check(hip.lib().vmg_sum_n(hip.dtype_code(t0.dtype), ptrs, len(ts), out.data_ptr(), t0.numel(), hip.stream_ptr()), "vmg_sum_n")
    return out


class DecayList:

    def __init__(self, weights: Sequence[torch.Tensor], gammas: Sequence[torch.Tensor]):
        if not weights or len(weights) != len(gammas):
            raise HipError("decay_weights: two non-empty lists of equal length expected")
# ... 441 lines not shown
    return dx, dw, db


def conv_wgrad_batched(xs: Sequence[torch.Tensor], dys: Sequence[torch.Tensor], dW: torch.Tensor, db: Optional[torch.Tensor], ks: int,
                       N: int, H: int, W: int, scale: float = 1.0, o0: int = 0, i0: int = 0):
    if len(xs) != len(dys) or not xs:
        raise HipError("conv_wgrad_batched: need equally many x and dy tensors")
    Cin, Cout, xps, dps, I_total = _wgrad_operands("conv_wgrad_batched", xs, dys, dW, db, ks, N * H * W, o0, i0)
    code = hip.dtype_code(xs[0].dtype)
    l = hip.lib()
    ws = _workspace("vmg_conv_wgrad_ws_bytes", dW.device)
    for s in range(0, len(xs), 16):
        n = min(16, len(xs) - s)
        xa = (ctypes.c_void_p * n)(*[t.data_ptr() for t in xs[s:s + n]])
        da = (ctypes.c_void_p * n)(*[t.data_ptr() for t in dys[s:s + n]])
        hip.check(l.vmg_conv_wgrad_batched_ws(code, ks, n, xa, da, N, H, W, xps, Cin, dps, Cout, dW.data_ptr(), I_total, o0, i0,
                                              db.data_ptr() if db is not None else None, scale, ws.data_ptr(), ws.numel(),
                                              hip.stream_ptr()), "vmg_conv_wgrad_batched_ws")


def conv_wgrad3_multi_ok(x: torch.Tensor, dy: torch.Tensor, ks: int) -> bool:
    if ks not in (1, 3) or x.dtype != torch.bfloat16 or dy.dtype != torch.bfloat16 or x.data_ptr() % 16 or dy.data_ptr() % 16:
        return False
    try:
        strides = ((_pix_stride(x), x.shape[-1]), (_pix_stride(dy), dy.shape[-1]))
    except HipError:
        return False
    if ks == 1:
        return all(ps % 8 == 0 and c % 8 == 0 for ps, c in strides) and x.numel() // x.shape[-1] >= 2048
    return all(ps % 8 == 0 and ps >= (c + 7) // 8 * 8 for ps, c in strides)


WGRAD_MULTI_PAIRS = 16


def _wgrad_multi(name: str, probs, dims: Sequence[int]):
    conv3 = len(dims) == 3
    M = dims[0] * dims[1] * dims[2] if conv3 else dims[0]
    xs0, dys0, dW0 = probs[0][:3]
    npairs = len(xs0)
    for xs, dys, dW, db, _ in probs:
        if len(xs) != npairs or len(dys) != npairs or dW.shape != dW0.shape or xs[0].dtype != torch.bfloat16:
            raise HipError(f"{name}: problems must share the shape; operands bf16")
        Cin, Cout, xps, dps, I_total = _wgrad_operands(name, xs, dys, dW, db, 3 if conv3 else 1, M, like=(xs0[0], dys0[0]), whole=True)
    entry = getattr(hip.lib(), "vmg_" + name)
    ws = _workspace("vmg_conv_wgrad_ws_bytes", dW0.device)
    for s in range(0, len(probs), 8):
        grp = probs[s:s + 8]
        n = len(grp)
        wa = (ctypes.c_void_p * n)(*[g[2].data_ptr() for g in grp])
        ba = (ctypes.c_void_p * n)(*[(g[3].data_ptr() if g[3] is not None else None) for g in grp])
        sa = (ctypes.c_float * n)(*[float(g[4]) for g in grp])
        for p0 in range(0, npairs, WGRAD_MULTI_PAIRS):
            p1 = min(npairs, p0 + WGRAD_MULTI_PAIRS)
            xa = (ctypes.c_void_p * (n * (p1 - p0)))(*[t.data_ptr() for g in grp for t in g[0][p0:p1]])
            da = (ctypes.c_void_p * (n * (p1 - p0)))(*[t.data_ptr() for g in grp for t in g[1][p0:p1]])
            hip.check(entry(n, p1 - p0, xa, da, *dims, xps, Cin, dps, Cout, wa, I_total, 0, 0, ba, sa, ws.data_ptr(), ws.numel(), hip.stream_ptr()),
                      "vmg_" + name)


def linear_wgrad2_multi(probs, M: int):
    _wgrad_multi("linear_wgrad2_multi", probs, (M,))


def conv_wgrad3_multi(probs, N: int, H: int, W: int):
    _wgrad_multi("conv_wgrad3_multi", probs, (N, H, W))


def _ptrs(ts):
    return (ctypes.c_void_p * len(ts))(*[t.data_ptr() for t in ts])


def warp_bilinear_forward(x: torch.Tensor, flow: torch.Tensor) -> torch.Tensor:
    hip.require_cuda(x, flow)
    n, h, w, c = x.shape
    if not x.is_contiguous() or flow.dtype != torch.float32 or not flow.is_contiguous() or tuple(flow.shape) != (n, h, w, 2):
        raise HipError("warp: x must be contiguous (n,h,w,c), flow contiguous fp32 (n,h,w,2)")
    out = torch.empty_like(x)
    hip.check(hip.lib().vmg_warp_bilinear_fwd(hip.dtype_code(x.dtype), x.data_ptr(), flow.data_ptr(), out.data_ptr(), n, h, w, c,
                                              hip.stream_ptr()), "vmg_warp_bilinear_fwd")
    return out


def warp_bilinear_backward(x: torch.Tensor, flow: torch.Tensor, dy: torch.Tensor):
    hip.require_cuda(x, flow, dy)
    n, h, w, c = x.shape
    if not x.is_contiguous() or flow.dtype != torch.float32 or not flow.is_contiguous() or tuple(flow.shape) != (n, h, w, 2):
        raise HipError("warp: x must be contiguous (n,h,w,c), flow contiguous fp32 (n,h,w,2)")
    if dy.dtype != x.dtype or tuple(dy.shape) != (n, h, w, c):
        raise HipError(f"warp_bilinear_backward: dy must have x's shape and dtype, got {tuple(dy.shape)} {dy.dtype}")
    dy = dy.contiguous()
    pooled = x.dtype != torch.float32 and (n * h * w * c) % 4 == 0
    dx_acc = ACC_POOL.take((n, h, w, c), x.device) if pooled else torch.zeros((n, h, w, c), dtype=torch.float32, device=x.device)
    dflow = torch.empty((n, h, w, 2), dtype=torch.float32, device=x.device)
    hip.check(hip.lib().vmg_warp_bilinear_bwd(hip.dtype_code(x.dtype), x.data_ptr(), flow.data_ptr(), dy.data_ptr(), dx_acc.data_ptr(),
                                              dflow.data_ptr(), n, h, w, c, hip.stream_ptr()), "vmg_warp_bilinear_bwd")
    if pooled:
        dx = cast_clear(dx_acc, x.dtype)
        ACC_POOL.give(dx_acc)
        return dx, dflow
    return dx_acc.to(x.dtype), dflow


def flow_smooth(x: torch.Tensor, r: int, backward: bool = False) -> torch.Tensor:
    hip.require_cuda(x)
    if x.dtype != torch.float32 or not x.is_contiguous() or x.dim() < 2:
        raise HipError("flow_smooth: contiguous fp32 (..., H, W) expected")
    H, W = x.shape[-2:]
    out = torch.empty_like(x)
    hip.check(hip.lib().vmg_flow_smooth(x.data_ptr(), out.data_ptr(), x.numel() // (H * W), H, W, int(r), 1 if backward else 0, hip.stream_ptr()), "vmg_flow_smooth")
    return out


def warp_nearest_planes(loc: torch.Tensor, flow: torch.Tensor) -> torch.Tensor:
    hip.require_cuda(loc, flow)
    n, k2, h, w = loc.shape
    if loc.dtype != torch.float32 or flow.dtype != torch.float32 or not flow.is_contiguous() or tuple(flow.shape) != (n, h, w, 2):
        raise HipError("warp_nearest_planes: fp32 loc (n,k2,h,w) and flow (n,h,w,2) expected")
    loc = loc.contiguous()
    out = torch.empty_like(loc)
    hip.check(hip.lib().vmg_warp_nearest_planes(loc.data_ptr(), flow.data_ptr(), out.data_ptr(), n, k2, h, w, hip.stream_ptr()),
              "vmg_warp_nearest_planes")
    return out


def _ltam_check_tables(rpe, decay, heads, wh, ww):
    wq = wh * ww
    if rpe.dtype != torch.float32 or decay.dtype != torch.float32 or not rpe.is_contiguous():
        raise HipError("ltam: rpe / decay must be fp32")
    if tuple(rpe.shape) != (heads, wq, wq):
        raise HipError(f"ltam: rpe must be (heads, wh*ww, wh*ww) = {(heads, wq, wq)}, got {tuple(rpe.shape)}")
    if decay.numel() != heads or not decay.is_contiguous():
        raise HipError(f"ltam: decay must hold {heads} contiguous values, got {tuple(decay.shape)}")


class LtamTables:

    def __init__(self):
        self.bufs = {}
        self.retired = []

    def get(self, t: int, device) -> torch.Tensor:
        need = hip.lib().vmg_ltam_tab_bytes(t)
        key = (device.index if device.index is not None else torch.cuda.current_device(), hip.stream_ptr())
        buf = self.bufs.get(key)
        if buf is None or buf.numel() < need:
            if buf is not None:
                self.retired.append(buf)
            buf = self.bufs[key] = torch.empty(max(need, 4096), dtype=torch.uint8, device=device)
        return buf

    def clear(self):
        self.bufs.clear()
        self.retired.clear()


LTAM_TABLES = LtamTables()


def _ltam_forward(tab, q, keys, vals, loc, rpe, decay, heads, wh, ww, scale):
    hip.require_cuda(q, loc, rpe, decay, *keys, *vals)
    n, h, w, c = q.shape
    t = len(keys)
    ts = [q] + list(keys) + list(vals)
    if any(x.dtype != q.dtype or tuple(x.shape) != (n, h, w, c) or not x.is_contiguous() for x in ts):
        raise HipError("ltam: q / keys / vals must be contiguous (n,h,w,c) tensors of one dtype")
    if loc.dtype != torch.float32 or tuple(loc.shape) != (n, 2 * t, h, w) or not loc.is_contiguous():
        raise HipError(f"ltam: loc must be contiguous fp32 (n,2t,h,w), got {tuple(loc.shape)}")
    _ltam_check_tables(rpe, decay, heads, wh, ww)
    out = torch.empty_like(q)
    lse = torch.empty((n, h, w, heads), dtype=torch.float32, device=q.device)
    if tab:
        if t < 1:
            raise HipError("ltam_forward_tab: at least one key-frame")
        ws = LTAM_TABLES.get(t, q.device)
        hip.check(hip.lib().vmg_ltam_fwd_tab(hip.dtype_code(q.dtype), q.data_ptr(), _ptrs(keys), _ptrs(vals), loc.data_ptr(), rpe.data_ptr(),
                                             decay.data_ptr(), out.data_ptr(), lse.data_ptr(), n, h, w, c, heads, wh, ww, t, scale,
                                             ws.data_ptr(), ws.numel(), hip.stream_ptr()), "vmg_ltam_fwd_tab")
        return out, lse
    hip.check(hip.lib().vmg_ltam_fwd(hip.dtype_code(q.dtype), q.data_ptr(), _ptrs(keys), _ptrs(vals), loc.data_ptr(), rpe.data_ptr(),
                                     decay.data_ptr(), out.data_ptr(), lse.data_ptr(), n, h, w, c, heads, wh, ww, t, scale,
                                     hip.stream_ptr()), "vmg_ltam_fwd")
    return out, lse

# ... 569 lines not shown
```

vmg_amd/model.py:

```python
from __future__ import annotations

import os
from fractions import Fraction
from typing import List, Sequence

import numpy as np
import torch
import torch.nn as nn
import torch.nn.functional as F

from . import functional as FH
from . import hip
from .hip import ACT_GELU, ACT_LRELU, ACT_RELU, HipError


def conv(mod: nn.Conv2d, srcs: Sequence[torch.Tensor], N: int, H: int, W: int, **kw) -> torch.Tensor:
    return FH.conv2d(srcs, mod.weight, mod.bias, N, H, W, ks=mod.kernel_size[0], **kw)


def lin(mod: nn.Linear, x: torch.Tensor, **kw) -> torch.Tensor:
    return FH.linear(x, mod.weight, mod.bias, **kw)


def lnorm(mod: nn.LayerNorm, x: torch.Tensor) -> torch.Tensor:
# ... 264 lines not shown
class ResidualBlocksWithInputConv(nn.Module):

    def __init__(self, in_channels, out_channels, num_blocks, r_scaling):
        super().__init__()
        self.main = nn.Sequential(nn.Conv2d(in_channels, out_channels, 3, 1, 1), nn.LeakyReLU(0.1),
                                  nn.Sequential(*[ResidualBlockNoBN0(out_channels, r_scaling) for _ in range(num_blocks)]))
        self.recompute = False
        self.fp8 = False

    def forward(self, srcs: Sequence[torch.Tensor]):
        blocks = list(self.main[2])
        r = blocks[0].res_scale if blocks else 1.0
        return FH.residual_chain([t.contiguous() for t in srcs], self.main[0], blocks, r, recompute=self.recompute and torch.is_grad_enabled(), fp8=self.fp8)


class LTAM_multi_head(nn.Module):

    def __init__(self, embed_dim, head, if_scale, twins, mode="wins"):
        super().__init__()
        if mode not in ("wins", "max"):
            raise NotImplementedError(f"LTAM_multi_head: mode 'wins' or 'max', got {mode!r}")
        self.mode = mode
        self.head = head
        self.proj = nn.Linear(embed_dim, embed_dim)
        if mode == "max":
            self.scale = 1.0
            return
        self.scale = (embed_dim // head) ** -0.5 if if_scale else 1.0
        self.win_h, self.win_w = twins
        self.relative_pos_encoding = nn.Parameter(torch.zeros(head, self.win_h * self.win_w, self.win_h * self.win_w))
        nn.init.trunc_normal_(self.relative_pos_encoding, std=.02)
        self.register_buffer("decay_v", 1 - 2 ** (-5 - torch.arange(head - 1, -1, -1, dtype=torch.float32)))

    def forward(self, q, keys, anchor, vals, loc):
        if self.mode == "max":
            att = FH.ltam_max_attention(q, keys, vals, loc, self.head)
        else:
            att = FH.ltam_attention(q, keys, vals, loc, self.relative_pos_encoding, self.decay_v, self.head, self.win_h, self.win_w,
                                    self.scale)
        return lin(self.proj, att, res=anchor)


class Trajectory_multi_head(nn.Module):

    def __init__(self, embed_dim, num_blocks, frame_stride, head, head_scale, r_scaling, twins, mode="wins"):
        super().__init__()
        self.embed_dims = embed_dim
        self.keyframe_stride = frame_stride
        self.LTAM = LTAM_multi_head(embed_dim, head, head_scale, twins, mode)
        self.resblocks = ResidualBlocksWithInputConv(2 * embed_dim, embed_dim, num_blocks, r_scaling)
        self.fusion = nn.Conv2d(3 * embed_dim, embed_dim, 1, 1, 0)

    def forward(self, x, flows_forward, flows_backward):
        n, t, h, w, c = x.shape
        fb = flows_backward.permute(1, 0, 3, 4, 2).float()
        ff = flows_forward.permute(1, 0, 3, 4, 2).float()
        s = self.keyframe_stride
        x_steps, x = FH.fan_out(x, 2)
        curs = FH.pair_frame_steps(x_steps)
        flpair = torch.cat([fb.flip(0), ff], 1).contiguous() if t > 1 else None
        ident = FH.identity_grid(2 * n, h, w, x.device)
        loc = ident
        feat = None
        k_in: List[torch.Tensor] = []
        k_state: List[torch.Tensor] = []
        feats = []
        fls = flpair.unbind(0) if flpair is not None else ()
        for j in range(t):
            key, last = j % s == 0, j == t - 1
            hd = list(FH.fan_out(curs[j], (1 if j > 0 else 0) + 1 + (1 if key else 0)))
            cur_q = hd.pop() if j > 0 else None
            cur_c = hd.pop()
            cur_k = hd.pop() if key else None
            if j == 0:
                feat = torch.zeros_like(cur_c)
            else:
                fl = fls[j - 1]
                feat = flow_warp_nhwc(feat_next, fl, "bilinear", "border")
                loc = FH.warp_locations(loc, fl)
                feat = self.LTAM(cur_q, k_in, feat, k_state, loc)
                if key:
                    loc = torch.cat([loc, ident], 1)
            feat = self.resblocks([cur_c, feat])
            hd = list(FH.fan_out(feat, 1 + (0 if last else 1) + (1 if key else 0)))
            f_out = hd.pop()
            feat_next = None if last else hd.pop()
            if key:
                k_state.append(FH.grad_bank(hd.pop()))
                k_in.append(FH.grad_bank(cur_k))
            feats.append(f_out)
        back, fwd = FH.unpair_steps(feats, n)
        out = conv(self.fusion, [back, x, fwd], n * t, h, w, act=ACT_LRELU, slope=0.1)
        return out.reshape(n, t, h, w, c)


def _get_window_size(x_size, window_size, shift_size):
    ws, ss = list(window_size), list(shift_size)
    for i in range(3):
        if x_size[i] <= window_size[i]:
            ws[i] = x_size[i]
            ss[i] = 0
    return tuple(ws), tuple(ss)


def _relative_position_index(ws) -> torch.Tensor:
    coords = torch.stack(torch.meshgrid(torch.arange(ws[0]), torch.arange(ws[1]), torch.arange(ws[2]), indexing="ij"))
    cf = coords.flatten(1)
    rel = (cf[:, :, None] - cf[:, None, :]).permute(1, 2, 0).contiguous()
    rel[:, :, 0] += ws[0] - 1
    rel[:, :, 1] += ws[1] - 1
    rel[:, :, 2] += ws[2] - 1
    rel[:, :, 0] *= (2 * ws[1] - 1) * (2 * ws[2] - 1)
    rel[:, :, 1] *= 2 * ws[2] - 1
    return rel.sum(-1)


class rWindowAttention(nn.Module):

    def __init__(self, dim, window_size, num_heads, qkv_bias):
        super().__init__()
        self.dim, self.window_size, self.num_heads = dim, tuple(window_size), num_heads
        n_rel = (2 * window_size[0] - 1) * (2 * window_size[1] - 1) * (2 * window_size[2] - 1)
        self.relative_position_bias_table = nn.Parameter(torch.zeros(n_rel, num_heads))
        self.register_buffer("relative_position_index", _relative_position_index(window_size))
        self.q = nn.Linear(dim, dim, bias=qkv_bias)
        self.kv = nn.Linear(dim, 2 * dim, bias=qkv_bias)
        self.proj = nn.Linear(dim, dim)
        nn.init.trunc_normal_(self.relative_position_bias_table, std=0.02)

    def forward(self, y, shift):
        q = lin(self.q, y)
        kv = lin(self.kv, y)
        o = FH.win3d_attention(q, kv, self.q.bias, self.kv.bias, self.relative_position_bias_table, self.num_heads, self.window_size[0], shift)
        return o


class EncoderBlockOnOnetoken(nn.Module):
    def __init__(self, dim, num_heads, window_size, shift_size, mlp_ratio, qkv_bias):
        super().__init__()
        self.window_size, self.shift_size, self.num_heads = tuple(window_size), tuple(shift_size), num_heads
        self.norm1 = nn.LayerNorm(dim)
        self.attn = rWindowAttention(dim, window_size, num_heads, qkv_bias)
        self.norm2 = nn.LayerNorm(dim)
        self.mlp = Mlp(dim, int(dim * mlp_ratio))

    def forward(self, x):
        B, D, H, W, C = x.shape
        ws, ss = _get_window_size((D, H, W), self.window_size, self.shift_size)
        if tuple(ws) != (self.window_size[0], 8, 8):
            raise HipError(f"3-D window attention: the feature map {(D, H, W)} must be at least one (wt, 8, 8) window ({self.window_size})")
        y = lnorm(self.norm1, x)
        x = lin(self.attn.proj, self.attn(y, ss), res=x)
        z = lnorm(self.norm2, x)
        return lin(self.mlp.fc2, lin(self.mlp.fc1, z, act=ACT_GELU), res=x)


class DecoderLayer(nn.Module):

    def __init__(self, dim, depth, num_heads, window_size, mlp_ratio, qkv_bias):
        super().__init__()
        self.window_size = list(window_size)
        self.shift_size = [i // 2 for i in window_size]
        self.blocks = nn.ModuleList([EncoderBlockOnOnetoken(dim, num_heads, window_size, [0, 0, 0] if i % 2 == 0 else self.shift_size,
                                                            mlp_ratio, qkv_bias) for i in range(depth)])

    def forward(self, x):
        B, D, H, W, C = x.shape
        wt = self.window_size[0]
        seq_back = None
        if D % wt != 0:
            delta_t = int(np.ceil(D / wt)) * wt - D
            delta = list(range(-1, -(delta_t + 1), -1))
# ... 348 lines not shown
```

Baseline: 594.6 LR-frames/s.

## Fuse chain input act-grad, add quad warp backward, share state gradient accumulators

Three separate changes. The first leaky-ReLU backward of the resblock chain moves into the epilogue of the chain's first dgrad conv, applied after the residual add, which removes a separate elementwise pass. A new quad-based bilinear warp backward kernel handles bf16 with C=144 or 112: each wave processes a 2x2 pixel quad, merges duplicate corner atomics, and can accumulate dx directly into a grad-bank buffer. The model now shares one banked accumulator for f_out, feat_next and the key state instead of fanning out copies, which cuts gradient summation and casts at the cost of more indirection and atomics.

Result: no change. 596.5 LR-frames/s (median of 3 runs) (+0.3%).

```diff
diff --git a/include/vmg_hip.h b/include/vmg_hip.h
--- a/include/vmg_hip.h
+++ b/include/vmg_hip.h
@@ -14,6 +14,7 @@
 #define VMG_ACT_RELU 1
 #define VMG_ACT_LRELU 2
 #define VMG_ACT_GELU 3
+#define VMG_ACTGRAD_AFTER_RES 8
 
 #define VMG_CONV_GENERAL 0
 #define VMG_CONV_KSPLIT 2
@@ -173,6 +174,10 @@
 int vmg_warp_bilinear_fwd(int dtype, const void* x, const float* flow, void* out, int N, int H, int W, int C, void* stream);
 int vmg_warp_bilinear_bwd(int dtype, const void* x, const float* flow, const void* dy, void* dx_acc, float* dflow, int N, int H,
                           int W, int C, void* stream);
+#define VMG_WARP_BWD_PIXEL 1
+#define VMG_WARP_BWD_QUAD 2
+int vmg_warp_bwd_variant(int variant);
+int vmg_warp_bwd_last_kernel(void);
 int vmg_warp_nearest_planes(const float* loc, const float* flow, float* out, int N, int K2, int H, int W, void* stream);
 int vmg_flow_smooth(const float* in, float* out, int64_t planes, int H, int W, int r, int backward, void* stream);
 
diff --git a/vmg_amd/csrc/conv_igemm.hip b/vmg_amd/csrc/conv_igemm.hip
--- a/vmg_amd/csrc/conv_igemm.hip
+++ b/vmg_amd/csrc/conv_igemm.hip
@@ -38,6 +38,7 @@
   int act;
   float slope, alpha;
   int actgrad, ps;
+  int agpost;
   int nstages;
   int halo_bytes;
   int ring;
@@ -505,17 +506,19 @@
 #pragma unroll
       for (int r = 0; r < 8; ++r) v[r] = (v[r] > 0.f ? v[r] : v[r] * neg) * a.alpha;
     }
-    if (a.aux) {
+    auto actgrad = [&]() __attribute__((always_inline)) {
 #pragma unroll
       for (int r = 0; r < 8; ++r) {
         const float u = (float)pre_aux[it][r];
         v[r] *= a.actgrad == 3 ? gelu_erf_grad(u) : (u > 0.f ? 1.f : (a.actgrad == 2 ? a.slope : 0.f));
       }
-    }
+    };
+    if (a.aux && !a.agpost) actgrad();
     if (a.res) {
 #pragma unroll
       for (int r = 0; r < 8; ++r) v[r] += (float)pre_res[it][r];
     }
+    if (a.aux && a.agpost) actgrad();
     bf16x8 t;
 #pragma unroll
     for (int r = 0; r < 8; ++r) t[r] = (bf16)v[r];
@@ -948,19 +951,21 @@
 #pragma unroll
             for (int q = 0; q < 8; ++q) v[q] = (v[q] > 0.f ? v[q] : v[q] * neg) * a.alpha;
           }
-          if (aux) {
+          auto actgrad = [&]() __attribute__((always_inline)) {
             const bf16x8 au = *reinterpret_cast<const bf16x8*>(aux + pix * a.aux_ps + cov);
 #pragma unroll
             for (int q = 0; q < 8; ++q) {
               const float u = (float)au[q];
               v[q] *= a.actgrad == 3 ? gelu_erf_grad(u) : (u > 0.f ? 1.f : (a.actgrad == 2 ? a.slope : 0.f));
             }
-          }
+          };
+          if (aux && !a.agpost) actgrad();
           if (res) {
             const bf16x8 rv = *reinterpret_cast<const bf16x8*>(res + pix * a.res_ps + cov);
 #pragma unroll
             for (int q = 0; q < 8; ++q) v[q] += (float)rv[q];
           }
+          if (aux && a.agpost) actgrad();
           bf16x8 tq;
 #pragma unroll
           for (int q = 0; q < 8; ++q) tq[q] = (bf16)v[q];
@@ -1375,7 +1380,7 @@
 #pragma unroll
         for (int r = 0; r < 8; ++r) v[r] *= a.alpha;
       }
-      if (auxb) {
+      auto actgrad = [&]() __attribute__((always_inline)) {
         bf16x8 u = pre[it];
         if (a.res) u = *reinterpret_cast<const bf16x8*>(auxb + opix * (int)a.aux_ps + c8 * 8);
 #pragma unroll
@@ -1383,11 +1388,13 @@
           const float uf = (float)u[r];
           v[r] *= a.actgrad == 3 ? gelu_erf_grad(uf) : (uf > 0.f ? 1.f : (a.actgrad == 2 ? a.slope : 0.f));
         }
-      }
+      };
+      if (auxb && !a.agpost) actgrad();
       if (a.res) {
 #pragma unroll
         for (int r = 0; r < 8; ++r) v[r] += (float)pre[it][r];
       }
+      if (auxb && a.agpost) actgrad();
       bf16x8 tq;
 #pragma unroll
       for (int r = 0; r < 8; ++r) tq[r] = (bf16)v[r];
@@ -2053,7 +2060,7 @@
   k.res = (const char*)d->res; k.res_ps = d->res_ps; k.aux = (const char*)d->aux; k.aux_ps = d->aux_ps;
   k.N = d->N; k.H = d->H; k.W = d->W; k.Cout = d->Cout; k.M = M;
   k.tiles_x = cdiv(d->W, 16); k.tiles_y = cdiv(d->H, TH);
-  k.act = d->act; k.slope = d->slope; k.alpha = d->alpha; k.actgrad = d->aux ? d->actgrad : 0; k.ps = d->pixel_shuffle;
+  k.act = d->act; k.slope = d->slope; k.alpha = d->alpha; k.actgrad = d->aux ? (d->actgrad & 7) : 0; k.agpost = d->aux && d->res && (d->actgrad & VMG_ACTGRAD_AFTER_RES) ? 1 : 0; k.ps = d->pixel_shuffle;
 #ifdef VMG_DIAG
   {
     const char* e = getenv("VMG_CONV_DBG");
@@ -2120,6 +2127,7 @@
       long long waves = (long long)(wg_per_cu * c / ncb > 0 ? wg_per_cu * c / ncb : 1) * 4;
       long long tpw = cdiv64(ntiles, waves);
       if (tpw < 4) tpw = 4;
+      VMG_CHECK(!k.agpost, "conv_fwd: VMG_ACTGRAD_AFTER_RES is not implemented by the streamed 1x1 kernel");
       p.family = VMG_CONV_FAM_LINEAR_WRES; p.variant = ns; p.gx = (int)cdiv64(cdiv64(ntiles, tpw), 4); p.tpw = (int)tpw; p.lds = wres_lds_bytes(ntb, ns);
       return 0;
     }
@@ -2150,6 +2158,7 @@
     VMG_CHECK(p.lds <= 160 * 1024, "conv: LDS request %d B exceeds 160 KiB", p.lds);
     p.family = VMG_CONV_FAM_IGEMM;
   }
+  VMG_CHECK(!k.agpost || p.family == VMG_CONV_FAM_KSPLIT, "conv_fwd: VMG_ACTGRAD_AFTER_RES needs the k-split, weight-streaming or weights-stationary kernel");
   const long long nblk = (d->ks > 1) ? (long long)k.N * k.tiles_y * k.tiles_x : cdiv64(k.M, 64 * mt);
   VMG_CHECK(nblk > 0 && nblk < (1ll << 31), "conv: bad grid %lld", nblk);
   p.gx = (int)nblk;
@@ -2245,6 +2254,9 @@
     if (rc) return rc;
     chain_base(c, d);
     d.src[0] = c->g_t[k]; d.packed = c->packed1[k]; d.out = c->g_y[k]; d.res = c->g_y[k + 1]; d.res_ps = c->C;
+    if (k == 0 && c->y) {
+      d.aux = c->y[0]; d.aux_ps = c->C; d.actgrad = 2 | VMG_ACTGRAD_AFTER_RES; d.slope = c->slope0;
+    }
     if ((rc = vmg_conv_fwd(&d, stream))) return rc;
   }
   return 0;
diff --git a/vmg_amd/csrc/warp.hip b/vmg_amd/csrc/warp.hip
--- a/vmg_amd/csrc/warp.hip
+++ b/vmg_amd/csrc/warp.hip
@@ -1,4 +1,6 @@
 #include "common.h"
+#include <type_traits>
+#include <utility>
 
 namespace {
 
@@ -134,6 +136,124 @@
   }
 }
 
+__device__ __forceinline__ float uniform_f(float v) {
+  return __builtin_bit_cast(float, __builtin_amdgcn_readfirstlane(__builtin_bit_cast(int, v)));
+}
+
+template <int... Is, typename F>
+__device__ __forceinline__ void static_for_impl(std::integer_sequence<int, Is...>, F&& f) {
+  (f(std::integral_constant<int, Is>{}), ...);
+}
+template <int N, typename F>
+__device__ __forceinline__ void static_for(F&& f) {
+  static_for_impl(std::make_integer_sequence<int, N>{}, f);
+}
+#define WP_INL __attribute__((always_inline))
+
+template <int C>
+__global__ __launch_bounds__(256) void warp_bilinear_bwd_quad_kernel(const bf16* __restrict__ x, const float* __restrict__ flow,
+                                                                     const bf16* __restrict__ dy, float* __restrict__ dx_acc,
+                                                                     float* __restrict__ dflow, int N, int H, int W) {
+  constexpr int NB = (C + 63) / 64;
+  const int lane = threadIdx.x & 63;
+  const int wave = __builtin_amdgcn_readfirstlane(threadIdx.x >> 6);
+  const int qw = (W + 1) >> 1, qh = (H + 1) >> 1;
+  const long long nquad = (long long)N * qh * qw;
+  for (long long q = blockIdx.x * 4LL + wave; q < nquad; q += (long long)gridDim.x * 4) {
+    const int qx = (int)(q % qw), qy = (int)((q / qw) % qh);
+    const long long img = (q / ((long long)qw * qh)) * H * W;
+    int own[4], cidx[16];
+    float ixs[4], iys[4];
+    unsigned pvm = 0, cvm = 0;
+    float val[16][NB];
+    bf16 graw[4][NB], xraw[16][NB];
+    static_for<4>([&](auto ic) WP_INL {
+      constexpr int i = ic, e = 4 * i;
+      const int px = 2 * qx + (i & 1), py = 2 * qy + (i >> 1);
+      const bool pv = px < W && py < H;
+      own[i] = pv ? py * W + px : (2 * qy) * W + 2 * qx;
+      const long long pix = img + own[i];
+      const float ix = uniform_f(clip_border(unnorm_coord((float)px, flow[pix * 2], W), W, nullptr));
+      const float iy = uniform_f(clip_border(unnorm_coord((float)py, flow[pix * 2 + 1], H), H, nullptr));
+      ixs[i] = ix;
+      iys[i] = iy;
+      const int x0 = (int)floorf(ix), y0 = (int)floorf(iy), x1 = x0 + 1, y1 = y0 + 1;
+      const bool yin0 = y0 >= 0 && y0 < H, yin1 = y1 >= 0 && y1 < H, xin0 = x0 >= 0 && x0 < W, xin1 = x1 >= 0 && x1 < W;
+      const bool c0 = pv && yin0 && xin0, c1 = pv && yin0 && xin1, c2 = pv && yin1 && xin0, c3 = pv && yin1 && xin1;
+      pvm |= (pv ? 1u : 0u) << i;
+      cvm |= ((c0 ? 1u : 0u) | (c1 ? 2u : 0u) | (c2 ? 4u : 0u) | (c3 ? 8u : 0u)) << e;
+      cidx[e] = __builtin_amdgcn_readfirstlane(c0 ? y0 * W + x0 : own[i]);
+      cidx[e + 1] = __builtin_amdgcn_readfirstlane(c1 ? y0 * W + x1 : own[i]);
+      cidx[e + 2] = __builtin_amdgcn_readfirstlane(c2 ? y1 * W + x0 : own[i]);
+      cidx[e + 3] = __builtin_amdgcn_readfirstlane(c3 ? y1 * W + x1 : own[i]);
+      static_for<NB>([&](auto bc) WP_INL {
+        constexpr int b = bc;
+        const int ch = lane + 64 * b, cl = ch < C ? ch : 0;
+        graw[i][b] = dy[pix * C + cl];
+        static_for<4>([&](auto kc) WP_INL { xraw[e + kc][b] = x[(img + cidx[e + kc]) * C + cl]; });
+      });
+    });
+    pvm = __builtin_amdgcn_readfirstlane(pvm);
+    cvm = __builtin_amdgcn_readfirstlane(cvm);
+    unsigned livem = 0;
+    static_for<4>([&](auto ic) WP_INL {
+      constexpr int i = ic;
+      const float ix = ixs[i], iy = iys[i];
+      const float x0f = floorf(ix), y0f = floorf(iy), x1f = x0f + 1.f, y1f = y0f + 1.f;
+      const float tx = ix - x0f, ty = iy - y0f;
+      const float wgt[4] = {(x1f - ix) * (y1f - iy), (ix - x0f) * (y1f - iy), (x1f - ix) * (iy - y0f), (ix - x0f) * (iy - y0f)};
+      const float sx[4] = {-(1.f - ty), 1.f - ty, -ty, ty}, sy[4] = {-(1.f - tx), -tx, 1.f - tx, tx};
+      float g[NB], gix = 0.f, giy = 0.f;
+      static_for<NB>([&](auto bc) WP_INL { g[bc] = lane + 64 * bc < C ? (float)graw[i][bc] : 0.f; });
+      static_for<4>([&](auto kc) WP_INL {
+        constexpr int k = kc, e = 4 * i + k;
+        const bool cv = (cvm >> e) & 1u;
+        livem |= (cv && wgt[k] != 0.f ? 1u : 0u) << e;
+        float xv = 0.f;
+        static_for<NB>([&](auto bc) WP_INL {
+          val[e][bc] = g[bc] * wgt[k];
+          xv += (float)xraw[e][bc] * g[bc];
+        });
+        if (cv) {
+          gix += xv * sx[k];
+          giy += xv * sy[k];
+        }
+      });
+      gix = wave_sum(gix);
+      giy = wave_sum(giy);
+      if (lane == 0 && ((pvm >> i) & 1u)) {
+        const long long pix = img + own[i];
+        dflow[pix * 2] = (ix <= 0.f || ix >= (float)(W - 1)) ? 0.f : gix;
+        dflow[pix * 2 + 1] = (iy <= 0.f || iy >= (float)(H - 1)) ? 0.f : giy;
+      }
+    });
+    livem = __builtin_amdgcn_readfirstlane(livem);
+    static_for<16>([&](auto ic) WP_INL {
+      constexpr int i = ic;
+      static_for<i>([&](auto jc) WP_INL {
+        constexpr int j = jc;
+        if (((livem >> i) & 1u) && ((livem >> j) & 1u) && cidx[i] == cidx[j]) {
+          static_for<NB>([&](auto bc) WP_INL { val[j][bc] += val[i][bc]; });
+          livem &= ~(1u << i);
+        }
+      });
+    });
+    static_for<16>([&](auto ec) WP_INL {
+      constexpr int e = ec;
+      if ((livem >> e) & 1u) {
+        float* dst = dx_acc + (img + cidx[e]) * C;
+        static_for<NB>([&](auto bc) WP_INL {
+          if (lane + 64 * bc < C) atomicAdd(dst + lane + 64 * bc, val[e][bc]);
+        });
+      }
+    });
+  }
+}
+#undef WP_INL
+
+int g_warp_bwd_variant = 1;
+int g_warp_bwd_last_kernel = 0;
+
 __global__ __launch_bounds__(256) void warp_nearest_planes_kernel(const float* __restrict__ loc, const float* __restrict__ flow,
                                                                   float* __restrict__ out, int N, int K2, int H, int W) {
   const long long total = (long long)N * H * W;
@@ -224,6 +344,15 @@
   VMG_CHECK(((uintptr_t)x | (uintptr_t)dy | (uintptr_t)dx_acc) % 16 == 0, "warp_bwd: pointers must be 16-byte aligned");
   const long long total = (long long)N * H * W * 64;
   hipStream_t st = (hipStream_t)stream;
+  if (dtype == VMG_BF16 && g_warp_bwd_variant == 1 && (C == 144 || C == 112) && (long long)H * W < (1ll << 30)) {
+    const long long qtotal = (long long)N * ((H + 1) / 2) * ((W + 1) / 2) * 64;
+    if (C == 144) hipLaunchKernelGGL(warp_bilinear_bwd_quad_kernel<144>, dim3(grid_for(qtotal)), dim3(256), 0, st, (const bf16*)x, flow, (const bf16*)dy, (float*)dx_acc, dflow, N, H, W);
+    else hipLaunchKernelGGL(warp_bilinear_bwd_quad_kernel<112>, dim3(grid_for(qtotal)), dim3(256), 0, st, (const bf16*)x, flow, (const bf16*)dy, (float*)dx_acc, dflow, N, H, W);
+    g_warp_bwd_last_kernel = VMG_WARP_BWD_QUAD;
+    VMG_LAUNCH_CHECK();
+    return 0;
+  }
+  g_warp_bwd_last_kernel = VMG_WARP_BWD_PIXEL;
   if (dtype == VMG_BF16) {
     hipLaunchKernelGGL(warp_bilinear_bwd_kernel<bf16>, dim3(grid_for(total)), dim3(256), 0, st, (const bf16*)x, flow, (const bf16*)dy, (float*)dx_acc, dflow, N, H, W, C);
   } else {
@@ -232,6 +361,14 @@
   VMG_LAUNCH_CHECK();
   return 0;
 }
+
+extern "C" int vmg_warp_bwd_variant(int v) {
+  const int was = g_warp_bwd_variant;
+  if (v == 0 || v == 1) g_warp_bwd_variant = v;
+  return was;
+}
+
+extern "C" int vmg_warp_bwd_last_kernel(void) { return g_warp_bwd_last_kernel; }
 
 extern "C" int vmg_warp_nearest_planes(const float* loc, const float* flow, float* out, int N, int K2, int H, int W, void* stream) {
   VMG_CHECK(loc && flow && out && N > 0 && K2 > 0 && H > 0 && W > 0, "warp_nearest: bad arguments");
diff --git a/vmg_amd/functional.py b/vmg_amd/functional.py
--- a/vmg_amd/functional.py
+++ b/vmg_amd/functional.py
@@ -48,6 +48,8 @@
 
 USE_WS = True
 GROUPED_DENSE = True
+SHARE_STATE_ACC = True
+CHAIN_ACT_EPILOGUE = True
 
 class _PlanState:
 
@@ -545,7 +547,8 @@
         pg = [None] * len(params)
         pd1 = [packed(params[2 + 4 * k], dt, "dgrad", None, 0, C, tiles=tiles, deep=deep) for k in range(nblk)]
         pd2 = [packed(params[4 + 4 * k], dt, "dgrad", None, 0, C, tiles=tiles, deep=deep) for k in range(nblk)]
-        gys, gts = K.resblock_chain_backward(g, ts, pd1, pd2, r, deep)
+        fused0 = CHAIN_ACT_EPILOGUE and nblk > 0 and (pd1[0].layout == "ws" or deep == hip.CONV_KSPLIT)
+        gys, gts = K.resblock_chain_backward(g, ts, pd1, pd2, r, deep, *((y0.contiguous(), 0.1) if fused0 else ()))
         with DEFERRED.collecting() if ctx.defer else contextlib.nullcontext():
             for k in range(nblk - 1, -1, -1):
                 w1, b1, w2, b2 = params[2 + 4 * k: 6 + 4 * k]
@@ -557,7 +560,7 @@
                     pg[2 + 4 * k], pg[3 + 4 * k] = _wgrad_now(w1, True, [ys[k]], [C], gts[k], 3, N, H, W)
             g = gys[0]
             w0, b0 = params[0], params[1]
-            dpre0 = K.act_backward(g, y0, hip.ACT_LRELU, 0.1, 1.0)
+            dpre0 = g if fused0 else K.act_backward(g, y0, hip.ACT_LRELU, 0.1, 1.0)
             d_srcs = []
             off = 0
             for i, c in enumerate(src_ch):
@@ -1255,22 +1258,26 @@
 
 class _WarpBilinear(_Fn):
     @staticmethod
-    def forward(ctx, x, flow):
+    def forward(ctx, x, flow, bank=None):
         x = x.contiguous()
         flow = flow.contiguous()
+        ctx.bank = bank
         ctx.save_for_backward(x, flow)
         return K.warp_bilinear_forward(x, flow)
 
     @staticmethod
     def backward(ctx, dy):
         x, flow = ctx.saved_tensors
-        return K.warp_bilinear_backward(x, flow, dy)
+        if ctx.bank is not None and ctx.needs_input_grad[0]:
+            _, dflow = K.warp_bilinear_backward(x, flow, dy, dx_into=_bank_buf(ctx.bank, x))
+            return None, dflow, None
+        return (*K.warp_bilinear_backward(x, flow, dy), None)
 
 
 def grid_sample_flow(x: torch.Tensor, flow: torch.Tensor, mode: str, padding: str) -> torch.Tensor:
     if mode != "bilinear" or padding != "border":
         raise HipError("the HIP flow warp implements bilinear / border (the only combination on the path)")
-    return _WarpBilinear.apply(x, flow.float())
+    return _WarpBilinear.apply(x, flow.float(), getattr(x, "_vmg_bank", None))
 
 
 class _FlowSmooth(_Fn):
@@ -1327,6 +1334,12 @@
     def __init__(self, dtype):
         self.buf = None
         self.dtype = dtype
+
+
+def _bank_buf(bank: _GradBank, like: torch.Tensor) -> torch.Tensor:
+    if bank.buf is None:
+        bank.buf = K.ACC_POOL.take(like.shape, like.device) if like.dtype != torch.float32 else torch.zeros_like(like, dtype=torch.float32)
+    return bank.buf
 
 
 class _Banked(_Fn):
@@ -1400,9 +1413,7 @@
             if b is None or not ctx.needs_input_grad[5 + i]:
                 into.append(None)
                 continue
-            if b.buf is None:
-                b.buf = K.ACC_POOL.take(q.shape, q.device) if q.dtype != torch.float32 else torch.zeros_like(q, dtype=torch.float32)
-            into.append(b.buf)
+            into.append(_bank_buf(b, q))
         bwd = K.ltam_backward if ltam_route(t) == "args" else K.ltam_backward_tab
         dq, dk, dv, drpe = bwd(q, keys, vals, loc, rpe, decay_v, out, lse, dout, heads, wh, ww, scale, dk_into=into[:t], dv_into=into[t:],
                                drpe_into=DEFERRED.grad_of(ctx.rpe_param) if ctx.direct else None)
@@ -1446,9 +1457,7 @@
             if b is None or not ctx.needs_input_grad[3 + i]:
                 into.append(None)
                 continue
-            if b.buf is None:
-                b.buf = K.ACC_POOL.take(q.shape, q.device) if q.dtype != torch.float32 else torch.zeros_like(q, dtype=torch.float32)
-            into.append(b.buf)
+            into.append(_bank_buf(b, q))
         bwd = K.ltam_max_backward if ltam_route(t) == "args" else K.ltam_max_backward_tab
         dq, dk, dv = bwd(q, keys, vals, loc, idx, dout, heads, dk_into=into[:t], dv_into=into[t:])
         gkv = [None if into[i] is not None else (g if g.dtype == q.dtype else g.to(q.dtype)) for i, g in enumerate(dk + dv)]
diff --git a/vmg_amd/hip.py b/vmg_amd/hip.py
--- a/vmg_amd/hip.py
+++ b/vmg_amd/hip.py
@@ -15,6 +15,7 @@
 CONV_FAM_IGEMM, CONV_FAM_KSPLIT, CONV_FAM_WS, CONV_FAM_LINEAR_WRES, CONV_FAM_WSTAT = 1, 2, 3, 4, 5
 CONV_PLAN_INTS = 11
 WGRAD_V1, WGRAD_3, WGRAD_3B, WGRAD_L2, WGRAD_7 = 1, 2, 3, 4, 5
+WARP_BWD_PIXEL, WARP_BWD_QUAD = 1, 2
 
 
 def wgrad_kernel_id(kind: int, a: int = 0, b: int = 0, c: int = 0) -> int:
@@ -153,6 +154,8 @@
                                        c_int64, c_int, c_void_p, c_int, c_int, c_int, c_void_p, c_float, c_void_p]),
     "vmg_warp_bilinear_fwd": (c_int, [c_int, c_void_p, c_void_p, c_void_p, c_int, c_int, c_int, c_int, c_void_p]),
     "vmg_warp_bilinear_bwd": (c_int, [c_int, c_void_p, c_void_p, c_void_p, c_void_p, c_void_p, c_int, c_int, c_int, c_int, c_void_p]),
+    "vmg_warp_bwd_variant": (c_int, [c_int]),
+    "vmg_warp_bwd_last_kernel": (c_int, []),
     "vmg_warp_nearest_planes": (c_int, [c_void_p, c_void_p, c_void_p, c_int, c_int, c_int, c_int, c_void_p]),
     "vmg_flow_smooth": (c_int, [c_void_p, c_void_p, c_int64, c_int, c_int, c_int, c_int, c_void_p]),
     "vmg_ltam_fwd": (c_int, [c_int, c_void_p, POINTER(c_void_p), POINTER(c_void_p), c_void_p, c_void_p, c_void_p, c_void_p, c_void_p,
diff --git a/vmg_amd/kernels.py b/vmg_amd/kernels.py
--- a/vmg_amd/kernels.py
+++ b/vmg_amd/kernels.py
@@ -241,7 +241,7 @@
     return (ctypes.c_void_p * max(1, len(ts)))(*[(t.data_ptr() if t is not None else None) for t in ts])
 
 
-CHAIN_STATS = {"fwd": {}, "bwd": {}}
+CHAIN_STATS = {"fwd": {}, "bwd": {}, "act0": {}}
 
 
 def resblock_chain_forward(srcs: Sequence[torch.Tensor], pw0: PackedConv, b0: torch.Tensor, slope0: float, deep0: int, pw1: Sequence[PackedConv],
@@ -281,11 +281,13 @@
 
 
 def resblock_chain_backward(g: torch.Tensor, ts: Sequence[torch.Tensor], pd1: Sequence[PackedConv], pd2: Sequence[PackedConv], r_scaling: float,
-                            deep: int):
-    hip.require_cuda(g, *ts)
+                            deep: int, y0: Optional[torch.Tensor] = None, slope0: float = 0.0):
+    hip.require_cuda(g, y0, *ts)
     nblk = len(ts)
     N, H, W, C = g.shape
     g = g.contiguous()
+    if y0 is not None and (nblk == 0 or y0.shape != g.shape or y0.dtype != g.dtype or not y0.is_contiguous()):
+        raise HipError("resblock_chain_backward: y0 needs at least one block and a contiguous tensor of the gradient's shape and dtype")
     if nblk == 0:
         return [g], []
     blk = torch.empty((2 * nblk, N, H, W, C), dtype=g.dtype, device=g.device).unbind(0)
@@ -297,8 +299,13 @@
     d.r_scaling = r_scaling
     d.cout_tiles = pd1[0].cout_tiles
     d.deep = hip.CONV_WS if pd1[0].layout == "ws" else deep
+    if y0 is not None:
+        keep.append(_parr([y0]))
+        d.y, d.slope0 = keep[-1], slope0
     hip.check(hip.lib().vmg_resblock_chain_bwd(ctypes.byref(d), hip.stream_ptr()), "vmg_resblock_chain_bwd")
     CHAIN_STATS["bwd"][d.deep] = CHAIN_STATS["bwd"].get(d.deep, 0) + 1
+    if y0 is not None:
+        CHAIN_STATS["act0"][d.deep] = CHAIN_STATS["act0"].get(d.deep, 0) + 1
     return gys, gts
 
 
@@ -906,24 +913,43 @@
     return out
 
 
-def warp_bilinear_backward(x: torch.Tensor, flow: torch.Tensor, dy: torch.Tensor):
-    hip.require_cuda(x, flow, dy)
+WARP_STATS = {"own": 0, "into": 0}
+
+
+def warp_bilinear_backward(x: torch.Tensor, flow: torch.Tensor, dy: torch.Tensor, dx_into: Optional[torch.Tensor] = None):
+    hip.require_cuda(x, flow, dy, dx_into)
     n, h, w, c = x.shape
     if not x.is_contiguous() or flow.dtype != torch.float32 or not flow.is_contiguous() or tuple(flow.shape) != (n, h, w, 2):
         raise HipError("warp: x must be contiguous (n,h,w,c), flow contiguous fp32 (n,h,w,2)")
     if dy.dtype != x.dtype or tuple(dy.shape) != (n, h, w, c):
         raise HipError(f"warp_bilinear_backward: dy must have x's shape and dtype, got {tuple(dy.shape)} {dy.dtype}")
+    if dx_into is not None and (dx_into.dtype != torch.float32 or tuple(dx_into.shape) != (n, h, w, c) or not dx_into.is_contiguous()):
+        raise HipError("warp_bilinear_backward: dx_into must be a contiguous fp32 accumulator of x's shape")
     dy = dy.contiguous()
-    pooled = x.dtype != torch.float32 and (n * h * w * c) % 4 == 0
-    dx_acc = ACC_POOL.take((n, h, w, c), x.device) if pooled else torch.zeros((n, h, w, c), dtype=torch.float32, device=x.device)
+    pooled = dx_into is None and x.dtype != torch.float32 and (n * h * w * c) % 4 == 0
+    if dx_into is not None:
+        dx_acc = dx_into
+    else:
+        dx_acc = ACC_POOL.take((n, h, w, c), x.device) if pooled else torch.zeros((n, h, w, c), dtype=torch.float32, device=x.device)
     dflow = torch.empty((n, h, w, 2), dtype=torch.float32, device=x.device)
     hip.check(hip.lib().vmg_warp_bilinear_bwd(hip.dtype_code(x.dtype), x.data_ptr(), flow.data_ptr(), dy.data_ptr(), dx_acc.data_ptr(),
                                               dflow.data_ptr(), n, h, w, c, hip.stream_ptr()), "vmg_warp_bilinear_bwd")
+    WARP_STATS["into" if dx_into is not None else "own"] += 1
+    if dx_into is not None:
+        return None, dflow
     if pooled:
         dx = cast_clear(dx_acc, x.dtype)
         ACC_POOL.give(dx_acc)
         return dx, dflow
     return dx_acc.to(x.dtype), dflow
+
+
+def warp_bwd_variant(v: int = -1) -> int:
+    return int(hip.lib().vmg_warp_bwd_variant(int(v)))
+
+
+def warp_bwd_last_kernel() -> int:
+    return int(hip.lib().vmg_warp_bwd_last_kernel())
 
 
 def flow_smooth(x: torch.Tensor, r: int, backward: bool = False) -> torch.Tensor:
diff --git a/vmg_amd/model.py b/vmg_amd/model.py
--- a/vmg_amd/model.py
+++ b/vmg_amd/model.py
@@ -370,12 +370,18 @@
                 if key:
                     loc = torch.cat([loc, ident], 1)
             feat = self.resblocks([cur_c, feat])
-            hd = list(FH.fan_out(feat, 1 + (0 if last else 1) + (1 if key else 0)))
-            f_out = hd.pop()
-            feat_next = None if last else hd.pop()
-            if key:
-                k_state.append(FH.grad_bank(hd.pop()))
-                k_in.append(FH.grad_bank(cur_k))
+            if FH.SHARE_STATE_ACC and not last:
+                f_out = feat_next = FH.grad_bank(feat)
+                if key:
+                    k_state.append(feat_next)
+                    k_in.append(FH.grad_bank(cur_k))
+            else:
+                hd = list(FH.fan_out(feat, 1 + (0 if last else 1) + (1 if key else 0)))
+                f_out = hd.pop()
+                feat_next = None if last else hd.pop()
+                if key:
+                    k_state.append(FH.grad_bank(hd.pop()))
+                    k_in.append(FH.grad_bank(cur_k))
             feats.append(f_out)
         back, fwd = FH.unpair_steps(feats, n)
         out = conv(self.fusion, [back, x, fwd], n * t, h, w, act=ACT_LRELU, slope=0.1)
```
